# h-walk/PSA

Hardware: AMD Instinct MI355X
Metric: SED throughput (k-points*timesteps*atoms/s) (higher is better)
Workload: dtype f32 (2xf16 split MFMA, fp32 accumulate)

## Files before the change

### include/psa_hip.h

```cpp
#ifndef PSA_HIP_H
#define PSA_HIP_H

#include <stdint.h>

#ifdef __cplusplus
extern "C" {
#endif

#define PSA_HIP_ABI_VERSION 6

#define PSA_OK          0
#define PSA_EINVAL     -1
#define PSA_EHIP       -2
#define PSA_EFFT       -3
#define PSA_ERCCL      -4
#define PSA_ESTATE     -5
#define PSA_ENOMEM     -6

#define PSA_SLOT_VELOCITIES 0
#define PSA_SLOT_POSITIONS  1
#define PSA_NUM_SLOTS       2

#define PSA_F_DISPLACEMENTS  0x1
#define PSA_F_INTENSITY      0x2

#define PSA_K1_AUTO   0
#define PSA_K1_WAVE   1
#define PSA_K1_MFMA32 2
#define PSA_K1_SPLIT_BF16 3

typedef struct psa_ctx psa_ctx;

int         psa_abi_version(void);
const char* psa_last_error(void);
int         psa_device_count(int* count);
int         psa_host_alloc(size_t bytes, void** out);
int         psa_host_free(void* p);
int         psa_create(int device, psa_ctx** out);
int         psa_destroy(psa_ctx* ctx);
int         psa_synchronize(psa_ctx* ctx);
int         psa_set_k1(psa_ctx* ctx, int selector);
int         psa_set_k1_lowrank_fold(psa_ctx* ctx, int on);
#define PSA_OPT_PLANES         0
#define PSA_OPT_PLANES_BUDGET  1
#define PSA_OPT_PLANES_EAGER   2
#define PSA_OPT_PLANES_MIN_K   3
#define PSA_OPT_FOLD_PAIRS     4
#define PSA_OPT_FFT_PRIME      5
#define PSA_OPT_K1_LOADER_WAVES 6
#define PSA_OPT_K1_WIDE         7
#define PSA_OPT_K1_LOWRANK      8
#define PSA_OPT_K1_LOWRANK_MIN_K 9
#define PSA_OPT_K1_LOWRANK_MIN_LOCAL 10
#define PSA_OPT_VDOS_WORK_BYTES 11
#define PSA_OPT_MODES_WORK_BYTES 12
#define PSA_OPT_DYNAMIC_WORK_BYTES 13
#define PSA_OPT_K1_LOWRANK_PAIR 15
int         psa_set_option(psa_ctx* ctx, int option, int64_t value);
int         psa_option_info(int index, int32_t* option, int64_t* default_value, const char** name);
int         psa_device_info(psa_ctx* ctx, char* name, int name_len,
                            int* compute_units, int64_t* hbm_bytes);

int psa_data_upload(psa_ctx* ctx, int slot, const float* host, int64_t T, int64_t N);
int psa_data_alloc(psa_ctx* ctx, int slot, int64_t T, int64_t N);
int psa_data_download(psa_ctx* ctx, int slot, float* host, int64_t t0, int64_t nt);
int psa_data_release(psa_ctx* ctx, int slot);
int psa_data_shape(psa_ctx* ctx, int slot, int64_t* T, int64_t* N);

int psa_data_fill_synthetic(psa_ctx* ctx, int slot, uint64_t seed, int64_t t_offset, int n_modes,
                            const float* amp, const int32_t* mode_comp,
                            const float* ct, const float* st,
                            const float* ca, const float* sa);

int psa_mean_positions(psa_ctx* ctx, int slot, float* mean_host );

int psa_host_mean_frames(const float* x , int64_t T, int64_t cols, float* mean_out, int threads);

int psa_set_atom_weights(psa_ctx* ctx, const float* w , int64_t N);

int psa_set_segments(psa_ctx* ctx, int64_t L, int64_t hop, const float* window );

int psa_sed_project(psa_ctx* ctx, int slot,
                    const float* mean_pos_all,
                    const float* k_vectors, int64_t K_local,
                    int64_t K_total, int64_t k_offset,
                    const int32_t* group_idx, const int64_t* group_off, int32_t G,
                    int32_t flags);

int psa_sed_project_upload(psa_ctx* ctx, int slot, const float* host, int64_t T, int64_t N,
                           const float* mean_pos_all, const float* k_vectors, int64_t K,
                           const int32_t* group_idx, const int64_t* group_off, int32_t G,
                           int32_t flags);

int psa_sed_finalize(psa_ctx* ctx, void* out_host, size_t out_bytes,
                     float* out_intensity, size_t out_intensity_bytes);

int psa_sed_calculate(psa_ctx* ctx, int slot, const float* mean_pos_all,
                      const float* k_vectors, int64_t K,
                      const int32_t* group_idx, const int64_t* group_off, int32_t G,
                      int32_t flags, void* out_host, size_t out_bytes,
                      float* out_intensity, size_t out_intensity_bytes);

int psa_vdos(psa_ctx* ctx, int slot, const float* mean_pos_all ,
             const int32_t* group_idx, const int64_t* group_off, int32_t G,
             int32_t flags , float* out_host , size_t out_bytes);

int psa_sed_modes(psa_ctx* ctx, int slot, const float* mean_pos_all, const float* k_vectors, int64_t K,
                  const int32_t* group_idx, const int64_t* group_off, int32_t B,
                  const void* eig , int64_t M, int32_t flags ,
                  float* out_host , size_t out_bytes);

int psa_sed_covariance(psa_ctx* ctx, int slot, const float* mean_pos_all, const float* k_vectors, int64_t K,
                       const int32_t* group_idx, const int64_t* group_off, int32_t B,
                       const float* freq_weights , int32_t n_w, int32_t flags ,
                       double* out_host , size_t out_bytes);

typedef struct {
    float   window_hwhm;
    int32_t half_window_bins;
    int32_t max_iter;
} psa_peak_opts;
int psa_fit_peaks(psa_ctx* ctx, const float* spec_host, int64_t F, int64_t C, double df, const int32_t* bands, int32_t lo,
                  int32_t hi, const psa_peak_opts* opts, float* fit , int32_t* info );
int psa_sed_modes_fit(psa_ctx* ctx, int slot, const float* mean_pos_all, const float* k_vectors, int64_t K,
                      const int32_t* group_idx, const int64_t* group_off, int32_t B, const void* eig, int64_t M,
// ... 31 lines not shown
                             const int32_t* bin_of , int64_t n_bins, const int32_t* idx, int64_t n_g,
                             int32_t currents , int64_t n_lags,
                             float* out_host , size_t out_bytes);

int psa_self_correlations(psa_ctx* ctx, const double* box_inverse , const int32_t* indices , int64_t K,
                          const int32_t* bin_of , int64_t n_bins, const int32_t* idx, int64_t n_g, int64_t n_lags,
                          float* out_host , size_t out_bytes);

int psa_displacement_moments(psa_ctx* ctx, const double* box , const double* box_inverse , const int32_t* idx,
                             const int64_t* group_start , int32_t n_groups, int64_t n_lags, int64_t origin_step,
                             int32_t unwrap, double* out_host , size_t out_bytes);

int psa_van_hove_self(psa_ctx* ctx, const double* box , const double* box_inverse , const int32_t* idx,
                      const int64_t* group_start , int32_t n_groups, const int64_t* lags , int64_t n_vh,
                      int64_t origin_step, int32_t unwrap, double dr, int32_t n_r, uint64_t* out_host ,
                      size_t out_bytes);

int psa_pair_histogram(psa_ctx* ctx, const double* box , const double* box_inverse , const int32_t* idx,
                       const int64_t* group_start , int32_t n_groups, const int64_t* lags , int64_t n_lags,
                       int64_t origin_step, double dr, int32_t n_r, uint64_t* out_host ,
                       size_t out_bytes);

int psa_angle_histogram(psa_ctx* ctx, const double* box , const double* box_inverse , const int32_t* idx,
                        const int64_t* group_start , int32_t n_groups, const double* r_cut , int64_t origin_step,
                        int32_t n_theta, uint64_t* angles , size_t angles_bytes,
                        uint64_t* coord , size_t coord_bytes, uint64_t* truncated );

int psa_bond_order(psa_ctx* ctx, const double* box , const double* box_inverse , const int32_t* idx,
                   const int64_t* group_start , int32_t n_groups, const double* r_cut , int64_t origin_step,
                   const int32_t* ls , int32_t n_ls, int32_t n_q, uint64_t* hist , size_t hist_bytes,
                   uint64_t* truncated , uint64_t* isolated , uint64_t* undefined ,
                   int64_t* x , int32_t* n );

int psa_local_order(psa_ctx* ctx, const double* box , const double* box_inverse , const int32_t* idx,
                    const int64_t* group_start , int32_t n_groups, const double* r_cut , int64_t origin_step,
                    const int32_t* ls , int32_t n_ls, int32_t n_q, int32_t n_w, double w_range, int32_t solid_l,
                    double solid_threshold, const double* w3j , int64_t w3j_count, uint64_t* hist ,
                    size_t hist_bytes, double* qbar2 , double* w ,
                    double* wbar , int32_t* connections , int32_t* n );

int psa_debug_qlm(psa_ctx* ctx, const double* box , const double* box_inverse , const int32_t* idx,
                  const int64_t* group_start , int32_t n_groups, const double* r_cut , int64_t frame,
                  const int32_t* ls , int32_t n_ls, int64_t* q );

int psa_solid_clusters(psa_ctx* ctx, const double* box , const double* box_inverse , const int32_t* idx,
                       const int64_t* group_start , int32_t n_groups, const double* r_cut , int64_t origin_step,
                       int32_t solid_l, double solid_threshold, int32_t min_connections, int32_t link, int32_t n_sizes,
                       uint64_t* species_rows , uint64_t* size_counts , uint64_t* large_atoms ,
                       int32_t* n_solid , int32_t* n_clusters , int32_t* largest ,
                       int32_t* largest_label , int32_t* labels , int32_t* size_atoms ,
                       int32_t* connections , int32_t* n , uint64_t* bond_masks );

int psa_debug_cluster_labels(psa_ctx* ctx, int64_t n_o, int64_t n_a, const int32_t* count ,
                             const int32_t* list , const uint8_t* solid ,
                             const uint64_t* bond_masks , int32_t link, int32_t n_sizes,
                             uint64_t* size_counts , uint64_t* large_atoms , int32_t* n_solid ,
                             int32_t* n_clusters , int32_t* largest , int32_t* largest_label ,
                             int32_t* labels , int32_t* size_atoms );

int psa_bond_persistence(psa_ctx* ctx, const double* box , const double* box_inverse , const int32_t* idx,
                         const int64_t* group_start , int32_t n_groups, const double* r_cut ,
                         const double* r_break , int64_t origin_step, const int64_t* lags , int32_t n_lags,
                         int64_t sample_step, int32_t continuous, uint64_t* bonds ,
                         uint64_t* alive , uint64_t* unbroken , size_t pair_bytes ,
                         uint64_t* lost , size_t lost_bytes, uint64_t* truncated ,
                         size_t truncated_bytes, uint64_t* alive_masks ,
                         uint64_t* unbroken_masks , size_t masks_bytes );

int psa_common_neighbours(psa_ctx* ctx, const double* box , const double* box_inverse , const int32_t* idx,
                          const int64_t* group_start , int32_t n_groups, const double* r_cut ,
                          int64_t origin_step, uint64_t* signature_counts , size_t signature_bytes,
                          uint64_t* signature_outside , uint64_t* type_counts , size_t type_bytes,
                          uint64_t* truncated , int32_t* types , int32_t* n ,
                          size_t atom_bytes , uint32_t* bond_signatures ,
                          size_t bond_bytes);

#define PSA_KMAP_MIRROR 0x80000000u
int psa_k_pairs(const float* k_vectors, int64_t K, int32_t* kmap ,
                int32_t* unique_idx , int64_t* n_unique);
int psa_sed_set_kmap(psa_ctx* ctx, const int32_t* kmap, int64_t K_out);

int psa_lowrank_plan(const float* k_vectors, int64_t K, const float* mean_pos_all, int64_t N, const int32_t* idx,
                     int64_t n_g, int32_t* ok, double* geo, double* kappa, float* C, float* L, float* phi);

int psa_sed_single_bin(psa_ctx* ctx, int slot, const float* mean_pos_all, const float* k_vector,
                       const int32_t* idx, int64_t n_g, int32_t flags, int64_t i_w,
                       float* out_c64x3 );

int psa_slab_read(psa_ctx* ctx, int64_t row0, int64_t nrows, void* host);
int psa_slab_write(psa_ctx* ctx, int64_t row0, int64_t nrows, const void* host);

int psa_result_intensity(psa_ctx* ctx, float* out_host , size_t out_bytes);
int psa_result_chiral_phase(psa_ctx* ctx, int c1, int c2, float* out_host, size_t out_bytes);

int psa_last_timings(psa_ctx* ctx, double* ms );
int psa_k1_stats(psa_ctx* ctx, int64_t* launches, double* total_ms);
int psa_k1_lowrank_launches(psa_ctx* ctx, int64_t* launches);
int psa_k1_lowrank_pair_launches(psa_ctx* ctx, int64_t* launches);
int psa_lowrank_pair_image(int32_t n_stage, int64_t* index, int64_t* bytes);
int psa_lowrank_fold_image(int32_t n_stage, int64_t* index, int64_t* bytes);
int psa_debug_device_buffers(int64_t* count, int64_t* bytes);
#define PSA_SCRATCH_REAL 0
#define PSA_SCRATCH_INDEX 1
#define PSA_SCRATCH_STATE 2
int psa_debug_scratch_info(int index, const char** name, int32_t* cls);
int psa_debug_scratch_fill(psa_ctx* ctx, int byte, int64_t* buffers, int64_t* bytes);
int psa_oneoff_stats(psa_ctx* ctx, double* ms );

int psa_debug_phase_table(psa_ctx* ctx, const float* mean_pos_all,
                          const float* k_vectors, int64_t K,
                          const int32_t* idx, int64_t n_g, int64_t N,
                          void* out_host);
int psa_debug_project_only(psa_ctx* ctx, int slot, const float* mean_pos_all,
                           const float* k_vectors, int64_t K,
                           const int32_t* idx, int64_t n_g, int32_t flags,
                           void* out_host);
int psa_debug_project_route(psa_ctx* ctx, int slot, const float* mean_pos_all,
                            const float* k_vectors, int64_t K,
                            const int32_t* idx, int64_t n_g, int32_t flags,
                            void* out_host);
int psa_debug_project_frames(psa_ctx* ctx, int slot, const float* mean_pos_all,
                             const float* k_vectors, int64_t K,
                             const int32_t* idx, int64_t n_g, int32_t flags,
                             int64_t t_begin, int64_t t_count, void* out_host);
int psa_debug_mode_power(psa_ctx* ctx, const void* S_host, const void* eig, int32_t B, int64_t K, int64_t M, int64_t T,
                         float* out_host);
int psa_debug_covariance(psa_ctx* ctx, const void* S_host , int32_t B, int64_t K,
                         int64_t T, const float* freq_weights, int32_t n_w, double scale, double* out_host);
int psa_debug_mode_power_welch(psa_ctx* ctx, const void* S_host, const void* eig, int32_t B, int64_t K, int64_t M, int64_t L,
                               int64_t ns, int64_t seg_block, float scale, float* out_host);
int psa_debug_dynamic_project(psa_ctx* ctx, const float* k_vectors, int64_t K, const int32_t* idx, int64_t n_g,
                              int32_t currents, void* out_host);
int psa_debug_dynamic_sincos(psa_ctx* ctx, const float* turns, int64_t n, float* out_host);
int psa_debug_lattice_project(psa_ctx* ctx, const double* box_inverse, const int32_t* indices, int64_t K, const int32_t* idx,
                              int64_t n_g, int32_t currents, void* out_host);
int psa_debug_self_series(psa_ctx* ctx, const double* box_inverse, const int32_t* indices, int64_t K, const int32_t* idx,
                          int64_t n_g, void* out_host);
int psa_debug_dynamic_power(psa_ctx* ctx, const void* seg_host, const float* k_vectors , int64_t K, int32_t currents,
                            int64_t n_seg, int64_t L, int64_t k_block, int64_t seg_block, float scale, float* out_host);
int psa_debug_lattice_shell(psa_ctx* ctx, const void* seg_host, const float* khat , const int32_t* bin_of ,
                            int64_t K, int64_t n_bins, int32_t currents, int64_t n_seg, int64_t L, int64_t k_block,
                            int64_t seg_block, double norm, float* out_host);
int psa_debug_self_power(psa_ctx* ctx, const void* work_host, int64_t na, int64_t nv, int64_t n_seg, int64_t L,
                         const int32_t* groups, int64_t n_groups, int64_t cols, const double* scale, int32_t mirror,
                         int64_t n_chunks, int64_t atom_block, int64_t vec_block, int64_t seg_block, float* out_host);
int psa_debug_partial_project(psa_ctx* ctx, const double* box_inverse, const int32_t* indices, int64_t K, const int32_t* idx,
                              const int64_t* species_start, int32_t n_species, int32_t currents, void* out_host);
int psa_debug_partial_power(psa_ctx* ctx, const void* seg_host, const float* khat , const int32_t* bin_of ,
                            int64_t K, int64_t n_bins, int32_t n_species, int32_t currents, int64_t n_seg, int64_t L,
                            int64_t k_block, int64_t seg_block, double norm, float* out_host);
int psa_debug_plane_cache(psa_ctx* ctx, int64_t* n_sets, int64_t* bytes);

#define PSA_UNIQUE_ID_BYTES 128
int psa_comm_unique_id(void* out );
int psa_comm_init(psa_ctx* ctx, const void* unique_id, int rank, int nranks);
int psa_comm_destroy(psa_ctx* ctx);
int psa_comm_selftest(psa_ctx* ctx);
int psa_sed_gather(psa_ctx* ctx, int root, const int64_t* k_offsets, const int64_t* k_counts);
int psa_comm_barrier(psa_ctx* ctx);

int psa_sed_fs_project(psa_ctx* ctx, int slot, const float* mean_pos_all,
                       const float* k_vectors, int64_t K_total,
                       const int32_t* idx, int64_t n_g, int32_t flags,
                       int64_t T_total, int64_t k_offset, int64_t k_count);
int psa_sed_fs_exchange(psa_ctx* ctx, const int64_t* t_offsets, const int64_t* t_counts,
                        const int64_t* k_offsets, const int64_t* k_counts);
int psa_sed_fs_read(psa_ctx* ctx, int64_t k0, int64_t nk, void* host);
int psa_sed_fs_write(psa_ctx* ctx, int64_t t0, int64_t nt, const void* host);
int psa_sed_fs_finish(psa_ctx* ctx, int32_t first_group);

int psa_debug_correlation_transform(psa_ctx* ctx, const double* X_host, int64_t fields, int64_t P, int64_t cols, int64_t L,
                                    int64_t n_seg, int64_t n_lags, int32_t as_float32, float* out_host);

int psa_debug_unwrap(psa_ctx* ctx, const double* box , const double* box_inverse , const int32_t* idx, int64_t n_g,
                     int32_t unwrap, double* out_u , int32_t* out_images );

int psa_debug_pair_fractions(psa_ctx* ctx, const double* box_inverse , const int32_t* idx, int64_t n_g,
                             float* out );

int psa_debug_pair_plan(const int64_t* sizes , int32_t n_groups, int32_t sym, int64_t n_origins, int64_t* out );

int psa_debug_neighbour_lists(psa_ctx* ctx, const double* box , const double* box_inverse , const int32_t* idx,
                              const int64_t* group_start , int32_t n_groups, const double* r_cut , int64_t frame,
// ... 7 lines not shown
```

### psa_amd/_hip.py

```python
from __future__ import annotations

import ctypes as C
import os
import threading
import weakref
from pathlib import Path
from types import SimpleNamespace
from typing import Optional, Sequence

import numpy as np

LIB_PATH = Path(__file__).resolve().parent / "csrc" / "libpsa_hip.so"

SLOT_VELOCITIES, SLOT_POSITIONS = 0, 1
F_DISPLACEMENTS, F_INTENSITY = 0x1, 0x2
K1_AUTO, K1_WAVE, K1_MFMA32, K1_SPLIT_BF16 = 0, 1, 2, 3
OPT_PLANES, OPT_PLANES_BUDGET, OPT_PLANES_EAGER, OPT_PLANES_MIN_K, OPT_FOLD_PAIRS, OPT_FFT_PRIME = 0, 1, 2, 3, 4, 5
OPT_K1_LOADER_WAVES = 6
OPT_K1_WIDE = 7
OPT_K1_LOWRANK = 8
OPT_K1_LOWRANK_MIN_K = 9
OPT_K1_LOWRANK_MIN_LOCAL = 10
OPT_VDOS_WORK_BYTES = 11
OPT_MODES_WORK_BYTES = 12
OPT_DYNAMIC_WORK_BYTES = 13
OPT_K1_LOWRANK_PAIR = 15
KMAP_MIRROR = 0x80000000
ABI_VERSION = 6
COV_CHAIN = 128
COV_FOLDS = 32
COV_TILE = 64
COV_CHUNK = COV_CHAIN * COV_FOLDS
COV_MAX_ROWS = 96
DYN_THREADS = 256
DYN_ATOMS = 512
DYN_CHAIN = 128
DYN_FRAMES = 4
DYN_SINCOS_ERR = 2.6e-7
LAT_THREADS = 256
LAT_KS = 512
LAT_ATOMS = 128
LAT_TABLE = 3584
LAT_CHAIN = 128
LAT_FRAMES = 4
LAT_MAX_INDEX = 64
LAT_MAX_ENTRIES = 3 * (2 * LAT_MAX_INDEX + 1)
PARTIAL_MAX_SPECIES = 8
SELF_THREADS = 256
SELF_ATOMS = 4
SELF_FRAMES = 64
SELF_ENTRIES = 24
SELF_KS = 64
MSD_LAGS = 256
MSD_ORIGINS = 1024
MSD_WINDOW = 1280
MSD_MAX_GROUPS = 8
MSD_MAX_BINS = 1024
MSD_MAX_VH_LAGS = 64
MSD_UNWRAP_FRAMES = 64
MSD_UNWRAP_ATOMS = 16
PAIR_TILE = 256
PAIR_MAX_BINS = 1024
PAIR_MAX_LAGS = 64
PAIR_MAX_SPECIES = 8
ANGLE_MAX_NEIGHBOURS = 64
ANGLE_MAX_BINS = 1024
ORDER_MAX_L = 12
ORDER_MAX_LS = 8
ORDER_MAX_BINS = 1024
ORDER_SHIFT = 24
LOCAL_MAX_LS = 4
LOCAL_MAX_BINS = 1024
LOCAL_SHIFT = 40
CLUSTER_MAX_SIZES = 4096
CLUSTER_ROW_WORDS = ANGLE_MAX_NEIGHBOURS + 1 + 4
CLUSTER_LINKS = ("neighbours", "solid_bonds")
PERSIST_MAX_LAGS = 1024
CNA_TABLE = (8, 16, 16)
CNA_TYPES = ("other", "fcc", "hcp", "bcc", "ico")
UNIQUE_ID_BYTES = 128
TIMING_NAMES = ("h2d", "phase", "project", "fft", "epilogue", "gather", "transpose", "d2h")

_f32p = C.POINTER(C.c_float)
_i32p = C.POINTER(C.c_int32)
_i64p = C.POINTER(C.c_int64)
_f64p = C.POINTER(C.c_double)
_u64p = C.POINTER(C.c_uint64)
_ctx = C.c_void_p

SIGNATURES = {
    "psa_abi_version": (C.c_int, []),
    "psa_last_error": (C.c_char_p, []),
    "psa_device_count": (C.c_int, [C.POINTER(C.c_int)]),
    "psa_host_alloc": (C.c_int, [C.c_size_t, C.POINTER(C.c_void_p)]),
    "psa_host_free": (C.c_int, [C.c_void_p]),
    "psa_create": (C.c_int, [C.c_int, C.POINTER(_ctx)]),
    "psa_destroy": (C.c_int, [_ctx]),
    "psa_synchronize": (C.c_int, [_ctx]),
    "psa_set_k1": (C.c_int, [_ctx, C.c_int]),
    "psa_set_k1_lowrank_fold": (C.c_int, [_ctx, C.c_int]),
    "psa_set_option": (C.c_int, [_ctx, C.c_int, C.c_int64]),
    "psa_device_info": (C.c_int, [_ctx, C.c_char_p, C.c_int, C.POINTER(C.c_int), _i64p]),
    "psa_data_upload": (C.c_int, [_ctx, C.c_int, _f32p, C.c_int64, C.c_int64]),
    "psa_data_alloc": (C.c_int, [_ctx, C.c_int, C.c_int64, C.c_int64]),
    "psa_data_download": (C.c_int, [_ctx, C.c_int, _f32p, C.c_int64, C.c_int64]),
    "psa_data_release": (C.c_int, [_ctx, C.c_int]),
    "psa_data_shape": (C.c_int, [_ctx, C.c_int, _i64p, _i64p]),
    "psa_data_fill_synthetic": (C.c_int, [_ctx, C.c_int, C.c_uint64, C.c_int64, C.c_int, _f32p, _i32p,
                                          _f32p, _f32p, _f32p, _f32p]),
    "psa_mean_positions": (C.c_int, [_ctx, C.c_int, _f32p]),
    "psa_host_mean_frames": (C.c_int, [_f32p, C.c_int64, C.c_int64, _f32p, C.c_int]),
    "psa_set_atom_weights": (C.c_int, [_ctx, _f32p, C.c_int64]),
    "psa_set_segments": (C.c_int, [_ctx, C.c_int64, C.c_int64, _f32p]),
    "psa_sed_project": (C.c_int, [_ctx, C.c_int, _f32p, _f32p, C.c_int64, C.c_int64, C.c_int64,
                                  _i32p, _i64p, C.c_int32, C.c_int32]),
    "psa_sed_project_upload": (C.c_int, [_ctx, C.c_int, _f32p, C.c_int64, C.c_int64, _f32p, _f32p, C.c_int64,
                                         _i32p, _i64p, C.c_int32, C.c_int32]),
    "psa_sed_finalize": (C.c_int, [_ctx, C.c_void_p, C.c_size_t, _f32p, C.c_size_t]),
    "psa_sed_calculate": (C.c_int, [_ctx, C.c_int, _f32p, _f32p, C.c_int64, _i32p, _i64p,
                                    C.c_int32, C.c_int32, C.c_void_p, C.c_size_t, _f32p, C.c_size_t]),
    "psa_vdos": (C.c_int, [_ctx, C.c_int, _f32p, _i32p, _i64p, C.c_int32, C.c_int32, _f32p, C.c_size_t]),
    "psa_sed_modes": (C.c_int, [_ctx, C.c_int, _f32p, _f32p, C.c_int64, _i32p, _i64p, C.c_int32, C.c_void_p, C.c_int64,
                                C.c_int32, _f32p, C.c_size_t]),
    "psa_fit_peaks": (C.c_int, [_ctx, _f32p, C.c_int64, C.c_int64, C.c_double, _i32p, C.c_int32, C.c_int32, C.c_void_p,
                                _f32p, _i32p]),
    "psa_sed_modes_fit": (C.c_int, [_ctx, C.c_int, _f32p, _f32p, C.c_int64, _i32p, _i64p, C.c_int32, C.c_void_p, C.c_int64,
                                    C.c_int32, C.c_double, _i32p, C.c_int32, C.c_int32, C.c_void_p, _f32p, _i32p, _f32p,
                                    C.c_size_t]),
    "psa_sed_modes_welch": (C.c_int, [_ctx, C.c_int, _f32p, _f32p, C.c_int64, _i32p, _i64p, C.c_int32, C.c_void_p, C.c_int64,
                                      C.c_int32, _f32p, C.c_size_t]),
    "psa_sed_modes_welch_fit": (C.c_int, [_ctx, C.c_int, _f32p, _f32p, C.c_int64, _i32p, _i64p, C.c_int32, C.c_void_p,
                                          C.c_int64, C.c_int32, C.c_double, _i32p, C.c_int32, C.c_int32, C.c_void_p, _f32p,
                                          _i32p, _f32p, C.c_size_t]),
    "psa_dynamic_spectra": (C.c_int, [_ctx, _f32p, C.c_int64, _i32p, C.c_int64, C.c_int32, _f32p, C.c_size_t]),
    "psa_debug_dynamic_project": (C.c_int, [_ctx, _f32p, C.c_int64, _i32p, C.c_int64, C.c_int32, C.c_void_p]),
    "psa_debug_dynamic_sincos": (C.c_int, [_ctx, _f32p, C.c_int64, _f32p]),
    "psa_lattice_spectra": (C.c_int, [_ctx, _f64p, _i32p, C.c_int64, _i32p, C.c_int64, _i32p, C.c_int64, C.c_int32,
                                      _f32p, C.c_size_t]),
    "psa_debug_lattice_project": (C.c_int, [_ctx, _f64p, _i32p, C.c_int64, _i32p, C.c_int64, C.c_int32, C.c_void_p]),
    "psa_self_spectra": (C.c_int, [_ctx, _f64p, _i32p, C.c_int64, _i32p, C.c_int64, _i32p, C.c_int64, _f32p,
                                   C.c_size_t]),
    "psa_debug_self_series": (C.c_int, [_ctx, _f64p, _i32p, C.c_int64, _i32p, C.c_int64, C.c_void_p]),
    "psa_debug_dynamic_power": (C.c_int, [_ctx, C.c_void_p, _f32p, C.c_int64, C.c_int32, C.c_int64, C.c_int64, C.c_int64, C.c_int64,
                                          C.c_float, _f32p]),
    "psa_debug_lattice_shell": (C.c_int, [_ctx, C.c_void_p, _f32p, _i32p, C.c_int64, C.c_int64, C.c_int32, C.c_int64, C.c_int64,
                                          C.c_int64, C.c_int64, C.c_double, _f32p]),
    "psa_debug_self_power": (C.c_int, [_ctx, C.c_void_p, C.c_int64, C.c_int64, C.c_int64, C.c_int64, _i32p, C.c_int64, C.c_int64,
                                       _f64p, C.c_int32, C.c_int64, C.c_int64, C.c_int64, C.c_int64, _f32p]),
    "psa_partial_spectra": (C.c_int, [_ctx, _f64p, _i32p, C.c_int64, _i32p, C.c_int64, _i32p, _i64p, C.c_int32,
                                      C.c_int32, _f32p, C.c_size_t]),
    "psa_debug_partial_project": (C.c_int, [_ctx, _f64p, _i32p, C.c_int64, _i32p, _i64p, C.c_int32, C.c_int32,
                                            C.c_void_p]),
    "psa_debug_partial_power": (C.c_int, [_ctx, C.c_void_p, _f32p, _i32p, C.c_int64, C.c_int64, C.c_int32, C.c_int32, C.c_int64,
                                          C.c_int64, C.c_int64, C.c_int64, C.c_double, _f32p]),
    "psa_lattice_correlations": (C.c_int, [_ctx, _f64p, _i32p, C.c_int64, _i32p, C.c_int64, _i32p, C.c_int64,
                                           C.c_int32, C.c_int64, _f32p, C.c_size_t]),
    "psa_self_correlations": (C.c_int, [_ctx, _f64p, _i32p, C.c_int64, _i32p, C.c_int64, _i32p, C.c_int64,
                                        C.c_int64, _f32p, C.c_size_t]),
    "psa_debug_correlation_transform": (C.c_int, [_ctx, _f64p, C.c_int64, C.c_int64, C.c_int64, C.c_int64,
                                                  C.c_int64, C.c_int64, C.c_int32, _f32p]),
    "psa_displacement_moments": (C.c_int, [_ctx, _f64p, _f64p, _i32p, _i64p, C.c_int32, C.c_int64,
                                           C.c_int64, C.c_int32, _f64p, C.c_size_t]),
    "psa_van_hove_self": (C.c_int, [_ctx, _f64p, _f64p, _i32p, _i64p, C.c_int32, _i64p, C.c_int64,
                                    C.c_int64, C.c_int32, C.c_double, C.c_int32, _u64p, C.c_size_t]),
    "psa_debug_unwrap": (C.c_int, [_ctx, _f64p, _f64p, _i32p, C.c_int64, C.c_int32,
                                   _f64p, _i32p]),
    "psa_pair_histogram": (C.c_int, [_ctx, _f64p, _f64p, _i32p, _i64p, C.c_int32, _i64p, C.c_int64,
                                     C.c_int64, C.c_double, C.c_int32, _u64p, C.c_size_t]),
    "psa_debug_pair_fractions": (C.c_int, [_ctx, _f64p, _i32p, C.c_int64, _f32p]),
    "psa_debug_pair_plan": (C.c_int, [_i64p, C.c_int32, C.c_int32, C.c_int64, _i64p]),
    "psa_angle_histogram": (C.c_int, [_ctx, _f64p, _f64p, _i32p, _i64p, C.c_int32, _f64p,
                                      C.c_int64, C.c_int32, _u64p, C.c_size_t, _u64p, C.c_size_t,
                                      _u64p]),
    "psa_debug_neighbour_lists": (C.c_int, [_ctx, _f64p, _f64p, _i32p, _i64p, C.c_int32,
                                            _f64p, C.c_int64, _i32p, _i32p]),
    "psa_bond_order": (C.c_int, [_ctx, _f64p, _f64p, _i32p, _i64p, C.c_int32, _f64p, C.c_int64,
                                 _i32p, C.c_int32, C.c_int32, _u64p, C.c_size_t, _u64p, _u64p, _u64p,
                                 _i64p, _i32p]),
    "psa_local_order": (C.c_int, [_ctx, _f64p, _f64p, _i32p, _i64p, C.c_int32, _f64p, C.c_int64,
                                  _i32p, C.c_int32, C.c_int32, C.c_int32, C.c_double, C.c_int32, C.c_double,
                                  _f64p, C.c_int64, _u64p, C.c_size_t, _f64p, _f64p, _f64p, _i32p, _i32p]),
    "psa_debug_qlm": (C.c_int, [_ctx, _f64p, _f64p, _i32p, _i64p, C.c_int32, _f64p, C.c_int64,
                                _i32p, C.c_int32, _i64p]),
    "psa_solid_clusters": (C.c_int, [_ctx, _f64p, _f64p, _i32p, _i64p, C.c_int32, _f64p, C.c_int64,
                                     C.c_int32, C.c_double, C.c_int32, C.c_int32, C.c_int32, _u64p, _u64p, _u64p,
                                     _i32p, _i32p, _i32p, _i32p, _i32p, _i32p, _i32p, _i32p, _u64p]),
    "psa_bond_persistence": (C.c_int, [_ctx, _f64p, _f64p, _i32p, _i64p, C.c_int32, _f64p, _f64p, C.c_int64,
                                       _i64p, C.c_int32, C.c_int64, C.c_int32, _u64p, _u64p, _u64p, C.c_size_t,
                                       _u64p, C.c_size_t, _u64p, C.c_size_t, _u64p, _u64p, C.c_size_t]),
    "psa_common_neighbours": (C.c_int, [_ctx, _f64p, _f64p, _i32p, _i64p, C.c_int32, _f64p, C.c_int64, _u64p, C.c_size_t,
                                        _u64p, _u64p, C.c_size_t, _u64p, _i32p, _i32p, C.c_size_t, C.POINTER(C.c_uint32),
                                        C.c_size_t]),
    "psa_debug_cluster_labels": (C.c_int, [_ctx, C.c_int64, C.c_int64, _i32p, _i32p, C.POINTER(C.c_uint8), _u64p, C.c_int32,
                                           C.c_int32, _u64p, _u64p, _i32p, _i32p, _i32p, _i32p, _i32p, _i32p]),
    "psa_k_pairs": (C.c_int, [_f32p, C.c_int64, _i32p, _i32p, _i64p]),
    "psa_lowrank_plan": (C.c_int, [_f32p, C.c_int64, _f32p, C.c_int64, _i32p, C.c_int64, _i32p, _f64p,
                                   _f64p, _f32p, _f32p, _f32p]),
    "psa_sed_set_kmap": (C.c_int, [_ctx, _i32p, C.c_int64]),
    "psa_sed_single_bin": (C.c_int, [_ctx, C.c_int, _f32p, _f32p, _i32p, C.c_int64, C.c_int32, C.c_int64, _f32p]),
    "psa_slab_read": (C.c_int, [_ctx, C.c_int64, C.c_int64, C.c_void_p]),
    "psa_slab_write": (C.c_int, [_ctx, C.c_int64, C.c_int64, C.c_void_p]),
    "psa_result_intensity": (C.c_int, [_ctx, _f32p, C.c_size_t]),
    "psa_result_chiral_phase": (C.c_int, [_ctx, C.c_int, C.c_int, _f32p, C.c_size_t]),
    "psa_last_timings": (C.c_int, [_ctx, _f64p]),
    "psa_k1_stats": (C.c_int, [_ctx, _i64p, _f64p]),
    "psa_k1_lowrank_launches": (C.c_int, [_ctx, _i64p]),
    "psa_k1_lowrank_pair_launches": (C.c_int, [_ctx, _i64p]),
    "psa_lowrank_pair_image": (C.c_int, [C.c_int32, _i64p, _i64p]),
    "psa_lowrank_fold_image": (C.c_int, [C.c_int32, _i64p, _i64p]),
    "psa_oneoff_stats": (C.c_int, [_ctx, _f64p]),
    "psa_option_info": (C.c_int, [C.c_int, C.POINTER(C.c_int32), _i64p, C.POINTER(C.c_char_p)]),
    "psa_debug_device_buffers": (C.c_int, [_i64p, _i64p]),
    "psa_debug_scratch_info": (C.c_int, [C.c_int, C.POINTER(C.c_char_p), C.POINTER(C.c_int32)]),
    "psa_debug_scratch_fill": (C.c_int, [_ctx, C.c_int, _i64p, _i64p]),
    "psa_debug_phase_table": (C.c_int, [_ctx, _f32p, _f32p, C.c_int64, _i32p, C.c_int64,
                                        C.c_int64, C.c_void_p]),
    "psa_debug_project_only": (C.c_int, [_ctx, C.c_int, _f32p, _f32p, C.c_int64, _i32p,
                                         C.c_int64, C.c_int32, C.c_void_p]),
    "psa_debug_project_route": (C.c_int, [_ctx, C.c_int, _f32p, _f32p, C.c_int64, _i32p,
                                          C.c_int64, C.c_int32, C.c_void_p]),
    "psa_debug_project_frames": (C.c_int, [_ctx, C.c_int, _f32p, _f32p, C.c_int64, _i32p,
                                           C.c_int64, C.c_int32, C.c_int64, C.c_int64, C.c_void_p]),
    "psa_debug_mode_power": (C.c_int, [_ctx, C.c_void_p, C.c_void_p, C.c_int32, C.c_int64, C.c_int64, C.c_int64, _f32p]),
    "psa_debug_mode_power_welch": (C.c_int, [_ctx, C.c_void_p, C.c_void_p, C.c_int32, C.c_int64, C.c_int64, C.c_int64,
                                             C.c_int64, C.c_int64, C.c_float, _f32p]),
    "psa_sed_covariance": (C.c_int, [_ctx, C.c_int, _f32p, _f32p, C.c_int64, _i32p, _i64p, C.c_int32, _f32p, C.c_int32, C.c_int32,
                                     C.c_void_p, C.c_size_t]),
    "psa_debug_covariance": (C.c_int, [_ctx, C.c_void_p, C.c_int32, C.c_int64, C.c_int64, _f32p, C.c_int32, C.c_double,
                                       C.c_void_p]),
    "psa_debug_plane_cache": (C.c_int, [_ctx, _i64p, _i64p]),
    "psa_comm_unique_id": (C.c_int, [C.c_void_p]),
    "psa_comm_init": (C.c_int, [_ctx, C.c_void_p, C.c_int, C.c_int]),
    "psa_comm_destroy": (C.c_int, [_ctx]),
    "psa_comm_selftest": (C.c_int, [_ctx]),
    "psa_sed_gather": (C.c_int, [_ctx, C.c_int, _i64p, _i64p]),
    "psa_comm_barrier": (C.c_int, [_ctx]),
    "psa_sed_fs_project": (C.c_int, [_ctx, C.c_int, _f32p, _f32p, C.c_int64, _i32p, C.c_int64, C.c_int32,
                                     C.c_int64, C.c_int64, C.c_int64]),
    "psa_sed_fs_exchange": (C.c_int, [_ctx, _i64p, _i64p, _i64p, _i64p]),
    "psa_sed_fs_read": (C.c_int, [_ctx, C.c_int64, C.c_int64, C.c_void_p]),
    "psa_sed_fs_write": (C.c_int, [_ctx, C.c_int64, C.c_int64, C.c_void_p]),
    "psa_sed_fs_finish": (C.c_int, [_ctx, C.c_int32]),
}


class PeakOpts(C.Structure):
    _fields_ = [("window_hwhm", C.c_float), ("half_window_bins", C.c_int32), ("max_iter", C.c_int32)]


class PsaHipError(RuntimeError):
    """A libpsa_hip entry point returned a non-zero code."""


_lib = None
_lib_lock = threading.Lock()


def load_library() -> C.CDLL:
    global _lib
    with _lib_lock:
        if _lib is not None:
            return _lib
        path = Path(os.environ.get("PSA_HIP_LIBRARY", LIB_PATH))
        if not path.exists():
            raise PsaHipError(
                f"{path} not found: build it with `make -C psa_amd/csrc` (needs hipcc, gfx950). "
                "psa_amd has no CPU fallback.")
        os.environ.setdefault("HSA_ENABLE_IPC_MODE_LEGACY", "0")
        lib = C.CDLL(str(path))
        for name, (res, args) in SIGNATURES.items():
            fn = getattr(lib, name)
            fn.restype, fn.argtypes = res, args
        _lib = lib
        return lib


def _check(rc: int, what: str):
    if rc != 0:
        msg = load_library().psa_last_error().decode("utf-8", "replace")
        if rc == -1 and "out of bounds" in msg:
            raise ValueError(msg)
        raise PsaHipError(f"{what} failed (rc={rc}): {msg}")


def _f32(a: np.ndarray):
    return a.ctypes.data_as(_f32p)


def _as_f32(a, shape_tail=None) -> np.ndarray:
    arr = np.ascontiguousarray(a, dtype=np.float32)
    if shape_tail is not None and arr.shape[1:] != shape_tail:
        raise ValueError(f"expected (*,{shape_tail}) array, got {arr.shape}")
    return arr


def device_count() -> int:
    n = C.c_int(0)
    _check(load_library().psa_device_count(C.byref(n)), "psa_device_count")
    return n.value


def option_table():
    lib, rows = load_library(), []
    opt, default, name = C.c_int32(0), C.c_int64(0), C.c_char_p()
    while lib.psa_option_info(len(rows), C.byref(opt), C.byref(default), C.byref(name)) == 0:
        rows.append((opt.value, name.value.decode(), default.value))
    return rows


def device_buffers():
    n, b = C.c_int64(0), C.c_int64(0)
    _check(load_library().psa_debug_device_buffers(C.byref(n), C.byref(b)), "psa_debug_device_buffers")
    return n.value, b.value


SCRATCH_CLASSES = ("real", "index", "state")


def scratch_table():
    lib, rows = load_library(), []
    name, cls = C.c_char_p(), C.c_int32(0)
    while lib.psa_debug_scratch_info(len(rows), C.byref(name), C.byref(cls)) == 0:
        rows.append((name.value.decode(), SCRATCH_CLASSES[cls.value]))
    return rows


def k_pairs(k_vectors):
    kv = _as_f32(k_vectors, (3,)) if len(k_vectors) else np.zeros((0, 3), np.float32)
    K = kv.shape[0]
    kmap, uidx, n = np.zeros(K, np.int32), np.zeros(K, np.int32), C.c_int64(0)
    _check(load_library().psa_k_pairs(_f32(kv), K, kmap.ctypes.data_as(_i32p), uidx.ctypes.data_as(_i32p), C.byref(n)),
           "psa_k_pairs")
    return kmap.view(np.uint32), uidx[:n.value].copy()


def lowrank_plan(k_vectors, mean_pos_all, idx=None):
    kv = _as_f32(k_vectors, (3,))
    mean = _as_f32(mean_pos_all, (3,))
    K, N = kv.shape[0], mean.shape[0]
    ix = None if idx is None else np.ascontiguousarray(idx, np.int32)
    n_g = N if ix is None else ix.size
    ok, geo = C.c_int32(0), np.zeros(14, np.float64)
    kappa, cm = np.zeros(64, np.float64), np.zeros((K, 64), np.complex64)
    lw, phi = np.zeros((K, 64), np.float32), np.zeros(K, np.complex64)
    _check(load_library().psa_lowrank_plan(_f32(kv), K, _f32(mean), N, None if ix is None else ix.ctypes.data_as(_i32p), n_g,
                                           C.byref(ok), geo.ctypes.data_as(_f64p), kappa.ctypes.data_as(_f64p),
                                           cm.ctypes.data_as(_f32p), _f32(lw), phi.ctypes.data_as(_f32p)), "psa_lowrank_plan")
    if not ok.value:
        return None
    return {"u": geo[0:3].copy(), "k0": geo[3:6].copy(), "x_c": geo[6], "h_x": geo[7], "width": geo[8],
            "interval": int(geo[9]), "d_bound": geo[10], "dscale": geo[11], "e_bound": geo[12],
            "dscale_fold": geo[13], "kappa": kappa, "C": cm, "L": lw, "phi": phi}


def lowrank_pair_image(n_stage: int):
    index, nbytes = np.zeros((512, 32 * int(n_stage)), np.int64), C.c_int64(0)
    _check(load_library().psa_lowrank_pair_image(int(n_stage), index.ctypes.data_as(_i64p), C.byref(nbytes)), "psa_lowrank_pair_image")
    return index, nbytes.value


def lowrank_fold_image(n_stage: int):
    index, nbytes = np.zeros((512, 32 * int(n_stage)), np.int64), C.c_int64(0)
    _check(load_library().psa_lowrank_fold_image(int(n_stage), index.ctypes.data_as(_i64p), C.byref(nbytes)), "psa_lowrank_fold_image")
    return index, nbytes.value


def host_mean_frames(x: np.ndarray, threads: int = 0) -> np.ndarray:
    if x.dtype != np.float32 or not x.flags.c_contiguous or x.ndim < 2 or x.shape[0] < 1 or x.size == 0:
        raise ValueError("host_mean_frames needs a non-empty C-contiguous float32 array")
    out = np.empty(x.shape[1:], np.float32)
    cols = int(np.prod(x.shape[1:], dtype=np.int64))
    _check(load_library().psa_host_mean_frames(_f32(x), x.shape[0], cols, _f32(out), int(threads)), "psa_host_mean_frames")
    return out


def pack_groups(groups: Optional[Sequence[np.ndarray]]):
    if groups is None:
        return None, None, 1
    off = np.zeros(len(groups) + 1, dtype=np.int64)
    off[1:] = np.cumsum([len(g) for g in groups])
    idx = (np.concatenate([np.asarray(g).ravel() for g in groups]) if off[-1] > 0
           else np.zeros(0, dtype=np.int64))
    if idx.size and (idx.min() < 0 or idx.max() >= 2 ** 31):
        raise ValueError("Atom indices in basis out of bounds.")
    return np.ascontiguousarray(idx, dtype=np.int32), off, len(groups)


class _PinnedPool:

    granule = 2 << 20
    min_bytes = 1 << 20
    keep_bytes = 4 << 30
    max_live_bytes = 16 << 30

    def __init__(self):
        self._idle = {}
        self._idle_bytes = 0
        self._live_bytes = 0
        self._lock = threading.Lock()
        self.stats = {"recycled": 0, "allocated": 0, "pageable": 0}

    def _give_back(self, address: int, size: int):
        with self._lock:
            self._live_bytes -= size
            if self._idle_bytes + size <= self.keep_bytes:
                self._idle.setdefault(size, []).append(address)
                self._idle_bytes += size
                return
        load_library().psa_host_free(C.c_void_p(address))

    def empty(self, shape, dtype) -> np.ndarray:
        dtype = np.dtype(dtype)
        nbytes = int(np.prod(shape, dtype=np.int64)) * dtype.itemsize
        if nbytes < self.min_bytes:
            return np.empty(shape, dtype)
        size = -(-nbytes // self.granule) * self.granule
        with self._lock:
            if self._live_bytes + size > self.max_live_bytes:
                self.stats["pageable"] += 1
                return np.empty(shape, dtype)
            self._live_bytes += size
            stack = self._idle.get(size)
            address = stack.pop() if stack else None
            if address is not None:
                self._idle_bytes -= size
        if address is None:
            p = C.c_void_p()
            try:
                _check(load_library().psa_host_alloc(size, C.byref(p)), "psa_host_alloc")
            except PsaHipError:
                with self._lock:
                    self._live_bytes -= size
                    self.stats["pageable"] += 1
                return np.empty(shape, dtype)
            address = p.value
            self.stats["allocated"] += 1
        else:
            self.stats["recycled"] += 1
        block = (C.c_char * size).from_address(address)
        weakref.finalize(block, self._give_back, address, size)
        return np.frombuffer(block, dtype=dtype, count=nbytes // dtype.itemsize).reshape(shape)

    def drain(self):
        with self._lock:
            idle, self._idle, self._idle_bytes = self._idle, {}, 0
        for stack in idle.values():
            for address in stack:
                load_library().psa_host_free(C.c_void_p(address))


_pinned_pool = _PinnedPool()


def pinned_empty(shape, dtype) -> np.ndarray:
    return _pinned_pool.empty(shape, dtype)


_SAMPLE_CACHE = {}


def _sample_positions(shape):
    hit = _SAMPLE_CACHE.get(shape)
    if hit is None:
        size = int(np.prod(shape, dtype=np.int64))
        lin = np.arange(0, size, max(1, size // 1021), dtype=np.int64)[:1021]
        if size > 2048:
            lin = np.concatenate([lin, np.sort(np.random.default_rng(size).integers(0, size, 1021)), [size - 1]])
        if len(_SAMPLE_CACHE) > 64:
            _SAMPLE_CACHE.clear()
        hit = _SAMPLE_CACHE[shape] = (lin, np.unravel_index(lin, shape))
    return hit


class Engine:

    def __init__(self, device: Optional[int] = None):
        self._lib = load_library()
        if device is None:
            device = int(os.environ.get("PSA_HIP_DEVICE", os.environ.get("LOCAL_RANK", "0")))
            n = device_count()
            if n == 0:
                raise PsaHipError("no HIP device visible; psa_amd has no CPU fallback")
            device %= n
        h = _ctx()
        _check(self._lib.psa_create(int(device), C.byref(h)), "psa_create")
        self._h = h
        self.device = int(device)
        self._resident = {}
        self._converted = {}
        self.lock = threading.RLock()
        self.rank, self.nranks = 0, 1
        self.result_serial = 0
        self.segment_length = 0

    def close(self):
        if getattr(self, "_h", None):
            self._lib.psa_destroy(self._h)
            self._h = None

    def __del__(self):
        try:
            self.close()
        except Exception:
            pass

    def synchronize(self):
        _check(self._lib.psa_synchronize(self._h), "psa_synchronize")

    def set_k1(self, selector: int):
        _check(self._lib.psa_set_k1(self._h, selector), "psa_set_k1")

    def set_lowrank_fold(self, on: bool):
        _check(self._lib.psa_set_k1_lowrank_fold(self._h, int(bool(on))), "psa_set_k1_lowrank_fold")

    def device_info(self) -> dict:
        name = C.create_string_buffer(256)
        cu, mem = C.c_int(0), C.c_int64(0)
        _check(self._lib.psa_device_info(self._h, name, 256, C.byref(cu), C.byref(mem)),
               "psa_device_info")
        return {"name": name.value.decode(), "compute_units": cu.value, "hbm_bytes": mem.value}

    @staticmethod
    def _fingerprint(a: np.ndarray) -> int:
        if a.size == 0:
            return 0
        base = a
        while base is not None and not isinstance(base, np.memmap):
            base = getattr(base, "base", None)
        if base is not None and getattr(base, "filename", None):
            try:
                st = os.stat(base.filename)
                return hash((str(base.filename), st.st_size, st.st_mtime_ns, a.shape, a.strides))
            except OSError:
                pass
        lin, idx = _sample_positions(a.shape)
        if a.flags.c_contiguous:
            return hash(a.reshape(-1)[lin].tobytes())
        return hash(a[idx].tobytes())

    def _as_device_layout(self, slot: int, array: np.ndarray) -> np.ndarray:
        if array.ndim != 3 or array.shape[2] != 3:
            raise ValueError("trajectory array must be (frames, atoms, 3)")
        if array.dtype == np.float32 and array.flags.c_contiguous:
            return array
        held = self._converted.get(slot)
        fp = self._fingerprint(array)
        if held is not None and held[0]() is array and held[1] == fp:
            return held[2]
        conv = np.ascontiguousarray(array, dtype=np.float32)
        try:
            self._converted[slot] = (weakref.ref(array), fp, conv)
        except TypeError:
            self._converted.pop(slot, None)
        return conv

    def is_resident(self, slot: int, array: np.ndarray) -> bool:
        held = self._resident.get(slot)
        if held is None or held[0] is None:
            return False
        a = array if held[0]() is array else self._as_device_layout(slot, array)
        return (held[0]() is a and held[1:3] == (a.ctypes.data, a.shape) and held[3] == self._fingerprint(a))

    def _note_resident(self, slot: int, a: np.ndarray):
        try:
            ref = weakref.ref(a)
        except TypeError:
            ref = None
        self._resident[slot] = (ref, a.ctypes.data, a.shape, self._fingerprint(a))

    def ensure_resident(self, slot: int, array: np.ndarray):
        if self.is_resident(slot, array):
            return
        a = self._as_device_layout(slot, array)
        T, N = a.shape[0], a.shape[1]
        _check(self._lib.psa_data_upload(self._h, slot, _f32(a), T, N), "psa_data_upload")
        self._note_resident(slot, a)

    def invalidate(self, slot: Optional[int] = None):
        if slot is None:
            self._resident.clear()
            self._converted.clear()
        else:
            self._resident.pop(slot, None)
            self._converted.pop(slot, None)

    def alloc(self, slot: int, T: int, N: int):
        _check(self._lib.psa_data_alloc(self._h, slot, T, N), "psa_data_alloc")
        self._resident[slot] = (None, None, (T, N, 3), None)

    def fill_synthetic(self, slot: int, seed: int, amp, comp, ct, st, ca, sa, t_offset: int = 0):
        amp = np.ascontiguousarray(amp, np.float32)
        comp = np.ascontiguousarray(comp, np.int32)
        tabs = [np.ascontiguousarray(x, np.float32) for x in (ct, st, ca, sa)]
        _check(self._lib.psa_data_fill_synthetic(
            self._h, slot, C.c_uint64(seed), int(t_offset), len(amp), _f32(amp), comp.ctypes.data_as(_i32p),
            *[_f32(t) for t in tabs]), "psa_data_fill_synthetic")

# ... 841 lines not shown
```

### psa_amd/csrc/api_core.hip

```cpp
#include "api_internal.h"

#include <unistd.h>

#include <atomic>
#include <filesystem>

namespace psa {

thread_local std::string g_error;


void set_error(const char* fmt, ...) {
    char    buf[1024];
    va_list ap;
    va_start(ap, fmt);
    vsnprintf(buf, sizeof(buf), fmt, ap);
    va_end(ap);
    g_error = buf;
}

static std::atomic<int64_t> g_devbuf_count{0}, g_devbuf_bytes{0};

int DevBuf::reserve(size_t bytes) {
    if (bytes <= cap) return PSA_OK;
// ... 305 lines not shown
    c->compute_units = prop.multiProcessorCount;
    if (const char* v = std::getenv("PSA_K1_LOWRANK")) c->opt_k1_lowrank = std::atoi(v) != 0;
    if (const char* v = std::getenv("PSA_K1_LOWRANK_MIN_K")) c->opt_k1_lowrank_min_k = std::max(1, std::atoi(v));
    hipError_t e = hipStreamCreateWithFlags(&c->stream, hipStreamNonBlocking);
    if (e != hipSuccess) {
        delete c;
        set_error("hipStreamCreate failed: %s", hipGetErrorString(e));
        return PSA_EHIP;
    }
    *out = c;
    return PSA_OK;
}

int psa_destroy(psa_ctx* c) {
    if (!c) return PSA_OK;
    { Guard g(c); }
    (void)hipSetDevice(c->device);
    delete c;
    return PSA_OK;
}

int psa_debug_device_buffers(int64_t* count, int64_t* bytes) {
    PSA_REQUIRE(count != nullptr && bytes != nullptr, "null argument");
    *count = g_devbuf_count.load();
    *bytes = g_devbuf_bytes.load();
    return PSA_OK;
}

int psa_debug_scratch_info(int index, const char** name, int32_t* cls) {
    PSA_REQUIRE(index >= 0 && index < (int)std::size(SCRATCH), "no device buffer at index %d", index);
    if (name) *name = SCRATCH[index].name;
    if (cls) *cls = SCRATCH[index].cls;
    return PSA_OK;
}

int psa_debug_scratch_fill(psa_ctx* c, int byte, int64_t* buffers, int64_t* bytes) {
    PSA_TRY(enter(c));
    PSA_REQUIRE(byte >= -1 && byte <= 255, "the fill byte is 0 .. 255, or -1 to disarm");
    Guard g(c);
    PSA_HIP_CHECK(hipStreamSynchronize(c->stream));
    if (c->d2h_stream) PSA_HIP_CHECK(hipStreamSynchronize(c->d2h_stream));
    if (c->stager.copy_stream) PSA_HIP_CHECK(hipStreamSynchronize(c->stager.copy_stream));
    int64_t n = 0, total = 0;
    c->scratch_byte = byte;
    for (const Scratch& s : SCRATCH) {
        DevBuf& b = c->*s.member;
        b.fill = byte < 0 || s.cls == PSA_SCRATCH_STATE ? nullptr : s.cls == PSA_SCRATCH_REAL ? &c->scratch_byte : &SCRATCH_ZERO;
        if (!b.fill || !b.ptr) continue;
        PSA_HIP_CHECK(hipMemsetAsync(b.ptr, *b.fill, b.cap, c->stream));
        n += 1;
        total += (int64_t)b.cap;
    }
    PSA_HIP_CHECK(hipStreamSynchronize(c->stream));
    if (byte >= 0) c->slab_valid = c->out_valid = c->inten_valid = false;
    if (buffers) *buffers = n;
    if (bytes) *bytes = total;
    return PSA_OK;
}

int psa_synchronize(psa_ctx* c) {
    PSA_TRY(enter(c));
    Guard g(c);
    PSA_HIP_CHECK(hipStreamSynchronize(c->stream));
    return PSA_OK;
}

int psa_set_k1(psa_ctx* c, int selector) {
    PSA_TRY(enter(c));
    PSA_REQUIRE(selector == PSA_K1_AUTO || selector == PSA_K1_WAVE || selector == PSA_K1_MFMA32 ||
                    selector == PSA_K1_SPLIT_BF16,
                "unknown K1 selector %d", selector);
    Guard g(c);
    c->k1_selector = selector;
    return PSA_OK;
}

int psa_set_k1_lowrank_fold(psa_ctx* c, int on) {
    PSA_TRY(enter(c));
    Guard g(c);
    c->k1_lowrank_fold = on != 0;
    return PSA_OK;
}

int psa_set_option(psa_ctx* c, int option, int64_t value) {
    PSA_TRY(enter(c));
    Guard g(c);
    for (const Option& o : OPTIONS) {
        if (o.id != option) continue;
        if (o.min == OPT_FLAG) value = value != 0;
        else if (o.min == 0) PSA_REQUIRE(value >= 0, "negative plane budget");
        else PSA_REQUIRE(value >= o.min, "%s must be >= %lld", o.name, (long long)o.min);
        c->*o.field = value;
        if (option == PSA_OPT_PLANES && !value) {
            PSA_HIP_CHECK(hipStreamSynchronize(c->stream));
            c->planes.clear();
        } else if (option == PSA_OPT_K1_LOWRANK && !value) {
            PSA_HIP_CHECK(hipStreamSynchronize(c->stream));
            for (DevBuf* b : {&c->d_lr_diff, &c->d_lr_qn, &c->d_lr_L, &c->d_lr_phi, &c->d_lr_f64}) b->release();
        }
        return PSA_OK;
    }
    set_error("unknown option %d", option);
    return PSA_EINVAL;
}

int psa_option_info(int index, int32_t* option, int64_t* default_value, const char** name) {
    PSA_REQUIRE(index >= 0 && index < (int)std::size(OPTIONS), "no option at index %d", index);
    if (option) *option = OPTIONS[index].id;
    if (default_value) *default_value = OPTIONS[index].def;
    if (name) *name = OPTIONS[index].name;
    return PSA_OK;
}

int psa_device_info(psa_ctx* c, char* name, int name_len, int* compute_units, int64_t* hbm_bytes) {
    PSA_TRY(enter(c));
    hipDeviceProp_t prop;
    PSA_HIP_CHECK(hipGetDeviceProperties(&prop, c->device));
    if (name && name_len > 0) {
        std::snprintf(name, (size_t)name_len, "%s (%s)", prop.name[0] ? prop.name : "AMD GPU",
                      prop.gcnArchName);
    }
    if (compute_units) *compute_units = prop.multiProcessorCount;
    if (hbm_bytes) *hbm_bytes = (int64_t)prop.totalGlobalMem;
    return PSA_OK;
}

int psa_last_timings(psa_ctx* c, double* ms) {
    PSA_TRY(enter(c));
    PSA_REQUIRE(ms != nullptr, "null output");
    Guard guard(c);
    TimingState& ts = timing(c);
    PSA_TRY(collect(c, ts));
    for (int i = 0; i < PSA_T_COUNT; ++i) {
        ms[i] = ts.acc[i];
        ts.acc[i] = 0.0;
    }
    return PSA_OK;
}

int psa_oneoff_stats(psa_ctx* c, double* ms) {
    PSA_TRY(enter(c));
    PSA_REQUIRE(ms != nullptr, "null output");
    Guard guard(c);
    for (int i = 0; i < 4; ++i) {
        ms[i] = c->oneoff_ms[i];
        c->oneoff_ms[i] = 0.0;
    }
    return PSA_OK;
}

int psa_k1_lowrank_launches(psa_ctx* c, int64_t* launches) {
    PSA_TRY(enter(c));
    PSA_REQUIRE(launches != nullptr, "null argument");
    *launches = c->lowrank_launches;
    return PSA_OK;
}

int psa_k1_lowrank_pair_launches(psa_ctx* c, int64_t* launches) {
    PSA_TRY(enter(c));
    PSA_REQUIRE(launches != nullptr, "null argument");
    *launches = c->lowrank_pair_launches;
    return PSA_OK;
}

int psa_k1_stats(psa_ctx* c, int64_t* launches, double* total_ms) {
    PSA_TRY(enter(c));
// ... 12 lines not shown
```

### psa_amd/csrc/api_internal.h

```cpp
#pragma once
#include <algorithm>
#include <chrono>
#include <cmath>
#include <condition_variable>
#include <cstdlib>
#include <cstring>
#include <functional>
#include <thread>
#include <unordered_map>

#include "k1_f16.h"

namespace psa {

extern thread_local std::string g_error;

struct HostTimer {
    double*                               into;
    std::chrono::steady_clock::time_point t0 = std::chrono::steady_clock::now();
    explicit HostTimer(double* into_) : into(into_) {}
    ~HostTimer() { *into += std::chrono::duration<double, std::milli>(std::chrono::steady_clock::now() - t0).count(); }
};

struct Guard {
// ... 18 lines not shown
    TimingState& ts;
    int          stage;
    hipEvent_t   e0 = nullptr, e1 = nullptr;
    bool         ok = false;
    StageTimer(psa_ctx* c_, int stage_) : c(c_), ts(timing(c_)), stage(stage_) {
        if (get_event(ts, &e0) == PSA_OK && get_event(ts, &e1) == PSA_OK &&
            hipEventRecord(e0, c->stream) == hipSuccess)
            ok = true;
    }
    ~StageTimer() {
        if (ok && hipEventRecord(e1, c->stream) == hipSuccess) {
            ts.pending.push_back({stage, e0, e1});
            return;
        }
        for (hipEvent_t ev : {e0, e1})
            if (ev) ts.pool.push_back(ev);
    }
};

int upload(psa_ctx* c, DevBuf& b, const void* host, size_t bytes);
int get_plan(psa_ctx* c, int64_t T, int64_t batch, FftPlan** out);
void prime_fft(psa_ctx* c, int64_t T);
int run_fft(psa_ctx* c, float2* data, int64_t T, int64_t batch);
int check_slot(psa_ctx* c, int slot);
int validate_groups(int64_t N, const int32_t* group_idx, const int64_t* group_off, int32_t G);

struct GroupView {
    int            slot = 0;
    bool           disp = false;
    int64_t        n_g = 0;
    const int*     d_idx = nullptr;
    const int32_t* h_idx = nullptr;
    PlaneSet*      ps = nullptr;
};
inline void set_group(const psa_ctx* c, const int32_t* group_idx, const int64_t* group_off, int gi, int64_t N, GroupView* v) {
    v->n_g = group_idx ? group_off[gi + 1] - group_off[gi] : N;
    v->d_idx = group_idx ? c->d_idx.as<int>() + group_off[gi] : nullptr;
    v->h_idx = group_idx ? group_idx + group_off[gi] : nullptr;
}

int  slot_absmax(psa_ctx* c, int slot);
int  group_absmax(psa_ctx* c, int slot, const int32_t* h_idx, int64_t n_g, unsigned* bits);
int  displaced_absmax(psa_ctx* c, int slot, const float* mean_host, const int32_t* h_idx, int64_t n_g, unsigned* bits);
int  stager_init(psa_ctx* c, size_t chunk_bytes);
void stager_release(psa_ctx* c);
int  staged_upload(psa_ctx* c, float* dev, const float* host, int64_t T, int64_t N,
                   const std::function<int(int64_t, int64_t, hipEvent_t)>& on_chunk);
int  data_alloc_locked(psa_ctx* c, int slot, int64_t T, int64_t N);
int  materialise_displacements(psa_ctx* c, GroupView* v, const float* mean_host);

struct ProjectArgs {
    int            slot;
    const float*   mean_pos_all;
    const float*   k_vectors;
    int64_t        K_local, K_total, k_offset;
    const int32_t* group_idx;
    const int64_t* group_off;
    int32_t        G, flags;
};

enum class GeomRule { product, bf16_anywhere, f32_only };

size_t planes_bytes_held(psa_ctx* c);
void   drop_stale_planes(psa_ctx* c);
int    get_planes(psa_ctx* c, const GroupView& v, int64_t K_local, const float* mean_host, PlaneSet** out);
int    group_source(psa_ctx* c, GroupView* v, const float* mean_host, int64_t K);
int    make_geom(psa_ctx* c, const GroupView& v, int64_t K_local, GeomRule rule, ProjGeom* g);
int    prepare_phase(psa_ctx* c, const GroupView& v, const ProjGeom& g, int64_t k_first);
int    launch_projection(psa_ctx* c, const GroupView& v, ProjGeom g, float2* d_q, int64_t q_stride, int64_t t_begin,
                         int64_t t_count);
int    prepare_block(psa_ctx* c, const GroupView& v, GeomRule rule, const ProjectArgs* lowrank, int64_t k_first, int64_t nk,
                     ProjGeom* g);
int    project_block(psa_ctx* c, const GroupView& v, const ProjectArgs* lowrank, int64_t k_first, int64_t nk, float2* d_q);
int    check_group_indices(const GroupView& v, int64_t N);
int    upload_single_group(psa_ctx* c, GroupView* v, int64_t N, const float* k_vectors, int64_t K, const float* mean_pos_all);
void   fold_pairs(const float* k, int64_t K, std::vector<int32_t>* kmap, std::vector<int32_t>* unique_idx);
int    install_kmap(psa_ctx* c, const std::vector<int32_t>& kmap);
struct LowRankPlan {
    bool                ok = false;
    const char*         why = "";
    double              u[3] = {0, 0, 0}, k0[3] = {0, 0, 0};
    double              x_c = 0, h_x = 0, width = 0;
    int64_t             interval = 0;
    double              kappa[LOWRANK_NODES] = {};
    double              d_bound = 0;
    float               dscale = 0.f;
    double              e_bound = 0;
    float               dscale_fold = 0.f;
    std::vector<double> kline;
    std::vector<float>  L;
    std::vector<float>  phi;
};
int plan_lowrank(const float* k, int64_t K, const float* mean_all, int64_t N, const int32_t* h_idx, int64_t n_g, LowRankPlan* p,
                 float* C = nullptr);
int prepare_lowrank(psa_ctx* c, const GroupView& v, const ProjectArgs& list, int64_t k_first, int64_t nk, ProjGeom* g);
struct ModesArgs {
    int            slot;
    const float*   mean_pos_all;
    const float*   k_vectors;
    int64_t        K;
    const int32_t* group_idx;
    const int64_t* group_off;
    int32_t        B;
    const float*   eig;
    int64_t        M;
    int32_t        flags;
    float*         out;
    size_t         out_bytes;
};
int modes_run(psa_ctx* c, const ModesArgs& a, bool segments, bool device_only);
struct ModesCall {
    int64_t                T = 0, N = 0, K = 0, M = 0;
    int32_t                B = 0;
    int                    MT = 0;
    size_t                 coef_k = 0;
    int64_t                per_k = 0;
    int64_t                kb_max = 0;
    ProjectArgs            list;
    std::vector<float>     coef;
    std::vector<GroupView> src;
};
int     modes_check_groups(psa_ctx* c, int slot, const float* mean_pos_all, const float* k_vectors, int64_t K, const int32_t* group_idx,
                           const int64_t* group_off, int32_t B, int32_t flags, ModesCall* m);
int     modes_upload(psa_ctx* c, ModesCall* m);
int64_t modes_block(const psa_ctx* c, const ModesCall& m, int64_t k0, int64_t kb);
int     modes_project(psa_ctx* c, const ModesCall& m, int64_t k0, int64_t nk, float2* d_work);
struct PeakArgs {
    int64_t        F, C;
    double         df;
    const int32_t* bands;
    int32_t        lo, hi;
    psa_peak_opts  opts;
    float*         fit;
    int32_t*       info;
    int            row0 = 0, row_end = 0;
};
int check_peak_args(const psa_peak_opts* opts, PeakArgs* a);
int peaks_run(psa_ctx* c, const float* d_spec, const PeakArgs& a);
struct DynCall {
    int64_t T = 0, N = 0, K = 0, n_g = 0;
    int     NC = 1, slices = 1;
    int     n_species = 1;
    bool    cut = false;
    int64_t L = 0, H = 0, n_seg = 0;
    int64_t n_lags = 0, P = 0;
    int64_t per_k = 0, unit = 0;
    int64_t kb = 0, bk = 0, bs = 0;
    std::vector<float> kappa, khat;
};
int dynamic_inputs(psa_ctx* c, const char* entry, int64_t K, const int32_t* idx, int64_t n_g, int32_t currents, DynCall* d);
int segment_shape(const psa_ctx* c, bool segments, DynCall* d);
int dynamic_plan(psa_ctx* c, DynCall* d);
struct PowerPass {
    int          NC = 1;
    int          n_species = 0;
    int64_t      L = 0, n_seg = 0, K = 0;
    float        scale = 0.f;
    const float* d_khat = nullptr;
    float*       d_out = nullptr;
    const int*   d_bins = nullptr;
    double*      d_acc = nullptr;
    int64_t      n_bins = 0;
};
using SegFill = std::function<int(int64_t k1, int64_t nb, int64_t s0, int64_t ns, const float2** d_seg)>;
int  power_block(psa_ctx* c, const PowerPass& p, int64_t k0, int64_t nk, int64_t bk, int64_t bs, const SegFill& fill);
struct BlockSource {
    std::function<int()>                                                     upload;
    std::function<int(int64_t block, int64_t k0, int64_t nk, float2* d_q)> project;
};
struct SpectraRun {
    BlockSource src;
    bool        pairs = false;
    int64_t     n_bins = 0;
    std::function<int(const float* d_power, const double* d_acc)> finish;
    float*      out_host = nullptr;
    size_t      out_bytes = 0;
};
// ... 108 lines not shown
```

### psa_amd/csrc/api_lowrank.hip

```cpp
#include "api_internal.h"
#include "k1_lowrank_fold.h"
#include "k1_lowrank_pair.h"

namespace psa {

namespace {
constexpr double LR_OMEGA = 30.0;
constexpr double LR_D_MAX = 1.0 / 8192.0;
}

int plan_lowrank(const float* k, int64_t K, const float* mean_all, int64_t N, const int32_t* h_idx, int64_t n_g, LowRankPlan* p,
                 float* C) {
    *p = LowRankPlan{};
    auto fail = [&](const char* why) {
        p->why = why;
        return PSA_OK;
    };
    if (K < 2) return fail("fewer than two k-vectors");
    if (n_g < 1) return fail("empty group");
    for (int64_t i = 0; i < 3 * K; ++i)
        if (!std::isfinite(k[i])) return fail("k-vector not finite");
    double  p0[3] = {k[0], k[1], k[2]}, far = 0.0;
    int64_t jf = 0;
    for (int64_t j = 1; j < K; ++j) {
        double d2 = 0.0;
        for (int i = 0; i < 3; ++i) d2 += ((double)k[3 * j + i] - p0[i]) * ((double)k[3 * j + i] - p0[i]);
        if (d2 > far) {
            far = d2;
            jf = j;
        }
    }
    if (!(far > 0.0)) return fail("all k-vectors equal");
    double u[3], nu = std::sqrt(far);
    for (int i = 0; i < 3; ++i) u[i] = ((double)k[3 * jf + i] - p0[i]) / nu;
    {
        int im = 0;
        for (int i = 1; i < 3; ++i)
            if (std::fabs(u[i]) > std::fabs(u[im])) im = i;
        if (u[im] < 0)
            for (double& v : u) v = -v;
    }
    bool snapped = false;
    for (int n = 1; n <= 12 && !snapped; ++n) {
        double m[3], mn = 0.0, dev = 0.0;
        const double s = n / std::max({std::fabs(u[0]), std::fabs(u[1]), std::fabs(u[2])});
        for (int i = 0; i < 3; ++i) {
            m[i] = std::nearbyint(u[i] * s);
            mn += m[i] * m[i];
        }
        mn = std::sqrt(mn);
        for (int i = 0; i < 3; ++i) dev = std::max(dev, std::fabs(m[i] / mn - u[i]));
        if (dev < 1e-6) {
            for (int i = 0; i < 3; ++i) u[i] = m[i] / mn + 0.0;
            snapped = true;
        }
    }
    if (!snapped) return fail("direction not a lattice direction");
    {
        double kmax2 = 0.0, off2 = 0.0;
        for (int64_t j = 0; j < K; ++j) {
            double kj[3], d = 0.0, n2 = 0.0;
            for (int i = 0; i < 3; ++i) {
                kj[i] = k[3 * j + i];
                d += kj[i] * u[i];
                n2 += kj[i] * kj[i];
            }
            double o2 = 0.0;
            for (int i = 0; i < 3; ++i) o2 += (kj[i] - d * u[i]) * (kj[i] - d * u[i]);
            kmax2 = std::max(kmax2, n2);
            off2 = std::max(off2, o2);
        }
        if (!(std::sqrt(off2) <= 1e-5 * std::sqrt(kmax2))) return fail("line does not pass through Gamma");
    }
    for (int i = 0; i < 3; ++i) p->u[i] = u[i];
    double xmin = INFINITY, xmax = -INFINITY, rmax = 0.0, rabs[3] = {0, 0, 0};
    for (int64_t a = 0; a < n_g; ++a) {
        const int64_t src = h_idx ? h_idx[a] : a;
        if (src < 0 || src >= N) return fail("index outside the trajectory");
        const float* r = mean_all + 3 * src;
        if (!std::isfinite(r[0]) || !std::isfinite(r[1]) || !std::isfinite(r[2])) return fail("mean position not finite");
        const double x = u[0] * r[0] + u[1] * r[1] + u[2] * r[2];
        xmin = std::min(xmin, x);
        xmax = std::max(xmax, x);
        rmax = std::max(rmax, std::sqrt((double)r[0] * r[0] + (double)r[1] * r[1] + (double)r[2] * r[2]));
        for (int i = 0; i < 3; ++i) rabs[i] = std::max(rabs[i], (double)std::fabs(r[i]));
    }
    p->x_c = 0.5 * (xmin + xmax);
    p->h_x = std::max(0.5 * (xmax - xmin), 1e-12);
    p->width = 2.0 * LR_OMEGA / p->h_x;
    p->kline.resize((size_t)3 * K);
    std::vector<double> kap((size_t)K);
    double              off = 0.0, kabs[3] = {0, 0, 0};
    for (int64_t j = 0; j < K; ++j) {
        double kj[3], kk = 0.0;
        for (int i = 0; i < 3; ++i) {
            kj[i] = k[3 * j + i];
            kk += (kj[i] - p->k0[i]) * u[i];
            kabs[i] = std::max(kabs[i], std::fabs(kj[i]));
        }
        kap[(size_t)j] = kk;
        double e2 = 0.0;
        for (int i = 0; i < 3; ++i) {
            p->kline[3 * j + i] = p->k0[i] + kk * u[i];
            e2 += (kj[i] - p->kline[3 * j + i]) * (kj[i] - p->kline[3 * j + i]);
        }
        off = std::max(off, std::sqrt(e2));
    }
    p->d_bound = 0x1p-22 * (kabs[0] * rabs[0] + kabs[1] * rabs[1] + kabs[2] * rabs[2]) + off * rmax + 0x1p-20;
    if (!(p->d_bound <= LR_D_MAX)) return fail("k-vectors not on one line (or phases too large)");
    bool pos = true, neg = true;
    for (int64_t j = 0; j < K; ++j) {
        pos = pos && kap[(size_t)j] >= 0.0;
        neg = neg && kap[(size_t)j] <= 0.0;
    }
    if (!pos && !neg) return fail("k-list crosses Gamma");
    const bool   side = pos;
    const double n0 = std::floor(std::fabs(kap[0]) / p->width);
    for (int64_t j = 0; j < K; ++j)
        if (std::floor(std::fabs(kap[(size_t)j]) / p->width) != n0) return fail("k-path longer than one node interval");
    p->interval = side ? (int64_t)n0 : -(int64_t)n0 - 1;
    const double mid = (p->interval + 0.5) * p->width, half = 0.5 * p->width;
    double       bw[LOWRANK_NODES];
    for (int l = 0; l < LOWRANK_NODES; ++l) {
        const double th = M_PI * (2 * l + 1) / (2.0 * LOWRANK_NODES);
        p->kappa[l] = mid + half * std::cos(th);
        bw[l] = ((l & 1) ? -1.0 : 1.0) * std::sin(th);
    }
    p->L.assign((size_t)K * LOWRANK_NODES, 0.f);
    p->phi.assign((size_t)K * 2, 0.f);
    for (int64_t j = 0; j < K; ++j) {
        const double kj = kap[(size_t)j];
        double       L[LOWRANK_NODES], den = 0.0;
        int          hit = -1;
        for (int l = 0; l < LOWRANK_NODES; ++l)
            if (kj == p->kappa[l]) hit = l;
        if (hit >= 0) {
            for (int l = 0; l < LOWRANK_NODES; ++l) L[l] = l == hit;
        } else {
            for (int l = 0; l < LOWRANK_NODES; ++l) {
                L[l] = bw[l] / (kj - p->kappa[l]);
                den += L[l];
            }
            for (double& v : L) v /= den;
        }
        const double cr = std::cos(kj * p->x_c), ci = std::sin(kj * p->x_c);
        p->phi[(size_t)j * 2 + 0] = (float)cr;
        p->phi[(size_t)j * 2 + 1] = (float)ci;
        for (int l = 0; l < LOWRANK_NODES; ++l) {
            p->L[(size_t)j * LOWRANK_NODES + l] = (float)L[l];
            if (C) {
                C[((size_t)j * LOWRANK_NODES + l) * 2 + 0] = (float)(cr * L[l]);
                C[((size_t)j * LOWRANK_NODES + l) * 2 + 1] = (float)(ci * L[l]);
            }
        }
    }
    p->dscale = std::ldexp(1.0f, 14 - (int)std::ceil(std::log2(p->d_bound)));
    for (int64_t j = 0; j < K; ++j) {
        double lam = 0.0;
        for (int l = 0; l < LOWRANK_NODES; ++l) lam += std::fabs((double)p->L[(size_t)j * LOWRANK_NODES + l]);
        const double rot = std::fabs((double)p->phi[(size_t)j * 2]) + std::fabs((double)p->phi[(size_t)j * 2 + 1]);
        p->e_bound = std::max(p->e_bound, rot * lam * 0x1p-12);
    }
    p->dscale_fold = std::ldexp(1.0f, 14 - (int)std::ceil(std::log2(p->d_bound + p->e_bound)));
    p->ok = true;
    return PSA_OK;
}

int prepare_lowrank(psa_ctx* c, const GroupView& v, const ProjectArgs& list, int64_t k_first, int64_t nk, ProjGeom* g) {
    g->lowrank = false;
    if (!c->opt_k1_lowrank || g->split != K1Family::f16_planes || !v.ps || list.K_total < c->opt_k1_lowrank_min_k ||
        nk < c->opt_k1_lowrank_min_local)
        return PSA_OK;
    LowRankPlan p;
    PSA_TRY(plan_lowrank(list.k_vectors + 3 * k_first, nk, list.mean_pos_all, c->slot[v.slot].N, v.h_idx, g->n_g, &p));
    if (!p.ok) return PSA_OK;
    std::vector<double> f64((size_t)7 + LOWRANK_NODES + 3 * (size_t)nk);
    std::memcpy(f64.data(), p.k0, 3 * sizeof(double));
    std::memcpy(f64.data() + 3, p.u, 3 * sizeof(double));
    f64[6] = p.x_c;
    std::memcpy(f64.data() + 7, p.kappa, sizeof(p.kappa));
    std::memcpy(f64.data() + 7 + LOWRANK_NODES, p.kline.data(), p.kline.size() * sizeof(double));
    PSA_TRY(upload(c, c->d_lr_f64, f64.data(), f64.size() * sizeof(double)));
    PSA_TRY(upload(c, c->d_lr_L, p.L.data(), p.L.size() * sizeof(float)));
    PSA_TRY(upload(c, c->d_lr_phi, p.phi.data(), p.phi.size() * sizeof(float)));
    PSA_TRY(c->d_lr_qn.reserve((size_t)LOWRANK_NODES * 3 * (size_t)c->slot[v.slot].T * sizeof(float2)));
    g->lowrank = true;
    g->lr_fold = c->k1_lowrank_fold;
    g->dscale = g->lr_fold ? p.dscale_fold : p.dscale;
    g->M_pad_d = (int)((2 * nk + 511) / 512 * 512);
    g->lr_pair = c->opt_k1_lowrank_pair && g->M_pad_d == LRP_ROWS;
    static_assert(LRF_ROWS == LRP_ROWS, "the folded pair launch serves the lists the pair launch serves");
    return PSA_OK;
}

}

using namespace psa;

extern "C" {

int psa_lowrank_plan(const float* k_vectors, int64_t K, const float* mean_pos_all, int64_t N, const int32_t* idx, int64_t n_g,
                     int32_t* ok, double* geo, double* kappa, float* C, float* L, float* phi) {
    PSA_REQUIRE(K >= 0 && K < (1ll << 29) && N >= 1 && n_g >= 0 && n_g <= (idx ? (int64_t)1 << 30 : N) && ok && geo &&
                    (K == 0 || k_vectors) && mean_pos_all,
                "bad argument");
    LowRankPlan p;
    PSA_TRY(plan_lowrank(k_vectors, K, mean_pos_all, N, idx, n_g, &p, C));
    *ok = p.ok;
    const double g[14] = {p.u[0],  p.u[1],    p.u[2],           p.k0[0],   p.k0[1],  p.k0[2],   p.x_c,
                          p.h_x,   p.width,   (double)p.interval, p.d_bound, p.dscale, p.e_bound, p.dscale_fold};
    std::memcpy(geo, g, sizeof(g));
    if (p.ok && kappa) std::memcpy(kappa, p.kappa, sizeof(p.kappa));
    if (p.ok && L) std::memcpy(L, p.L.data(), p.L.size() * sizeof(float));
    if (p.ok && phi) std::memcpy(phi, p.phi.data(), p.phi.size() * sizeof(float));
    return PSA_OK;
}

int psa_lowrank_pair_image(int32_t n_stage, int64_t* index, int64_t* bytes) {
    PSA_REQUIRE(n_stage >= 1 && n_stage < (1 << 20) && bytes, "bad argument");
    *bytes = (int64_t)pd16_pair_table_bytes(n_stage);
    if (index)
        for (int m = 0; m < LRP_ROWS; ++m)
            for (int a = 0; a < n_stage * K1_BA; ++a) index[(size_t)m * n_stage * K1_BA + a] = (int64_t)pd16_pair_index(m, a, n_stage);
    return PSA_OK;
}

int psa_lowrank_fold_image(int32_t n_stage, int64_t* index, int64_t* bytes) {
    PSA_REQUIRE(n_stage >= 1 && n_stage < (1 << 20) && bytes, "bad argument");
    *bytes = (int64_t)pd16_fold_table_bytes(n_stage);
    if (index)
        for (int m = 0; m < LRF_ROWS; ++m)
            for (int a = 0; a < n_stage * K1_BA; ++a) index[(size_t)m * n_stage * K1_BA + a] = (int64_t)pd16_fold_index(m, a, n_stage);
    return PSA_OK;
}

}
```

### psa_amd/csrc/api_project.hip

```cpp
#include "api_internal.h"

namespace psa {

uint64_t hash_idx(const int32_t* p, int64_t n) {
    uint64_t h = 1469598103934665603ull ^ (uint64_t)n;
    for (int64_t i = 0; i < n; ++i) h = (h ^ (uint32_t)p[i]) * 1099511628211ull;
    return h;
}

void fold_pairs(const float* k, int64_t K, std::vector<int32_t>* kmap, std::vector<int32_t>* unique_idx) {
    struct Key {
        uint32_t x, y, z;
        bool operator==(const Key& o) const { return x == o.x && y == o.y && z == o.z; }
    };
    struct KeyHash {
        size_t operator()(const Key& a) const {
            uint64_t h = 1469598103934665603ull;
            for (uint32_t v : {a.x, a.y, a.z}) h = (h ^ v) * 1099511628211ull;
            return (size_t)h;
        }
    };
    auto bits = [](float v, bool negate) {
        if (negate) v = -v;
        if (v == 0.f) v = 0.f;
// ... 142 lines not shown
    ps->slot = slot;
    ps->generation = s.generation;
    ps->all_atoms = all;
    if (!all) ps->idx.assign(h_idx, h_idx + n_g);
    ps->idx_hash = h;
    ps->displaced = displaced;
    if (displaced) ps->mean.assign(mean_host, mean_host + n_mean);
    ps->T = s.T;
    ps->n_fg = n_fg;
    ps->n_g = (int)n_g;
    ps->A_pad = A_pad;
    ps->vscale = vscale;
    ps->last_use = ++c->plane_tick;
    *out = ps.get();
    c->planes.push_back(std::move(ps));
    return PSA_OK;
}

int check_weights(psa_ctx* c, int64_t N) {
    PSA_REQUIRE(c->weights_N == 0 || c->weights_N == N, "atom weights were set for %lld atoms, the trajectory has %lld",
                (long long)c->weights_N, (long long)N);
    return PSA_OK;
}

void set_geom_weights(const psa_ctx* c, ProjGeom* g) {
    g->weights = c->weights_N ? c->d_weights.as<float>() : nullptr;
    g->wscale = c->weights_N ? c->weights_scale : 1.f;
}

int make_geom(psa_ctx* c, const GroupView& v, int64_t K_local, GeomRule rule, ProjGeom* g) {
    const int     slot = v.slot;
    const int64_t n_g = v.n_g;
    set_geom_weights(c, g);
    g->T = c->slot[slot].T;
    g->q_stride = g->T;
    g->N_tot = c->slot[slot].N;
    PSA_REQUIRE(n_g < (1ll << 30) && K_local < (1ll << 29), "group or k-list too large");
    g->n_g = (int)n_g;
    g->A_pad = (int)((n_g + 31) / 32 * 32);
    g->K = (int)K_local;
    g->split = K1Family::f32;
    const bool autosel = c->k1_selector == PSA_K1_AUTO;
    if (v.ps && rule == GeomRule::product) {
        g->split = K1Family::f16_planes;
        g->vscale = v.ps->vscale;
        g->m_blk = k1_planes_block_rows((int)K_local, c->opt_k1_wide != 0);
        g->A_pad = v.ps->A_pad;
        g->M_pad = (int)((2 * K_local + g->m_blk - 1) / g->m_blk * g->m_blk);
        return PSA_OK;
    }
    if (rule == GeomRule::product && autosel && k1_pair_eligible(v.d_idx, g->N_tot, n_g, K_local, v.disp)) {
        unsigned bits = 0;
        if (v.h_idx) {
            PSA_TRY(group_absmax(c, slot, v.h_idx, n_g, &bits));
        } else {
            PSA_TRY(slot_absmax(c, slot));
            bits = c->slot[slot].absmax_bits;
        }
        g->vscale = k1_f16_vscale(bits);
        if (g->vscale > 0.f) g->split = K1Family::f16_fly;
    }
    if (g->split == K1Family::f32 && rule != GeomRule::f32_only && (autosel || c->k1_selector == PSA_K1_SPLIT_BF16) &&
        k1_split_eligible(v.d_idx, g->N_tot, n_g, v.disp))
        g->split = K1Family::bf16;
    if (g->split == K1Family::f16_fly) {
        g->m_blk = k1_pair_block_rows((int)K_local);
        g->A_pad = k1_pair_atom_pad(n_g);
    } else {
        g->m_blk = g->split == K1Family::bf16 ? k1_split_block_rows((int)K_local) : k1_mfma_block_rows((int)K_local);
    }
    g->M_pad = (int)((2 * K_local + g->m_blk - 1) / g->m_blk * g->m_blk);
    return PSA_OK;
}

int prepare_phase(psa_ctx* c, const GroupView& v, const ProjGeom& g, int64_t k_first) {
    const int*   d_idx = v.d_idx;
    const float* d_kvec = c->d_kvec.as<float>() + 3 * k_first;
    const bool   f16 = g.split == K1Family::f16_fly || g.split == K1Family::f16_planes, bf16 = g.split == K1Family::bf16;
    if (g.lowrank) {
        PSA_TRY(c->d_lr_diff.reserve(pd16_table_bytes(g.M_pad_d, g.A_pad)));
        PSA_TRY(c->d_phase.reserve(pf16_table_bytes(128, g.A_pad)));
        StageTimer    st(c, PSA_T_PHASE);
        const double* f64 = c->d_lr_f64.as<double>();
        if (g.lr_fold)
            return launch_lowrank_tables_fold(c, d_kvec, f64 + 7 + LOWRANK_NODES, f64, f64 + 7, c->d_mean_all.as<float>(), d_idx,
                                              c->d_lr_L.as<float>(), c->d_lr_phi.as<float2>(), c->d_lr_diff.ptr, c->d_phase.ptr, g,
                                              g.M_pad_d, g.dscale, g.lr_pair);
        return launch_lowrank_tables(c, d_kvec, f64 + 7 + LOWRANK_NODES, f64, f64 + 7, c->d_mean_all.as<float>(), d_idx,
                                     c->d_lr_diff.ptr, c->d_phase.ptr, g, g.M_pad_d, g.dscale, g.lr_pair);
    }
    PSA_TRY(c->d_phase.reserve(f16    ? pf16_table_bytes(g.M_pad, g.A_pad)
                               : bf16 ? pb_table_bytes(g.M_pad, g.A_pad)
                                      : p_table_floats(g.M_pad, g.A_pad) * sizeof(float)));
    StageTimer st(c, PSA_T_PHASE);
    if (f16)
        PSA_TRY(launch_phase_table_f16(c, d_kvec, c->d_mean_all.as<float>(), d_idx, c->d_phase.ptr, g));
    else if (bf16)
        PSA_TRY(launch_phase_table_split(c, d_kvec, c->d_mean_all.as<float>(), d_idx, c->d_phase.ptr, g));
    else
        PSA_TRY(launch_phase_table(c, d_kvec, c->d_mean_all.as<float>(), d_idx, c->d_phase.as<float>(), g));
    if (v.disp) {
        PSA_TRY(c->d_mean_g.reserve((size_t)g.A_pad * 3 * sizeof(float)));
        PSA_TRY(launch_gather_mean(c, c->d_mean_all.as<float>(), d_idx, c->d_mean_g.as<float>(), g));
    }
    return PSA_OK;
}

static int launch_projection_once(psa_ctx* c, const GroupView& v, ProjGeom g, float2* d_q, int64_t q_stride, int64_t t_begin,
                                  int64_t t_count);

int launch_projection(psa_ctx* c, const GroupView& v, ProjGeom g, float2* d_q, int64_t q_stride, int64_t t_begin,
                      int64_t t_count) {
    static const int reps = [] {
        const char* e = std::getenv("PSA_DEBUG_REPEAT_K1");
        return e ? std::max(1, std::atoi(e)) : 1;
    }();
    for (int r = 0; r < reps; ++r) PSA_TRY(launch_projection_once(c, v, g, d_q, q_stride, t_begin, t_count));
    return PSA_OK;
}

static int launch_projection_once(psa_ctx* c, const GroupView& v, ProjGeom g, float2* d_q, int64_t q_stride, int64_t t_begin,
                                  int64_t t_count) {
    const DataSlot& s = c->slot[v.slot];
    const PlaneSet* ps = v.ps;
    PSA_REQUIRE(t_begin >= 0 && t_count > 0 && t_begin + t_count <= s.T && q_stride >= t_begin + t_count,
                "frame range [%lld,%lld) outside the slot", (long long)t_begin, (long long)(t_begin + t_count));
    g.T = t_count;
    g.q_stride = q_stride;
    StageTimer   st(c, PSA_T_PROJECT);
    const float* d_v = s.buf.as<float>() + (size_t)t_begin * 3 * (size_t)s.N;
    d_q += t_begin;
    if (g.split == K1Family::f16_planes) {
        PSA_REQUIRE(ps != nullptr && t_begin % 16 == 0, "planes are cut in groups of 16 frames");
        const int64_t fg0 = t_begin / 16, n_fg = ps->n_fg - fg0;
        const _Float16* pl = ps->buf.as<_Float16>() + (size_t)fg0 * (size_t)(ps->A_pad / K1_BA) * PL_STAGE_ELEMS;
        if (g.lowrank) {
            ProjGeom gn = g;
            gn.K = LOWRANK_NODES;
            gn.m_blk = gn.M_pad = 2 * LOWRANK_NODES;
            gn.q_stride = t_count;
            PSA_REQUIRE(c->d_lr_qn.cap >= (size_t)LOWRANK_NODES * 3 * t_count * sizeof(float2), "node projections not reserved");
            if (g.lr_pair) {
                PSA_TRY((g.lr_fold ? launch_k1_lowrank_fold : launch_k1_lowrank_pair)(c, pl, c->d_phase.ptr, c->d_lr_diff.ptr,
                                                                                      c->d_lr_qn.as<float2>(), d_q, g, n_fg, g.dscale));
                ++c->lowrank_pair_launches;
            } else {
                PSA_TRY((g.lr_fold ? launch_k1_planes_lw2 : launch_k1_planes_lw)(c, pl, c->d_phase.ptr, c->d_lr_qn.as<float2>(), gn, n_fg));
                ProjGeom gd = g;
                gd.M_pad = g.M_pad_d;
                PSA_TRY(launch_k1_planes_diff(c, pl, c->d_lr_diff.ptr, d_q, gd, n_fg, g.dscale));
            }
            PSA_TRY(launch_lowrank_combine_r(c, c->d_lr_qn.as<float2>(), c->d_lr_L.as<float>(), c->d_lr_phi.as<float2>(), d_q, g,
                                             t_count));
            ++c->lowrank_launches;
            return PSA_OK;
        }
        if (g.m_blk == 256) return launch_k1_planes_wide(c, pl, c->d_phase.ptr, d_q, g, n_fg);
        if (g.m_blk == 128 && c->opt_k1_loader_waves) return launch_k1_planes_lw(c, pl, c->d_phase.ptr, d_q, g, n_fg);
        return launch_k1_planes(c, pl, c->d_phase.ptr, d_q, g, n_fg);
    }
    if (g.split == K1Family::f16_fly) return launch_k1_pair(c, d_v, c->d_phase.ptr, v.d_idx, d_q, g);
    if (g.split == K1Family::bf16) return launch_k1_split(c, d_v, c->d_phase.ptr, v.d_idx, d_q, g);
    if (c->k1_selector == PSA_K1_WAVE)
        return launch_k1_wave(c, d_v, c->d_phase.as<float>(), v.d_idx, c->d_mean_g.as<float>(), d_q, g, v.disp);
    return launch_k1_mfma(c, d_v, c->d_phase.as<float>(), v.d_idx, c->d_mean_g.as<float>(), d_q, g, v.disp);
}

int prepare_block(psa_ctx* c, const GroupView& v, GeomRule rule, const ProjectArgs* lowrank, int64_t k_first, int64_t nk,
                  ProjGeom* g) {
    PSA_TRY(make_geom(c, v, nk, rule, g));
    if (lowrank) PSA_TRY(prepare_lowrank(c, v, *lowrank, k_first, nk, g));
    return prepare_phase(c, v, *g, k_first);
}

int project_block(psa_ctx* c, const GroupView& v, const ProjectArgs* lowrank, int64_t k_first, int64_t nk, float2* d_q) {
    const int64_t T = c->slot[v.slot].T;
    ProjGeom      g;
    PSA_TRY(prepare_block(c, v, GeomRule::product, lowrank, k_first, nk, &g));
    return launch_projection(c, v, g, d_q, T, 0, T);
}

int group_source(psa_ctx* c, GroupView* v, const float* mean_host, int64_t K) {
    PSA_TRY(get_planes(c, *v, K, v->disp ? mean_host : nullptr, &v->ps));
    if (v->ps) {
        v->disp = false;
        return PSA_OK;
    }
    return materialise_displacements(c, v, mean_host);
}

int check_group_indices(const GroupView& v, int64_t N) {
    for (int64_t i = 0; v.h_idx && i < v.n_g; ++i)
        PSA_REQUIRE(v.h_idx[i] >= 0 && v.h_idx[i] < N, "Atom indices in basis out of bounds.");
    return PSA_OK;
}

int upload_single_group(psa_ctx* c, GroupView* v, int64_t N, const float* k_vectors, int64_t K, const float* mean_pos_all) {
    if (v->n_g == 0) return PSA_OK;
    PSA_TRY(upload(c, c->d_kvec, k_vectors, (size_t)K * 3 * sizeof(float)));
    PSA_TRY(upload(c, c->d_mean_all, mean_pos_all, (size_t)N * 3 * sizeof(float)));
    if (v->h_idx) PSA_TRY(upload(c, c->d_idx, v->h_idx, (size_t)v->n_g * sizeof(int32_t)));
    v->d_idx = v->h_idx ? c->d_idx.as<int>() : nullptr;
    return PSA_OK;
}

int check_project_args(psa_ctx* c, const ProjectArgs& a, int64_t N) {
    PSA_REQUIRE(a.mean_pos_all != nullptr, "null mean_pos_all");
    PSA_REQUIRE(a.K_local >= 0 && a.K_total >= 1 && a.k_offset >= 0 && a.k_offset + a.K_local <= a.K_total,
                "k range [%lld,%lld) outside [0,%lld)", (long long)a.k_offset, (long long)(a.k_offset + a.K_local),
                (long long)a.K_total);
    PSA_REQUIRE(a.K_local == 0 || a.k_vectors != nullptr, "null k_vectors");
    PSA_TRY(validate_groups(N, a.group_idx, a.group_off, a.G));
    PSA_REQUIRE((a.flags & PSA_F_INTENSITY) || a.G == 1, "complex output needs exactly one atom group (got %d)", a.G);
    (void)c;
    return PSA_OK;
}

int begin_result(psa_ctx* c, int64_t T, int64_t K_total, int64_t k_offset, bool intensity, char** rows) {
    PSA_TRY(c->d_slab.reserve(row_bytes(T, intensity) * (size_t)K_total));
    c->res_T = T;
    c->res_K = K_total;
    c->res_intensity = intensity;
    c->slab_valid = true;
    c->out_valid = false;
    c->inten_valid = false;
    c->kmap.clear();
    c->out_K = K_total;
// ... 565 lines not shown
```

### psa_amd/csrc/k1_planes_diff.hip

```cpp
#include <utility>

#include "k1_f16.h"
#include "k1_lowrank_fold.h"
#include "k1_lowrank_pair.h"

namespace psa {

namespace {
constexpr int D_M_BLK = 512, D_T_BLK = 64, D_MT = 16, D_PERIOD = 40;
constexpr int D_STAGE_UNITS = 44, D_RING_UNITS = 160, D_EARLY = D_RING_UNITS - 3 * D_STAGE_UNITS;
constexpr int D_STAGE_BYTES = D_M_BLK * K1_BA * 2;
static_assert(D_EARLY == 28 && D_RING_UNITS % 4 == 0 && D_STAGE_UNITS % 4 == 0, "ring arithmetic");
constexpr auto d_unit_off = unit_off<D_STAGE_UNITS, D_RING_UNITS, D_PERIOD>;
}

__host__ __device__ inline size_t pd16_index(int m, int a, int n_stage) {
    const int row = m % D_M_BLK, rt = row >> 4, v = 2 * (rt & 15) + (rt >> 4), r = row & 15, al = a % K1_BA;
    return (((size_t)(m / D_M_BLK) * n_stage + a / K1_BA) * 32 + v) * (16 * K1_BA) + (size_t)r * K1_BA +
           (size_t)((((al >> 3) ^ pl_swizzle(r)) << 3) + (al & 7));
}
size_t pd16_table_bytes(int M_pad, int A_pad) { return ((size_t)M_pad * A_pad + 4 * (size_t)D_M_BLK * K1_BA) * 2; }

template <bool NT_V>
__global__ void __launch_bounds__(512, 2)
k1_planes_diff_kernel(const _Float16* __restrict__ planes, const _Float16* __restrict__ Db, float2* __restrict__ Q, int64_t T,
                      int64_t q_stride, int n_fg, int n_stage, int K, int n_mblk, int n_tblk, float qscale) {
    using PR = F16x2;
    using E8 = PR::v8;
    __shared__ __attribute__((aligned(16))) unsigned char smem[D_RING_UNITS * 1024];
    const unsigned lds0 = (unsigned)(size_t)(lds_u8*)smem;

    int mb, tb;
    if (!k1_block_map(n_mblk, n_tblk, mb, tb)) return;

    const int tid = threadIdx.x, lane = tid & 63;
    const int w = __builtin_amdgcn_readfirstlane(tid >> 6);
    const int wh = w >> 2, wf = w & 3;
    const int r16 = lane & 15, q = lane >> 4;

    const unsigned char* src[11];
    {
        int fg = tb * 4 + (w & 3);
        if (fg >= n_fg) fg = n_fg - 1;
        const unsigned char* pl0 = reinterpret_cast<const unsigned char*>(planes) + (size_t)fg * n_stage * PL_STAGE_BYTES;
#pragma unroll
        for (int i = 0; i < 3; ++i) src[i] = pl0 + 1024 * (2 * i);
        const unsigned char* d0 = reinterpret_cast<const unsigned char*>(Db) + (size_t)mb * n_stage * D_STAGE_BYTES;
#pragma unroll
        for (int i = 3; i < 11; ++i) src[i] = d0 + 1024 * ((w & 3) + 4 * (i - 3));
    }
    const unsigned dma_voff = 16 * lane;
    const unsigned wbase = lds0 + 1024 * (w & 3);
    using std::integral_constant;
    auto dma = [&](auto s40_c, auto i_c) __attribute__((always_inline)) {
        constexpr int      S40 = decltype(s40_c)::value, I = decltype(i_c)::value;
        constexpr unsigned OFF = d_unit_off(S40, 4 * I);
        if constexpr (I < 3) {
            lds_dma16_at<OFF, NT_V>(src[I], dma_voff, wbase);
            src[I] += PL_STAGE_BYTES;
        } else {
            lds_dma16_at<OFF, false>(src[I], dma_voff, wbase);
            src[I] += D_STAGE_BYTES;
        }
    };
    auto dma_range = [&]<int S40, int... Is>(integral_constant<int, S40>, std::integer_sequence<int, Is...>) __attribute__((always_inline)) {
        (dma(integral_constant<int, S40>{}, integral_constant<int, Is>{}), ...);
    };
    auto dma_late = [&](auto s40_c) __attribute__((always_inline)) {
        dma_range(s40_c, std::integer_sequence<int, 7, 8, 9, 10>{});
    };
    auto dma_early = [&](auto s40_c) __attribute__((always_inline)) {
        dma_range(s40_c, std::make_integer_sequence<int, 7>{});
    };

    const unsigned lane_off = lds0 + r16 * (K1_BA * 2) + ((q ^ pl_swizzle(r16)) << 4);
    unsigned       lane_a[3], lane_b[3];
    unit_ring_windows(lane_off + 1024 * wh, lane_off + 1024 * wf, lane_a, lane_b);
    E8    a[4];
    E8    bf[3];
    f32x4 acc[D_MT][3];
    auto  read_a = [&](auto s40_c, auto mt_c) __attribute__((always_inline)) {
        constexpr int S40 = decltype(s40_c)::value, MTI = decltype(mt_c)::value;
        a[MTI & 3] = lds_frag(lane_a, d_unit_off(S40, 12 + 2 * MTI));
    };
    auto read_b = [&](auto s40_c, auto c_c) __attribute__((always_inline)) {
        constexpr int S40 = decltype(s40_c)::value, CC = decltype(c_c)::value;
// ... 147 lines not shown
                       const int* __restrict__ idx, const float* __restrict__ w, float wnorm, const _Float16* __restrict__ Pn,
                       const float* __restrict__ L, const float2* __restrict__ phi, _Float16* __restrict__ Db, int K, int n_g,
                       int A_pad, float dscale) {
    const int a = blockIdx.y * 256 + threadIdx.x;
    const int k0 = blockIdx.x * FOLD_JB;
    if (a >= A_pad) return;
    const int n_stage = A_pad / K1_BA;
    _Float16  wl[2 * LOWRANK_NODES];
#pragma unroll
    for (int m = 0; m < 2 * LOWRANK_NODES; ++m) wl[m] = Pn[pf16_tile_index(1, m, a, 2 * LOWRANK_NODES, n_stage)];
    for (int k = k0; k < k0 + FOLD_JB; ++k) {
        float d[2] = {0.f, 0.f};
        if (k < K && a < n_g) {
            const float* Lk = L + (size_t)k * LOWRANK_NODES;
            float        sr = 0.f, si = 0.f;
#pragma unroll
            for (int l = 0; l < LOWRANK_NODES; ++l) {
                sr = __fmaf_rn(Lk[l], (float)wl[2 * l], sr);
                si = __fmaf_rn(Lk[l], (float)wl[2 * l + 1], si);
            }
            const float2 ph = phi[k];
            const float  er = __fmaf_rn(-ph.y, si, __fmul_rn(ph.x, sr)), ei = __fmaf_rn(ph.y, sr, __fmul_rn(ph.x, si));
            float        cs[2];
            double       se, ce, wa;
            diff_parts(kvec, kline, mean_all, idx, w, wnorm, k, a, cs, ce, se, wa);
            constexpr double inv_p = 1.0 / (double)F16x2::P_SCALE;
            d[0] = (float)((((double)cs[0] - ce) * wa + (double)er * inv_p) * (double)dscale);
            d[1] = (float)((((double)cs[1] - se) * wa + (double)ei * inv_p) * (double)dscale);
        }
        Db[FOLD ? pd16_fold_index(2 * k, a, n_stage) : pd16_index(2 * k, a, n_stage)] = (_Float16)d[0];
        Db[FOLD ? pd16_fold_index(2 * k + 1, a, n_stage) : pd16_index(2 * k + 1, a, n_stage)] = (_Float16)d[1];
    }
}

int launch_lowrank_tables_fold(psa_ctx* c, const float* d_kvec, const double* d_kline, const double* d_geo, const double* d_kappa,
                               const float* d_mean_all, const int* d_idx, const float* d_L, const float2* d_phi, void* d_diff,
                               void* d_nodes, const ProjGeom& g, int M_pad_d, float dscale, bool pair) {
    PSA_REQUIRE(M_pad_d % D_M_BLK == 0 && M_pad_d >= 2 * g.K && g.A_pad % K1_BA == 0, "bad low-rank table geometry");
    PSA_REQUIRE(!pair || M_pad_d == LRF_ROWS, "the folded pair launch's image is one 512-row block");
    static_assert((D_M_BLK / 2) % FOLD_JB == 0, "whole blocks of rows");
    hipLaunchKernelGGL(node_table_kernel, dim3(LOWRANK_NODES, (g.A_pad + 255) / 256), dim3(256), 0, c->stream, d_geo, d_kappa, d_mean_all,
                       d_idx, g.weights, 1.f / g.wscale, (_Float16*)d_nodes, g.n_g, g.A_pad);
    PSA_HIP_CHECK(hipGetLastError());
    hipLaunchKernelGGL(pair ? diff_fold_table_kernel<true> : diff_fold_table_kernel<false>,
                       dim3(M_pad_d / 2 / FOLD_JB, (g.A_pad + 255) / 256), dim3(256), 0, c->stream, d_kvec, d_kline, d_mean_all, d_idx,
                       g.weights, 1.f / g.wscale, (const _Float16*)d_nodes, d_L, d_phi, (_Float16*)d_diff, g.K, g.n_g, g.A_pad, dscale);
    PSA_HIP_CHECK(hipGetLastError());
    if (pair) {
        const size_t n_stage = (size_t)g.A_pad / K1_BA, a_pad = LRF_PAD_STAGES * LRF_A_UNITS * 1024, b_pad = LRF_PAD_STAGES * LRF_B_UNITS * 1024;
        static_assert(LRF_ROWS == D_M_BLK, "the fold image has the size of one D block");
        PSA_HIP_CHECK(hipMemsetAsync((char*)d_diff + n_stage * LRF_A_UNITS * 1024, 0, a_pad, c->stream));
        PSA_HIP_CHECK(hipMemsetAsync((char*)d_diff + pd16_fold_table_bytes((int)n_stage) - b_pad, 0, b_pad, c->stream));
    } else {
        PSA_HIP_CHECK(hipMemsetAsync((char*)d_diff + (size_t)M_pad_d * g.A_pad * 2, 0,
                                     pd16_table_bytes(M_pad_d, g.A_pad) - (size_t)M_pad_d * g.A_pad * 2, c->stream));
    }
    return PSA_OK;
}

int launch_lowrank_tables(psa_ctx* c, const float* d_kvec, const double* d_kline, const double* d_geo, const double* d_kappa,
                          const float* d_mean_all, const int* d_idx, void* d_diff, void* d_nodes, const ProjGeom& g, int M_pad_d,
                          float dscale, bool pair) {
    PSA_REQUIRE(M_pad_d % D_M_BLK == 0 && M_pad_d >= 2 * g.K && g.A_pad % K1_BA == 0, "bad low-rank table geometry");
    PSA_REQUIRE(!pair || M_pad_d == LRP_ROWS, "the pair launch's image is one 512-row block");
    hipLaunchKernelGGL(pair ? diff_table_kernel<true> : diff_table_kernel<false>, dim3(M_pad_d / 2, (g.A_pad + 255) / 256), dim3(256), 0,
                       c->stream, d_kvec, d_kline, d_mean_all, d_idx, g.weights, 1.f / g.wscale, (_Float16*)d_diff, g.K, g.n_g, g.A_pad,
                       dscale);
    PSA_HIP_CHECK(hipGetLastError());
    if (pair) {
        const size_t n_stage = (size_t)g.A_pad / K1_BA, a_pad = LRP_PAD_STAGES * LRP_A_UNITS * 1024, b_pad = LRP_PAD_STAGES * LRP_B_UNITS * 1024;
        static_assert(LRP_ROWS == D_M_BLK, "the pair image has the size of one D block");
        PSA_HIP_CHECK(hipMemsetAsync((char*)d_diff + n_stage * LRP_A_UNITS * 1024, 0, a_pad, c->stream));
        PSA_HIP_CHECK(hipMemsetAsync((char*)d_diff + pd16_pair_table_bytes((int)n_stage) - b_pad, 0, b_pad, c->stream));
    } else {
        PSA_HIP_CHECK(hipMemsetAsync((char*)d_diff + (size_t)M_pad_d * g.A_pad * 2, 0,
                                     pd16_table_bytes(M_pad_d, g.A_pad) - (size_t)M_pad_d * g.A_pad * 2, c->stream));
    }
    hipLaunchKernelGGL(node_table_kernel, dim3(LOWRANK_NODES, (g.A_pad + 255) / 256), dim3(256), 0, c->stream, d_geo, d_kappa, d_mean_all,
                       d_idx, g.weights, 1.f / g.wscale, (_Float16*)d_nodes, g.n_g, g.A_pad);
    PSA_HIP_CHECK(hipGetLastError());
    return PSA_OK;
}

}
```

### psa_amd/csrc/lowrank_combine.hip

```cpp
#include "k1_f16.h"

namespace psa {

namespace {
__device__ __forceinline__ void rmac4(f32x2& s0, f32x2& s1, f32x2& s2, f32x2& s3, f32x2 w0, f32x2 w1, f32x2 w2, f32x2 w3, f32x2 xa,
                                      f32x2 xb) {
    asm("v_pk_fma_f32 %0, %4, %8, %0 op_sel_hi:[0,1,1]\n\t"
        "v_pk_fma_f32 %1, %5, %8, %1 op_sel_hi:[0,1,1]\n\t"
        "v_pk_fma_f32 %2, %6, %8, %2 op_sel_hi:[0,1,1]\n\t"
        "v_pk_fma_f32 %3, %7, %8, %3 op_sel_hi:[0,1,1]\n\t"
        "v_pk_fma_f32 %0, %4, %9, %0 op_sel:[1,0,0] op_sel_hi:[1,1,1]\n\t"
        "v_pk_fma_f32 %1, %5, %9, %1 op_sel:[1,0,0] op_sel_hi:[1,1,1]\n\t"
        "v_pk_fma_f32 %2, %6, %9, %2 op_sel:[1,0,0] op_sel_hi:[1,1,1]\n\t"
        "v_pk_fma_f32 %3, %7, %9, %3 op_sel:[1,0,0] op_sel_hi:[1,1,1]"
        : "+v"(s0), "+v"(s1), "+v"(s2), "+v"(s3)
        : "v"(w0), "v"(w1), "v"(w2), "v"(w3), "v"(xa), "v"(xb));
}
__device__ __forceinline__ float2 phase_add(float2 o, float2 ph, f32x2 s) {
    float pr = ph.x * s[0], pi = ph.x * s[1];
    pr = __builtin_fmaf(-ph.y, s[1], pr);
    pi = __builtin_fmaf(ph.y, s[0], pi);
    return make_float2(o.x + pr, o.y + pi);
}
}

constexpr int COMBINE_R_JB = 64;
constexpr int COMBINE_R_PF = 2;
__global__ void __launch_bounds__(256)
lowrank_combine_r_kernel(const float2* __restrict__ Qn, const float* __restrict__ Lm, const float2* __restrict__ phi,
                         float2* __restrict__ q, int64_t T, int64_t q_stride, int64_t qn_stride, int K) {
    __shared__ __attribute__((aligned(16))) f32x4 ls[COMBINE_R_JB * LOWRANK_NODES / 4];
    __shared__ float2 ps[COMBINE_R_JB];
    const int64_t t = (int64_t)blockIdx.x * 256 + threadIdx.x;
    const int     c = blockIdx.y;
    const bool    live = t < T;
    const int64_t tl = live ? t : T - 1;
    auto at = [&](int j) -> float2& { return q[((int64_t)j * 3 + c) * q_stride + tl]; };
    auto row = [&](int j) { return j < K ? j : K - 1; };
    constexpr int PF = COMBINE_R_PF;
    float2        nx[PF][4];
#pragma unroll
    for (int d = 0; d < PF; ++d)
#pragma unroll
        for (int r = 0; r < 4; ++r) nx[d][r] = at(row(4 * d + r));
    f32x2 v[LOWRANK_NODES];
#pragma unroll
    for (int l = 0; l < LOWRANK_NODES; ++l) {
        const float2 x = Qn[((int64_t)l * 3 + c) * qn_stride + tl];
        v[l] = f32x2{x.x, x.y};
    }
    const f32x4* l4 = reinterpret_cast<const f32x4*>(Lm);
    for (int j0 = 0; j0 < K; j0 += COMBINE_R_JB) {
        const int nj = K - j0 < COMBINE_R_JB ? K - j0 : COMBINE_R_JB;
        __syncthreads();
        for (int i = threadIdx.x; i < nj * LOWRANK_NODES / 4; i += 256) ls[i] = l4[(size_t)j0 * (LOWRANK_NODES / 4) + i];
        if (threadIdx.x < nj) ps[threadIdx.x] = phi[j0 + threadIdx.x];
        __syncthreads();
        if (!live) continue;
        for (int j = 0; j < nj; j += 4) {
            int    jr[4];
            float2 ov[4];
#pragma unroll
            for (int r = 0; r < 4; ++r) {
                jr[r] = j + r < nj ? j + r : nj - 1;
                ov[r] = nx[0][r];
            }
#pragma unroll
            for (int d = 0; d + 1 < PF; ++d)
#pragma unroll
                for (int r = 0; r < 4; ++r) nx[d][r] = nx[d + 1][r];
#pragma unroll
            for (int r = 0; r < 4; ++r) nx[PF - 1][r] = at(row(j0 + j + 4 * PF + r));
            f32x2 s0 = {0.f, 0.f}, s1 = {0.f, 0.f}, s2 = {0.f, 0.f}, s3 = {0.f, 0.f};
            asm volatile("s_nop 0" : "+v"(s0), "+v"(s1), "+v"(s2), "+v"(s3));
#pragma unroll
            for (int i = 0; i < LOWRANK_NODES / 4; ++i) {
                const f32x4 w0 = ls[jr[0] * (LOWRANK_NODES / 4) + i], w1 = ls[jr[1] * (LOWRANK_NODES / 4) + i];
                const f32x4 w2 = ls[jr[2] * (LOWRANK_NODES / 4) + i], w3 = ls[jr[3] * (LOWRANK_NODES / 4) + i];
                rmac4(s0, s1, s2, s3, f32x2{w0[0], w0[1]}, f32x2{w1[0], w1[1]}, f32x2{w2[0], w2[1]}, f32x2{w3[0], w3[1]}, v[4 * i],
                      v[4 * i + 1]);
                rmac4(s0, s1, s2, s3, f32x2{w0[2], w0[3]}, f32x2{w1[2], w1[3]}, f32x2{w2[2], w2[3]}, f32x2{w3[2], w3[3]}, v[4 * i + 2],
                      v[4 * i + 3]);
            }
            asm volatile("s_nop 0" : "+v"(s0), "+v"(s1), "+v"(s2), "+v"(s3));
            const f32x2 s[4] = {s0, s1, s2, s3};
#pragma unroll
            for (int r = 0; r < 4; ++r)
                if (j + r < nj) at(j0 + j + r) = phase_add(ov[r], ps[j + r], s[r]);
        }
    }
}

int launch_lowrank_combine_r(psa_ctx* c, const float2* d_qn, const float* d_L, const float2* d_phi, float2* d_q, const ProjGeom& g,
                             int64_t qn_stride) {
    const int64_t nb = (g.T + 255) / 256;
    PSA_REQUIRE(nb < (1ll << 31) && g.K > 0, "combine grid too large");
    hipLaunchKernelGGL(lowrank_combine_r_kernel, dim3((unsigned)nb, 3), dim3(256), 0, c->stream, d_qn, d_L, d_phi, d_q, g.T, g.q_stride,
                       qn_stride, g.K);
    PSA_HIP_CHECK(hipGetLastError());
    return PSA_OK;
}

}
```

### psa_amd/csrc/psa_ctx.h

```cpp
#pragma once
#include <hip/hip_runtime.h>
#include <rocfft/rocfft.h>
#include <rccl/rccl.h>

#include <cstdarg>
#include <cstdint>
#include <cstdio>
#include <map>
#include <memory>
#include <mutex>
#include <string>
#include <thread>
#include <utility>
#include <vector>

#include "psa_hip.h"

namespace psa {

void set_error(const char* fmt, ...);

#define PSA_HIP_CHECK(expr)                                                              \
    do {                                                                                 \
        hipError_t e_ = (expr);                                                          \
// ... 51 lines not shown
            cap = std::exchange(o.cap, 0);
        }
        return *this;
    }
    ~DevBuf() { release(); }
    int reserve(size_t bytes);
    void release();
    template <class T> T* as() const { return static_cast<T*>(ptr); }
};

struct FftPlan {
    rocfft_plan           plan = nullptr;
    rocfft_execution_info info = nullptr;
    size_t                work_bytes = 0;
    FftPlan() = default;
    FftPlan(FftPlan&& o) noexcept
        : plan(std::exchange(o.plan, nullptr)), info(std::exchange(o.info, nullptr)), work_bytes(std::exchange(o.work_bytes, 0)) {}
    FftPlan& operator=(FftPlan&& o) noexcept {
        std::swap(plan, o.plan);
        std::swap(info, o.info);
        std::swap(work_bytes, o.work_bytes);
        return *this;
    }
    ~FftPlan();
};

struct DataSlot {
    DevBuf  buf;
    int64_t T = 0, N = 0;
    bool    valid = false;
    uint64_t generation = 0;
    bool     absmax_known = false;
    unsigned absmax_bits = 0;
    bool                  blocks_known = false;
    std::vector<unsigned> block_absmax;
};

struct Timed {
    int        stage;
    hipEvent_t e0, e1;
};
struct TimingState {
    std::vector<hipEvent_t> pool;
    std::vector<Timed>      pending;
    double                  acc[8] = {};
    int64_t                 k1_launches = 0;
    double                  k1_ms = 0.0;
};

constexpr int K1_BA   = 32;
constexpr int LOWRANK_NODES = 64;
constexpr int K1_VROW = 96;
constexpr int K1_PROW = 36;

__host__ __device__ inline size_t p_tile_index(int m, int a, int m_blk, int n_stage) {
    return ((size_t)(m / m_blk) * n_stage + (a / K1_BA)) * ((size_t)m_blk * K1_PROW) +
           (size_t)(m % m_blk) * K1_PROW + (a % K1_BA);
}
inline size_t p_table_floats(int M_pad, int A_pad) { return (size_t)M_pad * (A_pad / K1_BA) * K1_PROW; }

enum class K1Family : int {
    f32 = 0,
    f16_fly = 2,
    bf16 = 3,
    f16_planes = 4,
};

struct ProjGeom {
    int64_t T = 0;
    int64_t q_stride = 0;
    int64_t N_tot = 0;
    int     n_g = 0;
    int     A_pad = 0;
    int     K = 0;
    int     M_pad = 0;
    int     m_blk = 0;
    K1Family split = K1Family::f32;
    float   vscale = 0.f;
    bool    lowrank = false;
    int     M_pad_d = 0;
    float   dscale = 0.f;
    bool    lr_pair = false;
    bool    lr_fold = false;
    const float* weights = nullptr;
    float        wscale = 1.f;
};

struct PlaneSet {
    DevBuf               buf;
    int                  slot = 0;
    uint64_t             generation = 0;
    bool                 all_atoms = true;
    std::vector<int32_t> idx;
    uint64_t             idx_hash = 0;
    bool                 displaced = false;
    std::vector<float>   mean;
    int64_t              T = 0, n_fg = 0;
    int                  n_g = 0, A_pad = 0;
    float                vscale = 0.f;
    uint64_t             last_use = 0;
};

constexpr int KMAP_MIRROR = (int)0x80000000u;

struct Stager {
    void*       pin[2] = {nullptr, nullptr};
    size_t      cap = 0;
    hipEvent_t  freed[2] = {nullptr, nullptr};
    hipStream_t copy_stream = nullptr;
};

}

enum { PSA_T_H2D = 0, PSA_T_PHASE, PSA_T_PROJECT, PSA_T_FFT, PSA_T_EPILOGUE, PSA_T_GATHER,
       PSA_T_TRANSPOSE, PSA_T_D2H, PSA_T_COUNT };

struct psa_ctx {
    psa_ctx();
    ~psa_ctx();
    psa_ctx(const psa_ctx&) = delete;
    psa_ctx& operator=(const psa_ctx&) = delete;

    int         device = 0;
    hipStream_t stream = nullptr;
    std::mutex  mu;
    int         k1_selector = PSA_K1_AUTO;
    int         compute_units = 0;

    psa::DataSlot slot[PSA_NUM_SLOTS + 1];
    std::vector<float> disp_mean;
    uint64_t           disp_source = 0;
    std::vector<unsigned> disp_block_absmax;
    std::vector<float>    disp_abs_mean;
    uint64_t              disp_abs_source = ~0ull;

    psa::DevBuf d_kvec, d_mean_all, d_idx, d_mean_g, d_phase, d_qwork, d_fft_work, d_tables, d_absmax;
    psa::DevBuf d_upload_max;
    psa::DevBuf d_zeros;
    psa::DevBuf d_qrows, d_stage, d_bin;

    std::vector<std::unique_ptr<psa::PlaneSet>> planes;
    std::vector<uint64_t> seen_groups;
    uint64_t plane_tick = 0, plane_call_mark = 0;
    int64_t  opt_planes, opt_planes_budget, opt_planes_eager, opt_planes_min_k;
    psa::Stager stager;
    hipStream_t d2h_stream = nullptr;
    hipEvent_t  d2h_ready = nullptr;

    int64_t fs_T_total = 0, fs_T_local = 0, fs_K_total = 0, fs_rows_k0 = 0, fs_rows_nk = 0;
    bool    fs_intensity = false;
    psa::DevBuf d_slab;
    psa::DevBuf d_out;
    psa::DevBuf d_aux;
    int64_t res_T = 0, res_K = 0;
    bool    res_intensity = false;
    int64_t              out_K = 0;
    std::vector<int32_t> kmap;
    psa::DevBuf          d_kmap, d_cols;
    int64_t              opt_fold_pairs;
    psa::DevBuf          d_inten;
    bool                 inten_valid = false;
    bool    slab_valid = false, out_valid = false;

    std::map<std::pair<int64_t, int64_t>, psa::FftPlan> plans;
    std::thread  fft_primer;
    psa::FftPlan primed;
    int64_t      primed_T = 0;
    int64_t      opt_fft_prime;
    int64_t      opt_k1_wide;
    int64_t      opt_k1_loader_waves;
    int64_t      opt_k1_lowrank;
    int64_t      opt_k1_lowrank_min_k;
    int64_t      opt_k1_lowrank_min_local;
    int64_t      lowrank_launches = 0;
    int64_t      opt_k1_lowrank_pair;
    int64_t      lowrank_pair_launches = 0;
    bool         k1_lowrank_fold = true;
    psa::DevBuf  d_lr_diff, d_lr_qn, d_lr_L, d_lr_phi, d_lr_f64;

    psa::DevBuf  d_weights;
    int64_t      weights_N = 0;
    float        weights_scale = 1.f;

    psa::DevBuf  d_seg_window, d_seg;
    int64_t      seg_L = 0, seg_hop = 0;
    double       seg_U = 0.0;
    bool         seg_boxcar = false;

    psa::DevBuf  d_vdos_work, d_vdos_pairs, d_vdos_off, d_vdos_mean, d_vdos_part, d_vdos_acc, d_vdos_out;
    int64_t      opt_vdos_work_bytes;

    psa::DevBuf  d_modes_work, d_modes_coef, d_modes_out;
    int64_t      opt_modes_work_bytes;

    psa::DevBuf  d_cov_slab, d_cov_g, d_cov_out;

    psa::DevBuf  d_peaks_spec, d_peaks_bands, d_peaks_part, d_peaks_fit, d_peaks_info;

    psa::DevBuf  d_rc_work, d_rc_kappa, d_rc_khat, d_rc_idx, d_rc_tiles, d_rc_ent, d_rc_slot, d_rc_dest, d_rc_bins, d_rc_scale,
                 d_rc_acc, d_rc_out, d_rc_groups, d_rc_part;
    int64_t      opt_dynamic_work_bytes;

    psa::DevBuf  d_corr_tab, d_corr_factor, d_corr_scale, d_corr_in, d_corr_out;

    psa::DevBuf  d_rs_idx, d_rs_items, d_rs_part, d_rs_acc;

    psa::DevBuf  d_msd_u, d_msd_img, d_msd_sums, d_msd_offs, d_msd_sizes, d_msd_lags, d_msd_out;

    psa::DevBuf  d_pair_c;

    psa::DevBuf  d_angle_work, d_angle_edges;
    psa::DevBuf  d_local_tab;

    psa::TimingState timing;
    double oneoff_ms[4] = {0, 0, 0, 0};
    psa::DevBuf      d_sync;

    int scratch_byte = -1;

    ncclComm_t comm = nullptr;
    int        rank = 0, nranks = 1;
};

namespace psa {

int launch_phase_table(psa_ctx* c, const float* d_kvec, const float* d_mean_all, const int* d_idx,
                       float* d_phase, const ProjGeom& g);
int launch_gather_mean(psa_ctx* c, const float* d_mean_all, const int* d_idx, float* d_mean_g,
                       const ProjGeom& g);
int launch_fill_synthetic(psa_ctx* c, float* d_v, int64_t T, int64_t N, uint64_t seed, int64_t t_offset, int n_modes,
                          const float* d_amp, const int* d_comp, const float* d_ct,
                          const float* d_st, const float* d_ca, const float* d_sa);
int launch_mean_over_frames(psa_ctx* c, const float* d_x, int64_t T, int64_t N, float* d_mean);
int launch_subtract_mean(psa_ctx* c, const float* d_x, const float* d_mean, float* d_out, int64_t T, int64_t N);
int launch_absmax_bits(psa_ctx* c, const float* d_x, int64_t n, unsigned* d_out, bool reset = true);
int launch_absmax_blocks(psa_ctx* c, const float* d_x, const float* d_mean, int64_t T, int64_t N, unsigned* d_out);

int  k1_mfma_block_rows(int K);
int  launch_k1_mfma(psa_ctx* c, const float* d_v, const float* d_phase, const int* d_idx,
                    const float* d_mean_g, float2* d_q, const ProjGeom& g, bool displacements);
int  launch_k1_wave(psa_ctx* c, const float* d_v, const float* d_phase, const int* d_idx,
                    const float* d_mean_g, float2* d_q, const ProjGeom& g, bool displacements);

bool   k1_split_eligible(const int* d_idx, int64_t N_tot, int64_t n_g, bool displacements);
int    k1_split_block_rows(int K);
size_t pb_table_bytes(int M_pad, int A_pad);
int    launch_phase_table_split(psa_ctx* c, const float* d_kvec, const float* d_mean_all, const int* d_idx,
                                void* d_phase, const ProjGeom& g);
int    launch_k1_split(psa_ctx* c, const float* d_v, const void* d_phase, const int* d_idx, float2* d_q,
                       const ProjGeom& g);

bool   k1_pair_eligible(const int* d_idx, int64_t N_tot, int64_t n_g, int64_t K, bool displacements);
int    k1_pair_atom_pad(int64_t n_g);
int    k1_pair_block_rows(int K);
float  k1_f16_vscale(unsigned absmax_bits);
size_t pf16_table_bytes(int M_pad, int A_pad);
int    launch_phase_table_f16(psa_ctx* c, const float* d_kvec, const float* d_mean_all, const int* d_idx,
                              void* d_phase, const ProjGeom& g);
int    launch_k1_pair(psa_ctx* c, const float* d_v, const void* d_phase, const int* d_idx, float2* d_q,
                      const ProjGeom& g);

int    k1_planes_block_rows(int K, bool wide);
int    launch_split_planes(psa_ctx* c, const float* d_x, const float* d_mean, const int* d_idx, void* d_planes, int64_t T,
                           int64_t N_tot, int n_g, int A_pad, float vscale);
int    launch_k1_planes(psa_ctx* c, const void* d_planes, const void* d_phase, float2* d_q, const ProjGeom& g,
                        int64_t n_fg);
int    launch_k1_planes_lw(psa_ctx* c, const void* d_planes, const void* d_phase, float2* d_q, const ProjGeom& g,
                           int64_t n_fg);
int    launch_k1_planes_lw2(psa_ctx* c, const void* d_planes, const void* d_phase, float2* d_q, const ProjGeom& g,
                            int64_t n_fg);

int    launch_k1_planes_wide(psa_ctx* c, const void* d_planes, const void* d_phase, float2* d_q, const ProjGeom& g,
                             int64_t n_fg);

size_t pd16_table_bytes(int M_pad, int A_pad);
int    launch_lowrank_tables(psa_ctx* c, const float* d_kvec, const double* d_kline, const double* d_geo, const double* d_kappa,
                             const float* d_mean_all, const int* d_idx, void* d_diff, void* d_nodes, const ProjGeom& g, int M_pad_d,
                             float dscale, bool pair);
int    launch_k1_planes_diff(psa_ctx* c, const void* d_planes, const void* d_diff, float2* d_q, const ProjGeom& g, int64_t n_fg,
                             float dscale);
int    launch_lowrank_tables_fold(psa_ctx* c, const float* d_kvec, const double* d_kline, const double* d_geo, const double* d_kappa,
                                  const float* d_mean_all, const int* d_idx, const float* d_L, const float2* d_phi, void* d_diff,
                                  void* d_nodes, const ProjGeom& g, int M_pad_d, float dscale, bool pair);

int    launch_k1_lowrank_pair(psa_ctx* c, const void* d_planes, const void* d_nodes, const void* d_diff, float2* d_qn, float2* d_q,
                              const ProjGeom& g, int64_t n_fg, float dscale);

int    launch_k1_lowrank_fold(psa_ctx* c, const void* d_planes, const void* d_nodes, const void* d_diff, float2* d_qn, float2* d_q,
                              const ProjGeom& g, int64_t n_fg, float dscale);

int    launch_lowrank_combine_r(psa_ctx* c, const float2* d_qn, const float* d_L, const float2* d_phi, float2* d_q, const ProjGeom& g,
                                int64_t qn_stride);

int launch_dft_bin(psa_ctx* c, const float2* d_q, int64_t T, int64_t bin, float2* d_out3);
int launch_scale_transpose_c64(psa_ctx* c, const float2* d_slab, float2* d_out, float* d_inten, int64_t T, int64_t n,
                               int64_t K_pitch, int64_t col_first, int64_t src_first, const int32_t* d_cols,
                               const int32_t* d_srcs);
int launch_intensity_accumulate(psa_ctx* c, const float2* d_q, float* d_slab_rows, int64_t T,
                                int64_t K_local, bool first_group);
int launch_transpose_f32(psa_ctx* c, const float* d_slab, float* d_out, int64_t T, int64_t K, const int32_t* d_srcs);
int launch_segment_window(psa_ctx* c, const float2* d_q, const float* d_w, float2* d_seg, int64_t T, int64_t L, int64_t H,
                          int64_t s0, int64_t ns, int64_t nk);
int launch_segment_window_rows(psa_ctx* c, const float2* d_q, const float* d_w, float2* d_seg, int64_t T, int64_t L, int64_t H,
                               int64_t s0, int64_t ns, int64_t n_series);
int launch_segment_power(psa_ctx* c, const float2* d_seg, float* d_rows, int64_t L, int64_t ns, int64_t nk, float inv_norm,
                         bool first);
constexpr int VDOS_TILE_PAIRS = 32;
int launch_vdos_gather(psa_ctx* c, const float* d_data, const float* d_mean, const float* d_weights, const float* d_win,
                       const int* d_pair_atoms, float2* d_work, int64_t T, int64_t N, int64_t L, int64_t H, int64_t s0,
                       int64_t ns, int64_t n_pairs);
int launch_vdos_power(psa_ctx* c, const float2* d_work, const int64_t* d_pair_off, double* d_part, double* d_acc, int64_t L,
                      int64_t ns, int64_t n_pairs, int64_t p0, int64_t g_first, int64_t n_groups, int64_t n_chunks);
int launch_vdos_finish(psa_ctx* c, const double* d_acc, float* d_out, int64_t L, int64_t rows, double scale);
int modes_tile(int64_t M);
int launch_mode_power(psa_ctx* c, const float2* d_S, const float2* d_coef, float* d_out, int64_t L, int64_t ns, int64_t nk,
                      int64_t B, int64_t M, int MT, int64_t K_pitch, int64_t k_col0, float scale, bool first);
int64_t covariance_chunks(int64_t T);
int64_t covariance_slab_floats(int64_t T, int64_t n, int n_w);
int launch_covariance(psa_ctx* c, const float2* d_S, const float* d_g, float* d_slab, double2* d_out, int64_t T, int64_t nk, int64_t B,
                      int n_w, int64_t K_pitch, int64_t k_col0, double scale);
int peaks_slices(int64_t C, int64_t rows);
int launch_peak_find(psa_ctx* c, const float* d_spec, int64_t C, const int32_t* d_bands, int lo, int hi, int row0, int row_end,
                     int n_slices, float* d_pmax, int* d_pidx, int* d_pflag);
int launch_peak_fit(psa_ctx* c, const float* d_spec, int64_t C, const int32_t* d_bands, int lo, int hi, const float* d_pmax,
                    const int* d_pidx, const int* d_pflag, int n_slices, double df, float window_hwhm, int half_window_bins,
                    int max_iter, float* d_fit, int32_t* d_info);
constexpr int DYN_THREADS = 256;
constexpr int DYN_ATOMS = 512;
constexpr int DYN_CHAIN = 128;
constexpr int DYN_FRAMES = 4;
int dynamic_slices(int64_t K);
int launch_dynamic_project(psa_ctx* c, const float* d_pos, const float* d_vel, const float* d_weights, const int* d_idx,
                           const float* d_kappa, float2* d_q, int64_t T, int64_t N, int64_t n_g, int64_t nk, bool currents,
                           int slices);
int launch_dynamic_power(psa_ctx* c, const float2* d_seg, const float* d_khat, float* d_out, int64_t L, int64_t ns, int64_t nk,
                         bool currents, int64_t K_pitch, int64_t k_col0, float scale, bool first);
int launch_dynamic_sincos(psa_ctx* c, const float* d_turns, float2* d_out, int64_t n);
constexpr int LAT_THREADS = 256;
constexpr int LAT_KS = 512;
constexpr int LAT_ATOMS = 128;
constexpr int LAT_TABLE = 3584;
constexpr int LAT_CHAIN = 128;
constexpr int LAT_FRAMES = 4;
constexpr int LAT_MAX_INDEX = 64;
constexpr int LAT_MAX_ENTRIES = 3 * (2 * LAT_MAX_INDEX + 1);
int launch_lattice_project(psa_ctx* c, const float* d_pos, const float* d_vel, const float* d_weights, const int* d_idx,
                           const float* box_hi, const float* box_lo, const int* d_tile_off, const unsigned short* d_ent,
                           const unsigned* d_slot, const int* d_dest, float2* d_q, int64_t T, int64_t N, int64_t n_g, int64_t tile0,
                           int64_t n_tiles, bool currents);
int launch_lattice_shell(psa_ctx* c, const float2* d_seg, const float* d_khat, const int* d_bin_start, double* d_acc, int64_t L,
                         int64_t ns, int64_t g0, int64_t nb, int64_t n_bins, bool currents);
int launch_lattice_finish(psa_ctx* c, const double* d_acc, const double* d_scale, float* d_out, int64_t n, int64_t n_bins);
constexpr int PARTIAL_MAX_SPECIES = 8;
constexpr int PARTIAL_MAX_PAIRS = PARTIAL_MAX_SPECIES * (PARTIAL_MAX_SPECIES + 1) / 2;
int launch_partial_power(psa_ctx* c, const float2* d_seg, const float* d_khat, float* d_out, int64_t L, int64_t ns, int64_t nk,
                         int n_species, bool currents, int64_t K_pitch, int64_t k_col0, float scale, bool first);
int launch_partial_shell(psa_ctx* c, const float2* d_seg, const float* d_khat, const int* d_bin_start, double* d_acc, int64_t L,
                         int64_t ns, int64_t g0, int64_t nb, int64_t n_bins, int n_species, bool currents);
constexpr int SELF_THREADS = 256;
constexpr int SELF_ATOMS = 4;
constexpr int SELF_FRAMES = 64;
constexpr int SELF_ENTRIES = 24;
constexpr int SELF_KS = 64;
int launch_self_series(psa_ctx* c, const float* d_pos, const float* d_weights, const int* d_idx, int64_t a0, const float* box_hi,
                       const float* box_lo, const int* d_tile, const unsigned short* d_ent, const unsigned* d_slot, const float* d_win,
                       float2* d_work, int64_t T, int64_t N, int64_t na, int64_t tile0, int64_t n_tiles, int64_t v0, int64_t nv,
                       int64_t L, int64_t H, int64_t s0, int64_t ns, int64_t pitch);
int launch_self_power(psa_ctx* c, const float2* d_work, const int* d_groups, double* d_part, double* d_acc, int64_t L, int64_t ns,
                      int64_t na, int64_t v0, int64_t nv, int64_t g_first, int64_t ng, int64_t cols, int64_t n_chunks, bool mirror);
constexpr int CORR_LAGS = 8;
// ... 129 lines not shown
```

Baseline: 59920 billion.

## Add 48-node low-rank Chebyshev route with folded residual tables

Adds a 48-node variant of the low-rank phase interpolation alongside the existing 64-node one. The plan, node tables, diff tables, combine kernel and a dedicated pair image support the new node count, and it becomes the default when folding is on. Fewer nodes mean less MFMA work and smaller node tables in the projection kernel. In exchange the interpolation residual grows; it is absorbed into the fp16 diff correction through a larger bound, which costs some precision headroom.

```diff
diff --git a/include/psa_hip.h b/include/psa_hip.h
--- a/include/psa_hip.h
+++ b/include/psa_hip.h
@@ -41,6 +41,7 @@
 int         psa_synchronize(psa_ctx* ctx);
 int         psa_set_k1(psa_ctx* ctx, int selector);
 int         psa_set_k1_lowrank_fold(psa_ctx* ctx, int on);
+int         psa_set_k1_lowrank_nodes(psa_ctx* ctx, int nodes);
 #define PSA_OPT_PLANES         0
 #define PSA_OPT_PLANES_BUDGET  1
 #define PSA_OPT_PLANES_EAGER   2
@@ -238,6 +239,8 @@
 
 int psa_lowrank_plan(const float* k_vectors, int64_t K, const float* mean_pos_all, int64_t N, const int32_t* idx,
                      int64_t n_g, int32_t* ok, double* geo, double* kappa, float* C, float* L, float* phi);
+int psa_lowrank_plan_nodes(const float* k_vectors, int64_t K, const float* mean_pos_all, int64_t N, const int32_t* idx,
+                           int64_t n_g, int32_t nodes, int32_t* ok, double* geo, double* kappa, float* C, float* L, float* phi);
 
 int psa_sed_single_bin(psa_ctx* ctx, int slot, const float* mean_pos_all, const float* k_vector,
                        const int32_t* idx, int64_t n_g, int32_t flags, int64_t i_w,
@@ -255,6 +258,7 @@
 int psa_k1_lowrank_pair_launches(psa_ctx* ctx, int64_t* launches);
 int psa_lowrank_pair_image(int32_t n_stage, int64_t* index, int64_t* bytes);
 int psa_lowrank_fold_image(int32_t n_stage, int64_t* index, int64_t* bytes);
+int psa_lowrank_n48_image(int32_t n_stage, int64_t* index, int64_t* bytes);
 int psa_debug_device_buffers(int64_t* count, int64_t* bytes);
 #define PSA_SCRATCH_REAL 0
 #define PSA_SCRATCH_INDEX 1
diff --git a/psa_amd/_hip.py b/psa_amd/_hip.py
--- a/psa_amd/_hip.py
+++ b/psa_amd/_hip.py
@@ -99,6 +99,7 @@
     "psa_synchronize": (C.c_int, [_ctx]),
     "psa_set_k1": (C.c_int, [_ctx, C.c_int]),
     "psa_set_k1_lowrank_fold": (C.c_int, [_ctx, C.c_int]),
+    "psa_set_k1_lowrank_nodes": (C.c_int, [_ctx, C.c_int]),
     "psa_set_option": (C.c_int, [_ctx, C.c_int, C.c_int64]),
     "psa_device_info": (C.c_int, [_ctx, C.c_char_p, C.c_int, C.POINTER(C.c_int), _i64p]),
     "psa_data_upload": (C.c_int, [_ctx, C.c_int, _f32p, C.c_int64, C.c_int64]),
@@ -208,6 +209,9 @@
     "psa_k1_lowrank_pair_launches": (C.c_int, [_ctx, _i64p]),
     "psa_lowrank_pair_image": (C.c_int, [C.c_int32, _i64p, _i64p]),
     "psa_lowrank_fold_image": (C.c_int, [C.c_int32, _i64p, _i64p]),
+    "psa_lowrank_n48_image": (C.c_int, [C.c_int32, _i64p, _i64p]),
+    "psa_lowrank_plan_nodes": (C.c_int, [_f32p, C.c_int64, _f32p, C.c_int64, _i32p, C.c_int64, C.c_int32, _i32p, _f64p, _f64p, _f32p,
+                                         _f32p, _f32p]),
     "psa_oneoff_stats": (C.c_int, [_ctx, _f64p]),
     "psa_option_info": (C.c_int, [C.c_int, C.POINTER(C.c_int32), _i64p, C.POINTER(C.c_char_p)]),
     "psa_debug_device_buffers": (C.c_int, [_i64p, _i64p]),
@@ -353,6 +357,32 @@
             "dscale_fold": geo[13], "kappa": kappa, "C": cm, "L": lw, "phi": phi}
 
 
+def lowrank_plan_nodes(k_vectors, mean_pos_all, idx=None, nodes=48):
+    kv = _as_f32(k_vectors, (3,))
+    mean = _as_f32(mean_pos_all, (3,))
+    K, N, nodes = kv.shape[0], mean.shape[0], int(nodes)
+    ix = None if idx is None else np.ascontiguousarray(idx, np.int32)
+    n_g = N if ix is None else ix.size
+    ok, geo = C.c_int32(0), np.zeros(15, np.float64)
+    kappa, cm = np.zeros(nodes, np.float64), np.zeros((K, nodes), np.complex64)
+    lw, phi = np.zeros((K, nodes), np.float32), np.zeros(K, np.complex64)
+    _check(load_library().psa_lowrank_plan_nodes(_f32(kv), K, _f32(mean), N, None if ix is None else ix.ctypes.data_as(_i32p), n_g,
+                                                 nodes, C.byref(ok), geo.ctypes.data_as(_f64p), kappa.ctypes.data_as(_f64p),
+                                                 cm.ctypes.data_as(_f32p), _f32(lw), phi.ctypes.data_as(_f32p)),
+           "psa_lowrank_plan_nodes")
+    if not ok.value:
+        return None
+    return {"u": geo[0:3].copy(), "k0": geo[3:6].copy(), "x_c": geo[6], "h_x": geo[7], "width": geo[8],
+            "interval": int(geo[9]), "d_bound": geo[10], "dscale": geo[11], "e_bound": geo[12],
+            "dscale_fold": geo[13], "r_bound": geo[14], "nodes": nodes, "kappa": kappa, "C": cm, "L": lw, "phi": phi}
+
+
+def lowrank_n48_image(n_stage: int):
+    index, nbytes = np.zeros((512, 32 * int(n_stage)), np.int64), C.c_int64(0)
+    _check(load_library().psa_lowrank_n48_image(int(n_stage), index.ctypes.data_as(_i64p), C.byref(nbytes)), "psa_lowrank_n48_image")
+    return index, nbytes.value
+
+
 def lowrank_pair_image(n_stage: int):
     index, nbytes = np.zeros((512, 32 * int(n_stage)), np.int64), C.c_int64(0)
     _check(load_library().psa_lowrank_pair_image(int(n_stage), index.ctypes.data_as(_i64p), C.byref(nbytes)), "psa_lowrank_pair_image")
@@ -513,6 +543,9 @@
     def set_lowrank_fold(self, on: bool):
         _check(self._lib.psa_set_k1_lowrank_fold(self._h, int(bool(on))), "psa_set_k1_lowrank_fold")
 
+    def set_k1_lowrank_nodes(self, nodes: int):
+        _check(self._lib.psa_set_k1_lowrank_nodes(self._h, int(nodes)), "psa_set_k1_lowrank_nodes")
+
     def device_info(self) -> dict:
         name = C.create_string_buffer(256)
         cu, mem = C.c_int(0), C.c_int64(0)
diff --git a/psa_amd/csrc/api_core.hip b/psa_amd/csrc/api_core.hip
--- a/psa_amd/csrc/api_core.hip
+++ b/psa_amd/csrc/api_core.hip
@@ -411,6 +411,14 @@
     return PSA_OK;
 }
 
+int psa_set_k1_lowrank_nodes(psa_ctx* c, int nodes) {
+    PSA_TRY(enter(c));
+    PSA_REQUIRE(nodes == 48 || nodes == 64, "the low-rank route has 48 or 64 nodes, not %d", nodes);
+    Guard g(c);
+    c->k1_lowrank_nodes = nodes;
+    return PSA_OK;
+}
+
 int psa_set_option(psa_ctx* c, int option, int64_t value) {
     PSA_TRY(enter(c));
     Guard g(c);
diff --git a/psa_amd/csrc/api_internal.h b/psa_amd/csrc/api_internal.h
--- a/psa_amd/csrc/api_internal.h
+++ b/psa_amd/csrc/api_internal.h
@@ -124,17 +124,19 @@
     double              u[3] = {0, 0, 0}, k0[3] = {0, 0, 0};
     double              x_c = 0, h_x = 0, width = 0;
     int64_t             interval = 0;
+    int                 nodes = LOWRANK_NODES;
     double              kappa[LOWRANK_NODES] = {};
     double              d_bound = 0;
     float               dscale = 0.f;
     double              e_bound = 0;
     float               dscale_fold = 0.f;
+    double              r_bound = 0;
     std::vector<double> kline;
     std::vector<float>  L;
     std::vector<float>  phi;
 };
 int plan_lowrank(const float* k, int64_t K, const float* mean_all, int64_t N, const int32_t* h_idx, int64_t n_g, LowRankPlan* p,
-                 float* C = nullptr);
+                 float* C = nullptr, int nodes = LOWRANK_NODES, bool want_r = false);
 int prepare_lowrank(psa_ctx* c, const GroupView& v, const ProjectArgs& list, int64_t k_first, int64_t nk, ProjGeom* g);
 struct ModesArgs {
     int            slot;
diff --git a/psa_amd/csrc/api_lowrank.hip b/psa_amd/csrc/api_lowrank.hip
--- a/psa_amd/csrc/api_lowrank.hip
+++ b/psa_amd/csrc/api_lowrank.hip
@@ -1,5 +1,6 @@
 #include "api_internal.h"
 #include "k1_lowrank_fold.h"
+#include "k1_lowrank_n48.h"
 #include "k1_lowrank_pair.h"
 
 namespace psa {
@@ -7,11 +8,15 @@
 namespace {
 constexpr double LR_OMEGA = 30.0;
 constexpr double LR_D_MAX = 1.0 / 8192.0;
+constexpr double LR48_R_MAX = 1e-6;
+static_assert(LR_OMEGA == 30.0 && LOWRANK_NODES_48 == 48, "LR48_R_MAX was worked out for 48 nodes on h_k h_x = 30");
 }
 
 int plan_lowrank(const float* k, int64_t K, const float* mean_all, int64_t N, const int32_t* h_idx, int64_t n_g, LowRankPlan* p,
-                 float* C) {
+                 float* C, int nodes, bool want_r) {
     *p = LowRankPlan{};
+    PSA_REQUIRE(nodes == LOWRANK_NODES || nodes == LOWRANK_NODES_48, "the plan has 48 or 64 nodes");
+    p->nodes = nodes;
     auto fail = [&](const char* why) {
         p->why = why;
         return PSA_OK;
@@ -121,47 +126,72 @@
     p->interval = side ? (int64_t)n0 : -(int64_t)n0 - 1;
     const double mid = (p->interval + 0.5) * p->width, half = 0.5 * p->width;
     double       bw[LOWRANK_NODES];
-    for (int l = 0; l < LOWRANK_NODES; ++l) {
-        const double th = M_PI * (2 * l + 1) / (2.0 * LOWRANK_NODES);
+    for (int l = 0; l < nodes; ++l) {
+        const double th = M_PI * (2 * l + 1) / (2.0 * nodes);
         p->kappa[l] = mid + half * std::cos(th);
         bw[l] = ((l & 1) ? -1.0 : 1.0) * std::sin(th);
     }
-    p->L.assign((size_t)K * LOWRANK_NODES, 0.f);
+    p->L.assign((size_t)K * nodes, 0.f);
     p->phi.assign((size_t)K * 2, 0.f);
     for (int64_t j = 0; j < K; ++j) {
         const double kj = kap[(size_t)j];
         double       L[LOWRANK_NODES], den = 0.0;
         int          hit = -1;
-        for (int l = 0; l < LOWRANK_NODES; ++l)
+        for (int l = 0; l < nodes; ++l)
             if (kj == p->kappa[l]) hit = l;
         if (hit >= 0) {
-            for (int l = 0; l < LOWRANK_NODES; ++l) L[l] = l == hit;
+            for (int l = 0; l < nodes; ++l) L[l] = l == hit;
         } else {
-            for (int l = 0; l < LOWRANK_NODES; ++l) {
+            for (int l = 0; l < nodes; ++l) {
                 L[l] = bw[l] / (kj - p->kappa[l]);
                 den += L[l];
             }
-            for (double& v : L) v /= den;
+            for (int l = 0; l < nodes; ++l) L[l] /= den;
         }
         const double cr = std::cos(kj * p->x_c), ci = std::sin(kj * p->x_c);
         p->phi[(size_t)j * 2 + 0] = (float)cr;
         p->phi[(size_t)j * 2 + 1] = (float)ci;
-        for (int l = 0; l < LOWRANK_NODES; ++l) {
-            p->L[(size_t)j * LOWRANK_NODES + l] = (float)L[l];
+        for (int l = 0; l < nodes; ++l) {
+            p->L[(size_t)j * nodes + l] = (float)L[l];
             if (C) {
-                C[((size_t)j * LOWRANK_NODES + l) * 2 + 0] = (float)(cr * L[l]);
-                C[((size_t)j * LOWRANK_NODES + l) * 2 + 1] = (float)(ci * L[l]);
+                C[((size_t)j * nodes + l) * 2 + 0] = (float)(cr * L[l]);
+                C[((size_t)j * nodes + l) * 2 + 1] = (float)(ci * L[l]);
             }
         }
     }
     p->dscale = std::ldexp(1.0f, 14 - (int)std::ceil(std::log2(p->d_bound)));
     for (int64_t j = 0; j < K; ++j) {
         double lam = 0.0;
-        for (int l = 0; l < LOWRANK_NODES; ++l) lam += std::fabs((double)p->L[(size_t)j * LOWRANK_NODES + l]);
+        for (int l = 0; l < nodes; ++l) lam += std::fabs((double)p->L[(size_t)j * nodes + l]);
         const double rot = std::fabs((double)p->phi[(size_t)j * 2]) + std::fabs((double)p->phi[(size_t)j * 2 + 1]);
         p->e_bound = std::max(p->e_bound, rot * lam * 0x1p-12);
     }
     p->dscale_fold = std::ldexp(1.0f, 14 - (int)std::ceil(std::log2(p->d_bound + p->e_bound)));
+    if (nodes == LOWRANK_NODES_48) {
+        p->dscale_fold = std::ldexp(1.0f, 14 - (int)std::ceil(std::log2(p->d_bound + p->e_bound + LR48_R_MAX)));
+        if (want_r) {
+            std::vector<double> wr((size_t)nodes), wi((size_t)nodes);
+            for (int64_t a = 0; a < n_g; ++a) {
+                const float* r = mean_all + 3 * (h_idx ? h_idx[a] : a);
+                const double y = (u[0] * r[0] + u[1] * r[1] + u[2] * r[2]) - p->x_c;
+                const double t0 = p->k0[0] * r[0] + p->k0[1] * r[1] + p->k0[2] * r[2];
+                for (int l = 0; l < nodes; ++l) {
+                    wr[(size_t)l] = std::cos(t0 + p->kappa[l] * y);
+                    wi[(size_t)l] = std::sin(t0 + p->kappa[l] * y);
+                }
+                for (int64_t j = 0; j < K; ++j) {
+                    double sr = 0.0, si = 0.0;
+                    for (int l = 0; l < nodes; ++l) {
+                        sr += (double)p->L[(size_t)j * nodes + l] * wr[(size_t)l];
+                        si += (double)p->L[(size_t)j * nodes + l] * wi[(size_t)l];
+                    }
+                    const double pr = p->phi[(size_t)j * 2], pi = p->phi[(size_t)j * 2 + 1];
+                    const double th = p->kline[3 * j] * r[0] + p->kline[3 * j + 1] * r[1] + p->kline[3 * j + 2] * r[2];
+                    p->r_bound = std::max(p->r_bound, std::hypot(std::cos(th) - (pr * sr - pi * si), std::sin(th) - (pr * si + pi * sr)));
+                }
+            }
+        }
+    }
     p->ok = true;
     return PSA_OK;
 }
@@ -171,25 +201,28 @@
     if (!c->opt_k1_lowrank || g->split != K1Family::f16_planes || !v.ps || list.K_total < c->opt_k1_lowrank_min_k ||
         nk < c->opt_k1_lowrank_min_local)
         return PSA_OK;
+    const int   nodes = c->k1_lowrank_fold && c->k1_lowrank_nodes == LOWRANK_NODES_48 ? LOWRANK_NODES_48 : LOWRANK_NODES;
     LowRankPlan p;
-    PSA_TRY(plan_lowrank(list.k_vectors + 3 * k_first, nk, list.mean_pos_all, c->slot[v.slot].N, v.h_idx, g->n_g, &p));
+    PSA_TRY(plan_lowrank(list.k_vectors + 3 * k_first, nk, list.mean_pos_all, c->slot[v.slot].N, v.h_idx, g->n_g, &p, nullptr, nodes));
     if (!p.ok) return PSA_OK;
-    std::vector<double> f64((size_t)7 + LOWRANK_NODES + 3 * (size_t)nk);
+    const bool          kline = nodes == LOWRANK_NODES;
+    std::vector<double> f64((size_t)7 + nodes + (kline ? 3 * (size_t)nk : 0));
     std::memcpy(f64.data(), p.k0, 3 * sizeof(double));
     std::memcpy(f64.data() + 3, p.u, 3 * sizeof(double));
     f64[6] = p.x_c;
-    std::memcpy(f64.data() + 7, p.kappa, sizeof(p.kappa));
-    std::memcpy(f64.data() + 7 + LOWRANK_NODES, p.kline.data(), p.kline.size() * sizeof(double));
+    std::memcpy(f64.data() + 7, p.kappa, (size_t)nodes * sizeof(double));
+    if (kline) std::memcpy(f64.data() + 7 + nodes, p.kline.data(), p.kline.size() * sizeof(double));
     PSA_TRY(upload(c, c->d_lr_f64, f64.data(), f64.size() * sizeof(double)));
     PSA_TRY(upload(c, c->d_lr_L, p.L.data(), p.L.size() * sizeof(float)));
     PSA_TRY(upload(c, c->d_lr_phi, p.phi.data(), p.phi.size() * sizeof(float)));
-    PSA_TRY(c->d_lr_qn.reserve((size_t)LOWRANK_NODES * 3 * (size_t)c->slot[v.slot].T * sizeof(float2)));
+    PSA_TRY(c->d_lr_qn.reserve((size_t)nodes * 3 * (size_t)c->slot[v.slot].T * sizeof(float2)));
     g->lowrank = true;
+    g->lr_nodes = nodes;
     g->lr_fold = c->k1_lowrank_fold;
     g->dscale = g->lr_fold ? p.dscale_fold : p.dscale;
     g->M_pad_d = (int)((2 * nk + 511) / 512 * 512);
     g->lr_pair = c->opt_k1_lowrank_pair && g->M_pad_d == LRP_ROWS;
-    static_assert(LRF_ROWS == LRP_ROWS, "the folded pair launch serves the lists the pair launch serves");
+    static_assert(LRF_ROWS == LRP_ROWS && LRN_ROWS == LRP_ROWS, "the folded pair launches serve the lists the pair launch serves");
     return PSA_OK;
 }
 
@@ -216,6 +249,32 @@
     return PSA_OK;
 }
 
+int psa_lowrank_plan_nodes(const float* k_vectors, int64_t K, const float* mean_pos_all, int64_t N, const int32_t* idx, int64_t n_g,
+                           int32_t nodes, int32_t* ok, double* geo, double* kappa, float* C, float* L, float* phi) {
+    PSA_REQUIRE(K >= 0 && K < (1ll << 29) && N >= 1 && n_g >= 0 && n_g <= (idx ? (int64_t)1 << 30 : N) && ok && geo &&
+                    (K == 0 || k_vectors) && mean_pos_all && (nodes == LOWRANK_NODES || nodes == LOWRANK_NODES_48),
+                "bad argument");
+    LowRankPlan p;
+    PSA_TRY(plan_lowrank(k_vectors, K, mean_pos_all, N, idx, n_g, &p, C, nodes, true));
+    *ok = p.ok;
+    const double g[15] = {p.u[0],  p.u[1],  p.u[2],  p.k0[0], p.k0[1], p.k0[2], p.x_c, p.h_x, p.width, (double)p.interval,
+                          p.d_bound, p.dscale, p.e_bound, p.dscale_fold, p.r_bound};
+    std::memcpy(geo, g, sizeof(g));
+    if (p.ok && kappa) std::memcpy(kappa, p.kappa, (size_t)nodes * sizeof(double));
+    if (p.ok && L) std::memcpy(L, p.L.data(), p.L.size() * sizeof(float));
+    if (p.ok && phi) std::memcpy(phi, p.phi.data(), p.phi.size() * sizeof(float));
+    return PSA_OK;
+}
+
+int psa_lowrank_n48_image(int32_t n_stage, int64_t* index, int64_t* bytes) {
+    PSA_REQUIRE(n_stage >= 1 && n_stage < (1 << 20) && bytes, "bad argument");
+    *bytes = (int64_t)pd16_n48_table_bytes(n_stage);
+    if (index)
+        for (int m = 0; m < LRN_ROWS; ++m)
+            for (int a = 0; a < n_stage * K1_BA; ++a) index[(size_t)m * n_stage * K1_BA + a] = (int64_t)pd16_n48_index(m, a, n_stage);
+    return PSA_OK;
+}
+
 int psa_lowrank_pair_image(int32_t n_stage, int64_t* index, int64_t* bytes) {
     PSA_REQUIRE(n_stage >= 1 && n_stage < (1 << 20) && bytes, "bad argument");
     *bytes = (int64_t)pd16_pair_table_bytes(n_stage);
diff --git a/psa_amd/csrc/api_project.hip b/psa_amd/csrc/api_project.hip
--- a/psa_amd/csrc/api_project.hip
+++ b/psa_amd/csrc/api_project.hip
@@ -248,6 +248,9 @@
         PSA_TRY(c->d_phase.reserve(pf16_table_bytes(128, g.A_pad)));
         StageTimer    st(c, PSA_T_PHASE);
         const double* f64 = c->d_lr_f64.as<double>();
+        if (g.lr_nodes == 48)
+            return launch_lowrank_tables_n48(c, d_kvec, f64, f64 + 7, c->d_mean_all.as<float>(), d_idx, c->d_lr_L.as<float>(),
+                                             c->d_lr_phi.as<float2>(), c->d_lr_diff.ptr, c->d_phase.ptr, g, g.M_pad_d, g.dscale, g.lr_pair);
         if (g.lr_fold)
             return launch_lowrank_tables_fold(c, d_kvec, f64 + 7 + LOWRANK_NODES, f64, f64 + 7, c->d_mean_all.as<float>(), d_idx,
                                               c->d_lr_L.as<float>(), c->d_lr_phi.as<float2>(), c->d_lr_diff.ptr, c->d_phase.ptr, g,
@@ -302,13 +305,16 @@
         const _Float16* pl = ps->buf.as<_Float16>() + (size_t)fg0 * (size_t)(ps->A_pad / K1_BA) * PL_STAGE_ELEMS;
         if (g.lowrank) {
             ProjGeom gn = g;
-            gn.K = LOWRANK_NODES;
+            gn.K = g.lr_nodes;
             gn.m_blk = gn.M_pad = 2 * LOWRANK_NODES;
             gn.q_stride = t_count;
-            PSA_REQUIRE(c->d_lr_qn.cap >= (size_t)LOWRANK_NODES * 3 * t_count * sizeof(float2), "node projections not reserved");
+            PSA_REQUIRE(g.lr_nodes == LOWRANK_NODES || (g.lr_nodes == 48 && g.lr_fold), "48 nodes only with the fold");
+            PSA_REQUIRE(c->d_lr_qn.cap >= (size_t)g.lr_nodes * 3 * t_count * sizeof(float2), "node projections not reserved");
             if (g.lr_pair) {
-                PSA_TRY((g.lr_fold ? launch_k1_lowrank_fold : launch_k1_lowrank_pair)(c, pl, c->d_phase.ptr, c->d_lr_diff.ptr,
-                                                                                      c->d_lr_qn.as<float2>(), d_q, g, n_fg, g.dscale));
+                PSA_TRY((g.lr_nodes == 48 ? launch_k1_lowrank_n48
+                         : g.lr_fold      ? launch_k1_lowrank_fold
+                                          : launch_k1_lowrank_pair)(c, pl, c->d_phase.ptr, c->d_lr_diff.ptr, c->d_lr_qn.as<float2>(), d_q,
+                                                                    g, n_fg, g.dscale));
                 ++c->lowrank_pair_launches;
             } else {
                 PSA_TRY((g.lr_fold ? launch_k1_planes_lw2 : launch_k1_planes_lw)(c, pl, c->d_phase.ptr, c->d_lr_qn.as<float2>(), gn, n_fg));
diff --git a/psa_amd/csrc/k1_lowrank_n48.h b/psa_amd/csrc/k1_lowrank_n48.h
--- /dev/null
+++ b/psa_amd/csrc/k1_lowrank_n48.h
@@ -0,0 +1,32 @@
+#pragma once
+#include "k1_tile.h"
+
+namespace psa {
+
+constexpr int LOWRANK_NODES_48 = 48;
+constexpr int LRN_ROWS = 512;
+constexpr int LRN_NODE_MT = 3;
+constexpr int LRN_A_ROWS = 160, LRN_A_MT = 5, LRN_A_UNITS = 2 * LRN_A_MT;
+constexpr int LRN_B_MT = 11, LRN_B_UNITS = 2 * LRN_B_MT;
+constexpr int LRN_PAD_STAGES = 4;
+static_assert(2 * 16 * LRN_NODE_MT == 2 * LOWRANK_NODES_48, "six row tiles hold the 48 nodes' cos and sin rows");
+static_assert(LRN_A_ROWS == 16 * LRN_A_UNITS && LRN_A_ROWS + 16 * LRN_B_UNITS == LRN_ROWS, "the two roles share the block's rows");
+static_assert(2 * LRN_NODE_MT + LRN_A_MT == LRN_B_MT, "both roles multiply the same per stage");
+
+__host__ __device__ inline size_t lrn_b_first_unit(int n_stage) { return (size_t)(n_stage + LRN_PAD_STAGES) * LRN_A_UNITS; }
+__host__ __device__ inline size_t pd16_n48_index(int m, int a, int n_stage) {
+    const int rt = m >> 4, r = m & 15, al = a % K1_BA, st = a / K1_BA;
+    size_t    unit;
+    if (rt < LRN_A_UNITS) {
+        unit = (size_t)st * LRN_A_UNITS + (size_t)(2 * (rt % LRN_A_MT) + rt / LRN_A_MT);
+    } else {
+        const int rb = rt - LRN_A_UNITS, h = rb / LRN_B_MT, mt = rb % LRN_B_MT;
+        unit = lrn_b_first_unit(n_stage) + (size_t)st * LRN_B_UNITS + (size_t)(2 * mt + h);
+    }
+    return unit * (16 * K1_BA) + (size_t)r * K1_BA + (size_t)((((al >> 3) ^ pl_swizzle(r)) << 3) + (al & 7));
+}
+__host__ __device__ inline size_t pd16_n48_table_bytes(int n_stage) {
+    return (size_t)(n_stage + LRN_PAD_STAGES) * (LRN_A_UNITS + LRN_B_UNITS) * 1024;
+}
+
+}
diff --git a/psa_amd/csrc/k1_lowrank_n48.hip b/psa_amd/csrc/k1_lowrank_n48.hip
--- /dev/null
+++ b/psa_amd/csrc/k1_lowrank_n48.hip
@@ -0,0 +1,309 @@
+#include <utility>
+
+#include "k1_f16.h"
+#include "k1_lowrank_n48.h"
+
+namespace psa {
+
+namespace {
+constexpr int LN_T_BLK = 64, LN_PERIOD = 4;
+constexpr int LNA_STAGE_UNITS = 24 + 2 * LRN_NODE_MT + LRN_A_UNITS, LNA_RING_UNITS = LN_PERIOD * LNA_STAGE_UNITS, LNA_FOLD = 8;
+constexpr int LNA_NODE_U0 = 24, LNA_D_U0 = 24 + 2 * LRN_NODE_MT, LNA_DMA = LNA_STAGE_UNITS / 4;
+constexpr int LNB_STAGE_UNITS = 12 + LRN_B_UNITS, LNB_RING_UNITS = LN_PERIOD * LNB_STAGE_UNITS, LNB_D_U0 = 12;
+constexpr int LNB_DMA = (LNB_STAGE_UNITS + 3) / 4, LNB_LAST = LNB_STAGE_UNITS - 4 * (LNB_DMA - 1);
+constexpr int LN_NODE_STAGE_BYTES = pf16_stage_bytes(128);
+static_assert(LNA_STAGE_UNITS == 40 && LNA_RING_UNITS == 160 && LNA_FOLD % LN_PERIOD == 0 && LNA_DMA == 10 && LNA_D_U0 == 30,
+              "role A's ring is four whole stages");
+static_assert(LNB_STAGE_UNITS == 34 && LNB_RING_UNITS == 136 && LNB_DMA == 9 && LNB_LAST == 2, "role B's ring is four whole stages");
+static_assert(3 * 2 * LRN_NODE_MT + 3 * LRN_A_MT == 3 * LRN_B_MT && 3 * LRN_B_MT == 33, "both roles multiply the same per stage: 33 MFMAs per wavefront");
+constexpr auto a_unit_off = unit_off<LNA_STAGE_UNITS, LNA_RING_UNITS, LN_PERIOD>;
+constexpr auto b_unit_off = unit_off<LNB_STAGE_UNITS, LNB_RING_UNITS, LN_PERIOD>;
+constexpr int lnb_slot(int s4, int mt) { return (LRN_B_MT * s4 + mt) & 3; }
+static_assert((LRN_B_MT * LN_PERIOD) % 4 == 0, "the fragment slots repeat with the ring");
+}
+
+__global__ void __launch_bounds__(512, 2)
+k1_lowrank_n48_kernel(const _Float16* __restrict__ planes, const _Float16* __restrict__ Pn, const _Float16* __restrict__ Dp,
+                      float2* __restrict__ Qn, float2* __restrict__ Q, int64_t T, int64_t q_stride, int n_fg, int n_stage, int K,
+                      int n_tblk, float qscale_n, float qscale_d) {
+    using PR = F16x2;
+    using E8 = PR::v8;
+    using std::integral_constant;
+    __shared__ __attribute__((aligned(16))) unsigned char smem[LNA_RING_UNITS * 1024];
+    const unsigned lds0 = (unsigned)(size_t)(lds_u8*)smem;
+
+    int mb, tb;
+    if (!k1_block_map(2, n_tblk, mb, tb)) return;
+
+    const int tid = threadIdx.x, lane = tid & 63;
+    const int w = __builtin_amdgcn_readfirstlane(tid >> 6);
+    const int wh = w >> 2, wf = w & 3;
+    const int r16 = lane & 15, q = lane >> 4;
+
+    int fg = tb * 4 + wf;
+    if (fg >= n_fg) fg = n_fg - 1;
+    const unsigned char* pl0 = reinterpret_cast<const unsigned char*>(planes) + (size_t)fg * n_stage * PL_STAGE_BYTES;
+    const unsigned dma_voff = 16 * lane;
+    const unsigned wbase = lds0 + 1024 * wf;
+    const unsigned lane_off = lds0 + r16 * (K1_BA * 2) + ((q ^ pl_swizzle(r16)) << 4);
+    unsigned       lane_a[3], lane_b[3];
+    unit_ring_windows(lane_off + 1024 * wh, lane_off + 1024 * wf, lane_a, lane_b);
+    using I0 = integral_constant<int, 0>;
+    using I1 = integral_constant<int, 1>;
+    using I2 = integral_constant<int, 2>;
+
+    if (mb == 0) {
+        const unsigned char* src[LNA_DMA];
+        unsigned             inc7;
+#pragma unroll
+        for (int i = 0; i < 6; ++i) src[i] = pl0 + 1024 * i;
+#pragma unroll
+        for (int i = 6; i < LNA_DMA; ++i) {
+            const int u = 4 * i + wf;
+            if (u < LNA_D_U0) {
+                const int x = u - LNA_NODE_U0;
+                src[i] = reinterpret_cast<const unsigned char*>(Pn) + 1024 * (LRN_NODE_MT * (x & 1) + (x >> 1));
+            } else {
+                src[i] = reinterpret_cast<const unsigned char*>(Dp) + 1024 * (u - LNA_D_U0);
+            }
+        }
+        inc7 = 4 * 7 + wf < LNA_D_U0 ? LN_NODE_STAGE_BYTES : LRN_A_UNITS * 1024;
+        auto dma = [&](auto s4_c, auto i_c) __attribute__((always_inline)) {
+            constexpr int      S4 = decltype(s4_c)::value, I = decltype(i_c)::value;
+            constexpr unsigned OFF = a_unit_off(S4, 4 * I);
+            if constexpr (I < 6) {
+                lds_dma16_at<OFF, (I & 1) != 0>(src[I], dma_voff, wbase);
+                src[I] += PL_STAGE_BYTES;
+            } else if constexpr (I == 6) {
+                lds_dma16_at<OFF, false>(src[I], dma_voff, wbase);
+                src[I] += LN_NODE_STAGE_BYTES;
+            } else if constexpr (I == 7) {
+                lds_dma16_at<OFF, false>(src[I], dma_voff, wbase);
+                src[I] += inc7;
+            } else {
+                lds_dma16_at<OFF, false>(src[I], dma_voff, wbase);
+                src[I] += LRN_A_UNITS * 1024;
+            }
+        };
+        auto dma_stage = [&](auto s4_c) __attribute__((always_inline)) {
+            [&]<int... Is>(std::integer_sequence<int, Is...>) __attribute__((always_inline)) { (dma(s4_c, integral_constant<int, Is>{}), ...); }(
+                std::make_integer_sequence<int, LNA_DMA>{});
+        };
+
+        E8    a[2][LRN_NODE_MT];
+        E8    ad[2][LRN_A_MT];
+        E8    bb[3][2];
+        f32x4 hi[LRN_NODE_MT][3], lo[LRN_NODE_MT][3], accd[LRN_A_MT][3];
+        auto  read_a = [&](auto s_c, auto mt_c) __attribute__((always_inline)) {
+            constexpr int S = decltype(s_c)::value, MTI = decltype(mt_c)::value;
+            a[S & 1][MTI] = lds_frag(lane_a, a_unit_off(S, LNA_NODE_U0 + 2 * MTI));
+        };
+        auto read_ad = [&](auto s_c, auto mt_c) __attribute__((always_inline)) {
+            constexpr int S = decltype(s_c)::value, MTI = decltype(mt_c)::value;
+            ad[S & 1][MTI] = lds_frag(lane_a, a_unit_off(S, LNA_D_U0 + 2 * MTI));
+        };
+        auto read_b = [&](auto s_c, auto c_c, auto p_c) __attribute__((always_inline)) {
+            constexpr int S = decltype(s_c)::value, CC = decltype(c_c)::value, P = decltype(p_c)::value;
+            bb[CC][P] = lds_frag(lane_b, a_unit_off(S, 4 * (2 * CC + P)));
+        };
+        auto each_node = [&](auto&& f) __attribute__((always_inline)) {
+            [&]<int... Ms>(std::integer_sequence<int, Ms...>) __attribute__((always_inline)) { (f(integral_constant<int, Ms>{}), ...); }(
+                std::make_integer_sequence<int, LRN_NODE_MT>{});
+        };
+        auto each_d = [&](auto&& f) __attribute__((always_inline)) {
+            [&]<int... Ms>(std::integer_sequence<int, Ms...>) __attribute__((always_inline)) { (f(integral_constant<int, Ms>{}), ...); }(
+                std::make_integer_sequence<int, LRN_A_MT>{});
+        };
+        static_assert(LNA_FOLD % 2 == 0, "the fragment sets alternate with the stage");
+#pragma unroll
+        for (int c = 0; c < 3; ++c) {
+#pragma unroll
+            for (int mt = 0; mt < LRN_NODE_MT; ++mt) {
+                hi[mt][c] = f32x4{0.f, 0.f, 0.f, 0.f};
+                lo[mt][c] = f32x4{0.f, 0.f, 0.f, 0.f};
+            }
+#pragma unroll
+            for (int mt = 0; mt < LRN_A_MT; ++mt) accd[mt][c] = f32x4{0.f, 0.f, 0.f, 0.f};
+        }
+
+        if (wh == 0) {
+            dma_stage(I0{});
+            dma_stage(I1{});
+            dma_stage(I2{});
+        }
+        asm volatile("s_waitcnt vmcnt(%0)\n\ts_barrier" ::"n"(LNA_DMA) : "memory");
+        each_node([&](auto mt_c) __attribute__((always_inline)) { read_a(I0{}, mt_c); });
+        read_b(I0{}, I0{}, I1{});
+        read_b(I0{}, I0{}, I0{});
+        each_d([&](auto mt_c) __attribute__((always_inline)) { read_ad(I0{}, mt_c); });
+        read_b(I0{}, I1{}, I1{});
+        read_b(I0{}, I1{}, I0{});
+        read_b(I0{}, I2{}, I1{});
+        read_b(I0{}, I2{}, I0{});
+
+        int  left = n_stage;
+        auto stage = [&](auto s_c) __attribute__((always_inline)) {
+            constexpr int S = decltype(s_c)::value, PAR = S & 1;
+            if (left <= S) return;
+            constexpr bool restart = S == 0;
+            using SN = integral_constant<int, (S + 1) % LNA_FOLD>;
+            using S3 = integral_constant<int, (S + 3) % LNA_FOLD>;
+            if (wh == 0) dma_stage(S3{});
+            auto comp = [&](auto c_c) __attribute__((always_inline)) {
+                constexpr int CC = decltype(c_c)::value;
+                f32x4         ch[LRN_NODE_MT];
+                each_node([&](auto mt_c) __attribute__((always_inline)) {
+                    constexpr int MTI = decltype(mt_c)::value;
+                    ch[MTI] = PR::mma(a[PAR][MTI], bb[CC][1], restart ? f32x4{0.f, 0.f, 0.f, 0.f} : hi[MTI][CC]);
+                });
+                read_b(SN{}, c_c, I1{});
+                if constexpr (CC == 0) each_node([&](auto mt_c) __attribute__((always_inline)) { read_a(SN{}, mt_c); });
+                if constexpr (CC == 1) each_d([&](auto mt_c) __attribute__((always_inline)) { read_ad(SN{}, mt_c); });
+                __builtin_amdgcn_sched_barrier(0);
+                each_d([&](auto mt_c) __attribute__((always_inline)) {
+                    constexpr int MTI = decltype(mt_c)::value;
+                    accd[MTI][CC] = PR::mma(ad[PAR][MTI], bb[CC][0], accd[MTI][CC]);
+                });
+                each_node([&](auto mt_c) __attribute__((always_inline)) {
+                    constexpr int MTI = decltype(mt_c)::value;
+                    hi[MTI][CC] = PR::mma(a[PAR][MTI], bb[CC][0], ch[MTI]);
+                });
+                read_b(SN{}, c_c, I0{});
+                __builtin_amdgcn_sched_barrier(0);
+            };
+            comp(I0{});
+            comp(I1{});
+            comp(I2{});
+            asm volatile("s_waitcnt vmcnt(%0)\n\ts_barrier" ::"n"(LNA_DMA) : "memory");
+        };
+        for (; left > 0; left -= LNA_FOLD) {
+            [&]<int... Ss>(std::integer_sequence<int, Ss...>) __attribute__((always_inline)) { (stage(integral_constant<int, Ss>{}), ...); }(
+                std::make_integer_sequence<int, LNA_FOLD>{});
+            k1_fold(lo, hi);
+        }
+        asm volatile("s_waitcnt vmcnt(0)" ::: "memory");
+
+        const int     lane_e = __builtin_amdgcn_mbcnt_hi(~0u, __builtin_amdgcn_mbcnt_lo(~0u, 0u));
+        const int     r16_e = lane_e & 15, q_e = lane_e >> 4;
+        const int64_t t = (int64_t)tb * LN_T_BLK + wf * 16 + r16_e;
+        k1_store_q(Qn, lo, wh * LOWRANK_NODES_48, q_e, t, T, LOWRANK_NODES_48, T, qscale_n);
+        k1_store_q(Q, accd, wh * (LRN_A_ROWS / 2), q_e, t, T, K, q_stride, qscale_d);
+    } else {
+        const unsigned char* src[LNB_DMA];
+#pragma unroll
+        for (int i = 0; i < 3; ++i) src[i] = pl0 + 1024 * (2 * i);
+        const unsigned char* d0 = reinterpret_cast<const unsigned char*>(Dp) + lrn_b_first_unit(n_stage) * 1024;
+#pragma unroll
+        for (int i = 3; i < LNB_DMA; ++i) src[i] = d0 + 1024 * (wf + 4 * (i - 3));
+        const bool ninth = wf < LNB_LAST;
+        auto dma = [&](auto s4_c, auto i_c) __attribute__((always_inline)) {
+            constexpr int      S4 = decltype(s4_c)::value, I = decltype(i_c)::value;
+            constexpr unsigned OFF = b_unit_off(S4, 4 * I);
+            if constexpr (I == LNB_DMA - 1) {
+                if (ninth) {
+                    lds_dma16_at<OFF, false>(src[I], dma_voff, wbase);
+                    src[I] += LRN_B_UNITS * 1024;
+                }
+            } else {
+                lds_dma16_at<OFF, false>(src[I], dma_voff, wbase);
+                src[I] += I < 3 ? PL_STAGE_BYTES : LRN_B_UNITS * 1024;
+            }
+        };
+        auto dma_stage = [&](auto s4_c) __attribute__((always_inline)) {
+            [&]<int... Is>(std::integer_sequence<int, Is...>) __attribute__((always_inline)) { (dma(s4_c, integral_constant<int, Is>{}), ...); }(
+                std::make_integer_sequence<int, LNB_DMA>{});
+        };
+        auto landed = [&]() __attribute__((always_inline)) {
+            if (ninth)
+                asm volatile("s_waitcnt vmcnt(%0)" ::"n"(LNB_DMA) : "memory");
+            else
+                asm volatile("s_waitcnt vmcnt(%0)" ::"n"(LNB_DMA - 1) : "memory");
+            asm volatile("s_barrier" ::: "memory");
+        };
+
+        E8    a[4];
+        E8    bf[3];
+        f32x4 acc[LRN_B_MT][3];
+        auto read_a = [&](auto s4_c, auto mt_c) __attribute__((always_inline)) {
+            constexpr int S4 = decltype(s4_c)::value, MTI = decltype(mt_c)::value;
+            a[lnb_slot(S4, MTI)] = lds_frag(lane_a, b_unit_off(S4, LNB_D_U0 + 2 * MTI));
+        };
+        auto read_b = [&](auto s4_c, auto c_c) __attribute__((always_inline)) {
+            constexpr int S4 = decltype(s4_c)::value, CC = decltype(c_c)::value;
+            bf[CC] = lds_frag(lane_b, b_unit_off(S4, 4 * CC));
+        };
+#pragma unroll
+        for (int mt = 0; mt < LRN_B_MT; ++mt)
+#pragma unroll
+            for (int c = 0; c < 3; ++c) acc[mt][c] = f32x4{0.f, 0.f, 0.f, 0.f};
+
+        if (wh == 0) {
+            dma_stage(I0{});
+            dma_stage(I1{});
+            dma_stage(I2{});
+        }
+        landed();
+        read_b(I0{}, I0{});
+        read_b(I0{}, I1{});
+        read_b(I0{}, I2{});
+        read_a(I0{}, I0{});
+        read_a(I0{}, I1{});
+
+        int  left = n_stage;
+        auto stage = [&](auto s4_c) __attribute__((always_inline)) {
+            constexpr int S4 = decltype(s4_c)::value;
+            if (left <= S4) return;
+            using SN = integral_constant<int, (S4 + 1) % LN_PERIOD>;
+            using S3 = integral_constant<int, (S4 + 3) % LN_PERIOD>;
+            if (wh == 0) dma_stage(S3{});
+            auto tile = [&](auto mt_c) __attribute__((always_inline)) {
+                constexpr int MTI = decltype(mt_c)::value;
+                if constexpr (MTI + 2 < LRN_B_MT)
+                    read_a(s4_c, integral_constant<int, MTI + 2>{});
+                else
+                    read_a(SN{}, integral_constant<int, MTI + 2 - LRN_B_MT>{});
+                auto comp = [&](auto c_c) __attribute__((always_inline)) {
+                    constexpr int CC = decltype(c_c)::value;
+                    acc[MTI][CC] = PR::mma(a[lnb_slot(S4, MTI)], bf[CC], acc[MTI][CC]);
+                    if constexpr (MTI == LRN_B_MT - 1) read_b(SN{}, c_c);
+                };
+                comp(I0{});
+                comp(I1{});
+                comp(I2{});
+                __builtin_amdgcn_sched_barrier(0);
+            };
+            [&]<int... Ms>(std::integer_sequence<int, Ms...>) __attribute__((always_inline)) { (tile(integral_constant<int, Ms>{}), ...); }(
+                std::make_integer_sequence<int, LRN_B_MT>{});
+            landed();
+        };
+        for (; left > 0; left -= LN_PERIOD)
+            [&]<int... Ss>(std::integer_sequence<int, Ss...>) __attribute__((always_inline)) { (stage(integral_constant<int, Ss>{}), ...); }(
+                std::make_integer_sequence<int, LN_PERIOD>{});
+        asm volatile("s_waitcnt vmcnt(0)" ::: "memory");
+
+        const int lane_e = __builtin_amdgcn_mbcnt_hi(~0u, __builtin_amdgcn_mbcnt_lo(~0u, 0u));
+        const int r16_e = lane_e & 15, q_e = lane_e >> 4;
+        k1_store_q(Q, acc, wh * (16 * LRN_B_MT) + LRN_A_ROWS, q_e, (int64_t)tb * LN_T_BLK + wf * 16 + r16_e, T, K, q_stride, qscale_d);
+    }
+}
+
+int launch_k1_lowrank_n48(psa_ctx* c, const void* d_planes, const void* d_nodes, const void* d_diff, float2* d_qn, float2* d_q,
+                          const ProjGeom& g, int64_t n_fg, float dscale) {
+    PSA_REQUIRE(g.M_pad_d == LRN_ROWS && 2 * g.K <= LRN_ROWS && g.K > 0, "48-node pair launch: one 512-row D block only");
+    PSA_REQUIRE(g.A_pad % (2 * K1_BA) == 0 && g.A_pad > 0, "48-node pair launch needs the atom axis padded to %d", 2 * K1_BA);
+    PSA_REQUIRE(g.vscale > 0.f && dscale > 0.f && n_fg * 16 >= g.T, "planes do not cover the launch");
+    ProjGeom g2 = g;
+    g2.M_pad = 2 * LRN_ROWS;
+    K1Grid gr;
+    PSA_TRY(k1_grid(g2, LRN_ROWS, LN_T_BLK, gr));
+    PSA_REQUIRE(gr.n_mblk == 2 && gr.n_tblk < (1 << 29) && n_fg < (1ll << 31), "projection grid too large");
+    const float qscale_n = 1.f / (g.vscale * F16x2::P_SCALE) * g.wscale;
+    const float qscale_d = 1.f / (g.vscale * dscale) * g.wscale;
+    hipLaunchKernelGGL(k1_lowrank_n48_kernel, dim3(gr.blocks), dim3(512), 0, c->stream, (const _Float16*)d_planes,
+                       (const _Float16*)d_nodes, (const _Float16*)d_diff, d_qn, d_q, g.T, g.q_stride, (int)n_fg, g.A_pad / K1_BA, g.K,
+                       gr.n_tblk, qscale_n, qscale_d);
+    PSA_HIP_CHECK(hipGetLastError());
+    return PSA_OK;
+}
+
+}
diff --git a/psa_amd/csrc/k1_planes_diff.hip b/psa_amd/csrc/k1_planes_diff.hip
--- a/psa_amd/csrc/k1_planes_diff.hip
+++ b/psa_amd/csrc/k1_planes_diff.hip
@@ -2,6 +2,7 @@
 
 #include "k1_f16.h"
 #include "k1_lowrank_fold.h"
+#include "k1_lowrank_n48.h"
 #include "k1_lowrank_pair.h"
 
 namespace psa {
@@ -315,4 +316,117 @@
     return PSA_OK;
 }
 
-}
+__global__ void __launch_bounds__(256)
+node_table_n48_kernel(const double* __restrict__ geo, const double* __restrict__ kappa, const float* __restrict__ mean_all,
+                      const int* __restrict__ idx, const float* __restrict__ w, float wnorm, _Float16* __restrict__ Pb, int n_g,
+                      int A_pad) {
+    const int a = blockIdx.y * 256 + threadIdx.x;
+    const int l = blockIdx.x;
+    if (a >= A_pad) return;
+    double cs[2] = {0.0, 0.0};
+    if (a < n_g && l < LOWRANK_NODES_48) {
+        const int    src = idx ? idx[a] : a;
+        const double rx = mean_all[3 * (size_t)src + 0], ry = mean_all[3 * (size_t)src + 1], rz = mean_all[3 * (size_t)src + 2];
+        const double th = (geo[0] * rx + geo[1] * ry + geo[2] * rz) + kappa[l] * ((geo[3] * rx + geo[4] * ry + geo[5] * rz) - geo[6]);
+        sincos(th, &cs[1], &cs[0]);
+        if (w) {
+            const double wa = (double)(w[src] * wnorm);
+            cs[0] *= wa;
+            cs[1] *= wa;
+        }
+    }
+    const int n_stage = A_pad / K1_BA;
+#pragma unroll
+    for (int ri = 0; ri < 2; ++ri) {
+        const double   x = cs[ri] * (double)F16x2::P_SCALE;
+        const _Float16 lead = (_Float16)(float)x;
+        Pb[pf16_tile_index(0, 2 * l + ri, a, 128, n_stage)] = lead;
+        Pb[pf16_tile_index(1, 2 * l + ri, a, 128, n_stage)] = (_Float16)(float)(x - (double)lead);
+    }
+}
+
+__device__ __forceinline__ _Float16 f64_to_f16(double x) {
+    float        f = (float)x;
+    const double e = x - (double)f;
+    if (e != 0.0 && f != 0.f) {
+        unsigned b = __float_as_uint(f);
+        if (!(b & 1u)) {
+            const bool grow = (e > 0.0) == !(b >> 31);
+            f = __uint_as_float(grow ? b + 1u : b - 1u);
+        }
+    }
+    return (_Float16)f;
+}
+
+template <bool N48>
+__global__ void __launch_bounds__(256)
+diff_n48_table_kernel(const float* __restrict__ kvec, const float* __restrict__ mean_all, const int* __restrict__ idx,
+                      const float* __restrict__ w, float wnorm, const _Float16* __restrict__ Pn, const float* __restrict__ L,
+                      const float2* __restrict__ phi, _Float16* __restrict__ Db, int K, int n_g, int A_pad, float dscale) {
+    constexpr int NN = LOWRANK_NODES_48;
+    const int     a = blockIdx.y * 256 + threadIdx.x;
+    const int     k0 = blockIdx.x * FOLD_JB;
+    if (a >= A_pad) return;
+    const int n_stage = A_pad / K1_BA;
+    double    wh[2 * NN];
+#pragma unroll
+    for (int m = 0; m < 2 * NN; ++m) wh[m] = (double)(float)Pn[pf16_tile_index(0, m, a, 128, n_stage)];
+    float  rx = 0.f, ry = 0.f, rz = 0.f;
+    double wa = 0.0;
+    if (a < n_g) {
+        const int src = idx ? idx[a] : a;
+        rx = mean_all[3 * (size_t)src + 0], ry = mean_all[3 * (size_t)src + 1], rz = mean_all[3 * (size_t)src + 2];
+        wa = w ? (double)(w[src] * wnorm) : 1.0;
+    }
+    for (int k = k0; k < k0 + FOLD_JB; ++k) {
+        double d[2] = {0.0, 0.0};
+        if (k < K && a < n_g) {
+            const float* Lk = L + (size_t)k * NN;
+            double       sr = 0.0, si = 0.0;
+#pragma unroll
+            for (int l = 0; l < NN; ++l) {
+                const double ll = (double)Lk[l];
+                sr = fma(ll, wh[2 * l], sr);
+                si = fma(ll, wh[2 * l + 1], si);
+            }
+            const float2 ph = phi[k];
+            const double pr = (double)ph.x, pi = (double)ph.y;
+            const double er = fma(-pi, si, pr * sr), ei = fma(pi, sr, pr * si);
+            const float  kx = kvec[3 * k + 0], ky = kvec[3 * k + 1], kz = kvec[3 * k + 2];
+            const float  arg = __fmaf_rn(kz, rz, __fmaf_rn(ky, ry, __fmul_rn(kx, rx)));
+            float        cs[2];
+            sincosf(arg, &cs[1], &cs[0]);
+            constexpr double inv_p = 1.0 / (double)F16x2::P_SCALE;
+            d[0] = ((double)cs[0] * wa - er * inv_p) * (double)dscale;
+            d[1] = ((double)cs[1] * wa - ei * inv_p) * (double)dscale;
+        }
+        Db[N48 ? pd16_n48_index(2 * k, a, n_stage) : pd16_index(2 * k, a, n_stage)] = f64_to_f16(d[0]);
+        Db[N48 ? pd16_n48_index(2 * k + 1, a, n_stage) : pd16_index(2 * k + 1, a, n_stage)] = f64_to_f16(d[1]);
+    }
+}
+
+int launch_lowrank_tables_n48(psa_ctx* c, const float* d_kvec, const double* d_geo, const double* d_kappa, const float* d_mean_all,
+                              const int* d_idx, const float* d_L, const float2* d_phi, void* d_diff, void* d_nodes, const ProjGeom& g,
+                              int M_pad_d, float dscale, bool pair) {
+    PSA_REQUIRE(M_pad_d % D_M_BLK == 0 && M_pad_d >= 2 * g.K && g.A_pad % K1_BA == 0, "bad low-rank table geometry");
+    PSA_REQUIRE(!pair || M_pad_d == LRN_ROWS, "the 48-node pair launch's image is one 512-row block");
+    hipLaunchKernelGGL(node_table_n48_kernel, dim3(64, (g.A_pad + 255) / 256), dim3(256), 0, c->stream, d_geo, d_kappa, d_mean_all,
+                       d_idx, g.weights, 1.f / g.wscale, (_Float16*)d_nodes, g.n_g, g.A_pad);
+    PSA_HIP_CHECK(hipGetLastError());
+    hipLaunchKernelGGL(pair ? diff_n48_table_kernel<true> : diff_n48_table_kernel<false>,
+                       dim3(M_pad_d / 2 / FOLD_JB, (g.A_pad + 255) / 256), dim3(256), 0, c->stream, d_kvec, d_mean_all, d_idx, g.weights,
+                       1.f / g.wscale, (const _Float16*)d_nodes, d_L, d_phi, (_Float16*)d_diff, g.K, g.n_g, g.A_pad, dscale);
+    PSA_HIP_CHECK(hipGetLastError());
+    if (pair) {
+        const size_t n_stage = (size_t)g.A_pad / K1_BA, a_pad = LRN_PAD_STAGES * LRN_A_UNITS * 1024, b_pad = LRN_PAD_STAGES * LRN_B_UNITS * 1024;
+        static_assert(LRN_ROWS == D_M_BLK, "the 48-node image has the size of one D block");
+        PSA_HIP_CHECK(hipMemsetAsync((char*)d_diff + n_stage * LRN_A_UNITS * 1024, 0, a_pad, c->stream));
+        PSA_HIP_CHECK(hipMemsetAsync((char*)d_diff + pd16_n48_table_bytes((int)n_stage) - b_pad, 0, b_pad, c->stream));
+    } else {
+        PSA_HIP_CHECK(hipMemsetAsync((char*)d_diff + (size_t)M_pad_d * g.A_pad * 2, 0,
+                                     pd16_table_bytes(M_pad_d, g.A_pad) - (size_t)M_pad_d * g.A_pad * 2, c->stream));
+    }
+    return PSA_OK;
+}
+
+}
diff --git a/psa_amd/csrc/lowrank_combine.hip b/psa_amd/csrc/lowrank_combine.hip
--- a/psa_amd/csrc/lowrank_combine.hip
+++ b/psa_amd/csrc/lowrank_combine.hip
@@ -26,10 +26,11 @@
 
 constexpr int COMBINE_R_JB = 64;
 constexpr int COMBINE_R_PF = 2;
+template <int NODES>
 __global__ void __launch_bounds__(256)
 lowrank_combine_r_kernel(const float2* __restrict__ Qn, const float* __restrict__ Lm, const float2* __restrict__ phi,
                          float2* __restrict__ q, int64_t T, int64_t q_stride, int64_t qn_stride, int K) {
-    __shared__ __attribute__((aligned(16))) f32x4 ls[COMBINE_R_JB * LOWRANK_NODES / 4];
+    __shared__ __attribute__((aligned(16))) f32x4 ls[COMBINE_R_JB * NODES / 4];
     __shared__ float2 ps[COMBINE_R_JB];
     const int64_t t = (int64_t)blockIdx.x * 256 + threadIdx.x;
     const int     c = blockIdx.y;
@@ -43,9 +44,9 @@
     for (int d = 0; d < PF; ++d)
 #pragma unroll
         for (int r = 0; r < 4; ++r) nx[d][r] = at(row(4 * d + r));
-    f32x2 v[LOWRANK_NODES];
+    f32x2 v[NODES];
 #pragma unroll
-    for (int l = 0; l < LOWRANK_NODES; ++l) {
+    for (int l = 0; l < NODES; ++l) {
         const float2 x = Qn[((int64_t)l * 3 + c) * qn_stride + tl];
         v[l] = f32x2{x.x, x.y};
     }
@@ -53,7 +54,7 @@
     for (int j0 = 0; j0 < K; j0 += COMBINE_R_JB) {
         const int nj = K - j0 < COMBINE_R_JB ? K - j0 : COMBINE_R_JB;
         __syncthreads();
-        for (int i = threadIdx.x; i < nj * LOWRANK_NODES / 4; i += 256) ls[i] = l4[(size_t)j0 * (LOWRANK_NODES / 4) + i];
+        for (int i = threadIdx.x; i < nj * NODES / 4; i += 256) ls[i] = l4[(size_t)j0 * (NODES / 4) + i];
         if (threadIdx.x < nj) ps[threadIdx.x] = phi[j0 + threadIdx.x];
         __syncthreads();
         if (!live) continue;
@@ -74,9 +75,9 @@
             f32x2 s0 = {0.f, 0.f}, s1 = {0.f, 0.f}, s2 = {0.f, 0.f}, s3 = {0.f, 0.f};
             asm volatile("s_nop 0" : "+v"(s0), "+v"(s1), "+v"(s2), "+v"(s3));
 #pragma unroll
-            for (int i = 0; i < LOWRANK_NODES / 4; ++i) {
-                const f32x4 w0 = ls[jr[0] * (LOWRANK_NODES / 4) + i], w1 = ls[jr[1] * (LOWRANK_NODES / 4) + i];
-                const f32x4 w2 = ls[jr[2] * (LOWRANK_NODES / 4) + i], w3 = ls[jr[3] * (LOWRANK_NODES / 4) + i];
+            for (int i = 0; i < NODES / 4; ++i) {
+                const f32x4 w0 = ls[jr[0] * (NODES / 4) + i], w1 = ls[jr[1] * (NODES / 4) + i];
+                const f32x4 w2 = ls[jr[2] * (NODES / 4) + i], w3 = ls[jr[3] * (NODES / 4) + i];
                 rmac4(s0, s1, s2, s3, f32x2{w0[0], w0[1]}, f32x2{w1[0], w1[1]}, f32x2{w2[0], w2[1]}, f32x2{w3[0], w3[1]}, v[4 * i],
                       v[4 * i + 1]);
                 rmac4(s0, s1, s2, s3, f32x2{w0[2], w0[3]}, f32x2{w1[2], w1[3]}, f32x2{w2[2], w2[3]}, f32x2{w3[2], w3[3]}, v[4 * i + 2],
@@ -91,12 +92,16 @@
     }
 }
 
+template __global__ void lowrank_combine_r_kernel<LOWRANK_NODES>(const float2*, const float*, const float2*, float2*, int64_t, int64_t, int64_t, int);
+template __global__ void lowrank_combine_r_kernel<48>(const float2*, const float*, const float2*, float2*, int64_t, int64_t, int64_t, int);
+
 int launch_lowrank_combine_r(psa_ctx* c, const float2* d_qn, const float* d_L, const float2* d_phi, float2* d_q, const ProjGeom& g,
                              int64_t qn_stride) {
     const int64_t nb = (g.T + 255) / 256;
     PSA_REQUIRE(nb < (1ll << 31) && g.K > 0, "combine grid too large");
-    hipLaunchKernelGGL(lowrank_combine_r_kernel, dim3((unsigned)nb, 3), dim3(256), 0, c->stream, d_qn, d_L, d_phi, d_q, g.T, g.q_stride,
-                       qn_stride, g.K);
+    PSA_REQUIRE(g.lr_nodes == LOWRANK_NODES || g.lr_nodes == 48, "combine: 48 or 64 nodes");
+    hipLaunchKernelGGL(g.lr_nodes == LOWRANK_NODES ? lowrank_combine_r_kernel<LOWRANK_NODES> : lowrank_combine_r_kernel<48>, dim3((unsigned)nb, 3),
+                       dim3(256), 0, c->stream, d_qn, d_L, d_phi, d_q, g.T, g.q_stride, qn_stride, g.K);
     PSA_HIP_CHECK(hipGetLastError());
     return PSA_OK;
 }
diff --git a/psa_amd/csrc/psa_ctx.h b/psa_amd/csrc/psa_ctx.h
--- a/psa_amd/csrc/psa_ctx.h
+++ b/psa_amd/csrc/psa_ctx.h
@@ -157,6 +157,7 @@
     float   dscale = 0.f;
     bool    lr_pair = false;
     bool    lr_fold = false;
+    int     lr_nodes = 64;
     const float* weights = nullptr;
     float        wscale = 1.f;
 };
@@ -250,6 +251,7 @@
     int64_t      lowrank_launches = 0;
     int64_t      opt_k1_lowrank_pair;
     int64_t      lowrank_pair_launches = 0;
+    int          k1_lowrank_nodes = 48;
     bool         k1_lowrank_fold = true;
     psa::DevBuf  d_lr_diff, d_lr_qn, d_lr_L, d_lr_phi, d_lr_f64;
 
@@ -361,6 +363,11 @@
 int    launch_k1_lowrank_pair(psa_ctx* c, const void* d_planes, const void* d_nodes, const void* d_diff, float2* d_qn, float2* d_q,
                               const ProjGeom& g, int64_t n_fg, float dscale);
 
+int    launch_lowrank_tables_n48(psa_ctx* c, const float* d_kvec, const double* d_geo, const double* d_kappa, const float* d_mean_all,
+                                 const int* d_idx, const float* d_L, const float2* d_phi, void* d_diff, void* d_nodes, const ProjGeom& g,
+                                 int M_pad_d, float dscale, bool pair);
+int    launch_k1_lowrank_n48(psa_ctx* c, const void* d_planes, const void* d_nodes, const void* d_diff, float2* d_qn, float2* d_q,
+                             const ProjGeom& g, int64_t n_fg, float dscale);
 int    launch_k1_lowrank_fold(psa_ctx* c, const void* d_planes, const void* d_nodes, const void* d_diff, float2* d_qn, float2* d_q,
                               const ProjGeom& g, int64_t n_fg, float dscale);
 
```

New measurement: 63510 billion (median of 6 runs). 6.0% higher.
